# SIA-IDE/MMGT

Measured on AMD Instinct MI355X. Metric: UNet3D denoise-steps/sec at 512x512x24 bf16, higher is better.
Workload: dtype bf16; 1 GPU; BASELINE configs[1]: 512x512x24 pose2vid denoise step (CFG batch 2, UNet3D + MM-HAA, 16 reference banks, 1 window of 24 frames, guidance 3.5, DDIM v-pred), random-init weights; frames=24, parallelism=clip-parallel x1

## Files before the change

### include/mmgt_hip.h

```cpp
#ifndef MMGT_HIP_H
#define MMGT_HIP_H

#ifdef __cplusplus
extern "C" {
#endif

#define MMGT_F32 0
#define MMGT_BF16 1

#define MMGT_ACT_NONE 0
#define MMGT_ACT_GEGLU 1
#define MMGT_ACT_SILU 2
#define MMGT_ACT_RELU 3
#define MMGT_ACT_QUICK_GELU 4
#define MMGT_ACT_GELU 5
#define MMGT_ACT_MISH 6

int mmgt_abi_version(void);
const char* mmgt_last_error(void);
int mmgt_tune(const char* key, int value);
int mmgt_tune_get(const char* key, int* value);
int mmgt_box_calib(float warm_seconds, float* mfma_mhz, float* mfma_tflops, void* stream);
void mmgt_gemm16_set_trace(void* p);
void mmgt_ffn_set_trace(void* p);

int mmgt_gemm(const void* A, long lda, const void* W, const float* bias, const float* bias2, int bias2_rows,
              const float* row_scale, float alpha, const void* residual, long ldr, void* out, long ldo, int M, int N,
              int K, int act, int batch, long bsA, long bsW, long bsR, long bsO, int dtype, void* stream);

int mmgt_gemm_post(const void* A, long lda, const void* W, const float* bias, const float* row_scale, float alpha,
                   const float* bias_post, const void* residual, long ldr, void* out, long ldo, int M, int N, int K,
                   int dtype, void* stream);

int mmgt_conv3x3_nhwc(const void* x0, int C0, const void* x1, int C1, int NB, int IH, int IW, int stride, int upsample,
                      const void* Wp, const float* bias, const float* bias2, int bias2_rows, const void* residual,
                      void* out, int Cout, int act, int dtype, void* stream);

int mmgt_conv1x1_cat_nhwc(const void* x0, int C0, const void* x1, int C1, long rows, const void* Wp, const float* bias, const void* residual, void* out,
                          int Cout, int dtype, void* stream);

int mmgt_conv_taps_gather(const void* Y, int ldY, const float* bias, void* out, int NB, int H, int W, int dtype, void* stream);

int mmgt_groupnorm_chunks(int HW);
int mmgt_groupnorm_affine(const void* x, int C, const float* gamma, const float* beta, float* workspace, float* scale, float* shift,
                          int NB, int HW, int G, float eps, int dtype, void* stream);
int mmgt_groupnorm_affine2(const void* x0, int C0, const void* x1, int C1, const float* gamma, const float* beta, float* workspace, float* scale,
                           float* shift, int NB, int HW, int G, float eps, int dtype, void* stream);
int mmgt_groupnorm_nhwc(const void* x0, int C0, const void* x1, int C1, const float* gamma, const float* beta, void* out,
                        float* workspace, int NB, int HW, int G, float eps, int silu, int dtype, void* stream);

int mmgt_layernorm(const void* x, long ldx, const float* gamma, const float* beta, float eps, const float* pe, int pe_div,
                   int pe_mod, void* out, long ldo, int rows, int C, int dtype, void* stream);

int mmgt_attention(const void* q, long q_bs0, long q_bs1, long q_ts, const void* k, long k_bs0, long k_bs1, long k_ts,
                   const void* v, long v_bs0, long v_bs1, long v_ts, void* o, long o_bs0, long o_bs1, long o_ts,
                   int bdiv, const void* k2, const void* v2, long k2_bs, long k2_ts, long v2_bs, long v2_ts, int k2_bdiv,
                   int nk2, int seg2_first_batch, int batch, int heads, int hd, int nq, int nk, float scale,
                   int v_transposed, int dtype, void* stream);

int mmgt_attention_scaled(const void* q, long q_bs0, long q_bs1, long q_ts, const void* k, long k_bs0, long k_bs1, long k_ts,
                          const void* v, long v_bs0, long v_bs1, long v_ts, void* o, long o_bs0, long o_bs1, long o_ts,
                          const float* out_scale, long os_group_stride, int os_heads, int batch, int heads, int hd, int nq, int nk,
                          float scale, int dtype, void* stream);

int mmgt_attention_twin(const void* q, long q_bs0, long q_bs1, long q_ts, const void* k, long k_bs0, long k_bs1, long k_ts,
                        const void* v, long v_bs0, long v_bs1, long v_ts, void* o, void* o_twin, long o_bs0, long o_bs1, long o_ts,
                        int bdiv, const void* k2, const void* v2, long k2_bs, long k2_ts, long v2_bs, long v2_ts, int k2_bdiv,
                        int nk2, int batch, int heads, int hd, int nq, int nk, float scale, int dtype, void* stream);

int mmgt_softmax_rows(const void* x, long ldx, void* out, long ldo, int rows, int cols, float scale, int dtype,
                      void* stream);

int mmgt_gemm_bf16_f32(const void* A, long lda, const void* W, long ldw, float* out, long ldo, int M, int N, int K, void* stream);
int mmgt_qk_split3(const float* qk, const float* bias_q, const float* bias_k, void* Qp, void* Kp, long rows, int C, void* stream);
int mmgt_softmax_rows_f32_bf16(const float* x, long ldx, void* out, long ldo, int rows, int cols, float scale, void* stream);

int mmgt_ncfhw_to_nhwc(const float* in, void* out, int B, int C, int F, int H, int W, int Cpad, float scale, int dtype,
                       void* stream);
int mmgt_nhwc_to_ncfhw(const void* in, float* out, int B, int C, int F, int H, int W, int Cpad, float scale, float shift,
                       int clamp01, int dtype, void* stream);

int mmgt_timestep_features(const float* timesteps, void* out, int B, int dim, int dtype, void* stream);

int mmgt_ff_fused_image_bytes(int C, int inner);
int mmgt_ff_fused(const void* x, long ldx, const float* ln_gamma, const float* ln_beta, float eps, const void* wimg,
                  const float* bias2, const void* residual, long ldr, void* out, long ldo, int M, int C, int inner, int dtype,
                  void* stream);
int mmgt_ff_fused_po(const void* x, long ldx, const float* ln_gamma, const float* ln_beta, float eps, const void* wimg,
                     const float* bias2, const void* residual, long ldr, const void* wpo, const float* bias_po, const void* residual2,
                     long ldr2, void* out, long ldo, int M, int C, int inner, int dtype, void* stream);

long mmgt_rowgemm320_image_bytes(int N);
// ... 105 lines not shown
```

### mmgt_amd/csrc/common.h

```cpp
#pragma once
#ifndef MMGT_ST_AUX
#define MMGT_ST_AUX 0
#endif
#include <hip/hip_runtime.h>
#include <hip/hip_bf16.h>
#include <stdint.h>

typedef __attribute__((ext_vector_type(16))) float f32x16;
typedef __attribute__((ext_vector_type(8))) short s16x8;
typedef __attribute__((ext_vector_type(4))) short s16x4;
typedef __attribute__((ext_vector_type(4))) float f32x4;
typedef __attribute__((ext_vector_type(4))) unsigned int u32x4;
typedef __attribute__((ext_vector_type(2))) unsigned int u32x2;

typedef unsigned short bf16_t;

__device__ __forceinline__ float bf16_to_f32(bf16_t v) { return __uint_as_float(((unsigned int)v) << 16); }
__device__ __forceinline__ bf16_t f32_to_bf16(float f) {
  __hip_bfloat16 b = __float2bfloat16(f);
  return *reinterpret_cast<bf16_t*>(&b);
}

template <typename T> struct Elem;
template <> struct Elem<float> {
// ... 61 lines not shown

__device__ __forceinline__ float silu_f(float x) { return x / (1.f + __expf(-x)); }
__device__ __forceinline__ float mish_f(float x) {
  if (x > 20.f) return x;
  const float e = __expf(x), n = e * (e + 2.f);
  return x * n / (n + 2.f);
}
__device__ __forceinline__ float quick_gelu_f(float x) { return x / (1.f + __expf(-1.702f * x)); }
typedef __attribute__((ext_vector_type(2))) float f32x2;
#define MMGT_GELU_K  1.0442737824274138f
#define MMGT_GELU_C1 (0.04986734694f * MMGT_GELU_K)
#define MMGT_GELU_C2 (0.02114100615f * MMGT_GELU_K)
#define MMGT_GELU_C3 (0.003277626324f * MMGT_GELU_K)
#define MMGT_GELU_C4 (0.000038003575f * MMGT_GELU_K)
#define MMGT_GELU_C5 (0.000048890636f * MMGT_GELU_K)
#define MMGT_GELU_C6 (0.00000538297500f * MMGT_GELU_K)
__device__ __forceinline__ float gelu_erf_f(float x) {
  const float z = fabsf(x);
  float p = fmaf(MMGT_GELU_C6, z, MMGT_GELU_C5);
  p = fmaf(p, z, MMGT_GELU_C4);
  p = fmaf(p, z, MMGT_GELU_C3);
  p = fmaf(p, z, MMGT_GELU_C2);
  p = fmaf(p, z, MMGT_GELU_C1);
  p = fmaf(p, z, MMGT_GELU_K);
  p *= p; p *= p; p *= p; p *= p;
  const float h = __builtin_amdgcn_rcpf(p);
  return fmaf(-z, h, fmaxf(x, 0.f));
}
__device__ __forceinline__ f32x2 gelu_erf_f2(f32x2 x) {
  const f32x2 z = {fabsf(x[0]), fabsf(x[1])};
  f32x2 p = z * MMGT_GELU_C6 + MMGT_GELU_C5;
  p = p * z + MMGT_GELU_C4;
  p = p * z + MMGT_GELU_C3;
  p = p * z + MMGT_GELU_C2;
  p = p * z + MMGT_GELU_C1;
  p = p * z + MMGT_GELU_K;
  p *= p; p *= p; p *= p; p *= p;
  const f32x2 h = {__builtin_amdgcn_rcpf(p[0]), __builtin_amdgcn_rcpf(p[1])};
  const f32x2 r = {fmaxf(x[0], 0.f), fmaxf(x[1], 0.f)};
  return r - z * h;
}

__device__ __forceinline__ float wave_sum(float v) {
#pragma unroll
  for (int o = 32; o > 0; o >>= 1) v += __shfl_xor(v, o);
  return v;
}
__device__ __forceinline__ float wave_max(float v) {
#pragma unroll
  for (int o = 32; o > 0; o >>= 1) v = fmaxf(v, __shfl_xor(v, o));
  return v;
}

#ifdef __cplusplus
extern "C" {
#endif
void mmgt_set_error(const char* fmt, ...);
#ifdef __cplusplus
}
#endif

#define MMGT_CHECK(cond, ...)      \
  do {                             \
    if (!(cond)) {                 \
      mmgt_set_error(__VA_ARGS__); \
      return 1;                    \
    }                              \
  } while (0)

#define MMGT_LAUNCH_CHECK()                                              \
  do {                                                                   \
    hipError_t e_ = hipGetLastError();                                   \
    if (e_ != hipSuccess) {                                              \
      mmgt_set_error("%s:%d: %s", __FILE__, __LINE__, hipGetErrorString(e_)); \
      return 2;                                                          \
    }                                                                    \
  } while (0)

__device__ __forceinline__ void st_out16(void* p, u32x4 v) {
#if MMGT_ST_AUX == 16
  asm volatile("global_store_dwordx4 %0, %1, off sc1\n\ts_nop 1" ::"v"(p), "v"(v) : "memory");
#else
  *reinterpret_cast<u32x4*>(p) = v;
#endif
}
```

### mmgt_amd/csrc/gemm.hip

```cpp
#include <string.h>

#include <type_traits>

#include "common.h"
#include "gemm_common.h"
#include "mmgt_hip.h"

#ifndef MMGT_GEMM_VARIANT
#define MMGT_GEMM_VARIANT 7
#endif

namespace {

constexpr bool V_FRAGDB = (MMGT_GEMM_VARIANT & 1) != 0;
constexpr bool V_ILV = (MMGT_GEMM_VARIANT & 2) != 0;
constexpr bool V_LATE = (MMGT_GEMM_VARIANT & 4) != 0;
constexpr bool V_LATE_ALL = (MMGT_GEMM_VARIANT & 8) != 0;
constexpr bool V_NODMA = (MMGT_GEMM_VARIANT & 16) != 0;

template <int CTRL>
__device__ __forceinline__ unsigned dpp_quad(unsigned v) {
  return (unsigned)__builtin_amdgcn_mov_dpp((int)v, CTRL, 0xf, 0xf, true);
}
template <int S>
// ... 560 lines not shown
              if (ep.act == 5) x = gelu_erf_f(x);
              if (ep.act == 6) x = mish_f(x);
              x *= (ep.row_scale ? ep.row_scale[m] : 1.f) * ep.alpha;
              if (POST_OK && ep.bias_post) x += ep.bias_post[ncol];
            }
            if (res) x += Elem<T>::ld(res + (long)m * ep.ldr + ocol);
            Elem<T>::st(out + (long)m * ep.ldo + ocol, x);
          }
        }
      }
    }
  }
}

template <typename T, int MODE, int BM, int BN, int WM, int WN, int NSTAGE, int ROWB = 128, int EPI = 0>
int launch_cfg(const ADesc& ad, const void* W, long bsw, const Epi& ep, int M, int N, int K, int batch, hipStream_t s) {
  const int tiles_m = (M + BM - 1) / BM, tiles_n = (N + BN - 1) / BN;
  const size_t lds = (size_t)NSTAGE * (BM + BN) * ROWB;
  auto kern = gemm_kernel<T, MODE, BM, BN, WM, WN, NSTAGE, ROWB, EPI>;
  static int resident = 0;
  if (!resident) {
    if (hipFuncSetAttribute(reinterpret_cast<const void*>(kern), hipFuncAttributeMaxDynamicSharedMemorySize, (int)lds) !=
        hipSuccess) {
      mmgt_set_error("gemm: cannot reserve %zu bytes of LDS", lds);
      return 2;
    }
    int per_cu = 0, dev = 0;
    hipDeviceProp_t prop;
    if (hipOccupancyMaxActiveBlocksPerMultiprocessor(&per_cu, kern, WM * WN * 64, lds) != hipSuccess || per_cu < 1 ||
        hipGetDevice(&dev) != hipSuccess || hipGetDeviceProperties(&prop, dev) != hipSuccess) {
      mmgt_set_error("gemm: occupancy query failed");
      return 2;
    }
    resident = per_cu * prop.multiProcessorCount;
  }
  long gx = (resident + batch - 1) / batch;
  gx = (gx + 7) / 8 * 8;
  if (gx > (long)tiles_m * tiles_n) gx = (long)tiles_m * tiles_n;
  dim3 grid((unsigned)gx, 1, batch);
  hipLaunchKernelGGL(kern, grid, dim3(WM * WN * 64), lds, s, ad, reinterpret_cast<const char*>(W), bsw, ep, M, N, K, tiles_m,
                     tiles_n);
  MMGT_LAUNCH_CHECK();
  return 0;
}

int g_splitk = 1;
int g_tailsplit = 1;
int g_gemm_cfg = 0;
int g_bm192 = 1;

}
int mmgt_gemm16_launch(int mode, int bn, const void* ad, const void* W, long bsw, const void* ep, int M, int N, int K,
                       int batch, void* stream);
int mmgt_gemm16_splitk(int mode, int bn, const void* ad, const void* W, const void* ep, int M, int N, int K, int S, void* stream, int m0);
namespace {

template <typename T, int MODE>
int launch(const ADesc& ad, const void* W, long bsw, const Epi& ep, int M, int N, int K, int batch, hipStream_t s) {
  const bool geglu = ep.act == 1;
  int cfg = g_gemm_cfg;
  if ((cfg == 0 || cfg == 18) && g_splitk && std::is_same<T, bf16_t>::value && batch == 1 && ep.act == 0 && ep.fast && !ep.row_scale &&
      ep.alpha == 1.f && !ep.bias_post && N % 8 == 0 && K >= 2560 && (N % 256 == 0 || N % 320 == 0) &&
      (((uintptr_t)ep.bias | (uintptr_t)ep.bias2) & 15) == 0) {
    const int bn = N % 256 == 0 ? 256 : 320;
    const long tiles = (long)((M + 255) / 256) * (N / bn);
    const int nch = K / 64;
    int S = 0;
    for (int c = 8; c >= 2; --c)
      if (tiles * c <= 256 && nch % c == 0 && nch / c >= (tiles <= 64 ? 16 : 64)) { S = c; break; }
    if (S >= 2 && tiles <= 128 && (MODE == 1 || tiles <= 32 || tiles > 64)) return mmgt_gemm16_splitk(MODE, bn, &ad, W, &ep, M, N, K, S, s, 0);
  }
  if (cfg == 18) cfg = 0;
  if (cfg == 0) {
    const long tiles128 = (long)((M + 127) / 128) * ((N + 127) / 128) * batch;
    const long tiles256 = (long)((M + 255) / 256) * ((N + 127) / 128) * batch;
    const long tiles256sq = (long)((M + 255) / 256) * ((N + 255) / 256) * batch;
    const bool big_ok = N % 256 == 0 && K >= 2560 && tiles256sq >= 192 && tiles256sq <= 512;
    const bool sq_ok = ((N + 255) / 256) * 256l * 100 <= (long)N * 107 && ((M + 255) / 256) * 256l * 100 <= (long)M * 115 && tiles256sq >= 192;
    const bool b16 = std::is_same<T, bf16_t>::value;
    if (MODE == 1) {
      if (b16 && N % 320 == 0 && (M >= 49152 || (M >= 24576 && N >= 640))) cfg = 17;
      else if (b16 && N % 256 == 0 && tiles256sq >= 192) cfg = 16;
      else cfg = (N % 320 == 0 && M >= 49152) ? 12 : big_ok ? 9 : (tiles128 < 512 || N <= 64) ? 3 : 1;
    } else if (b16 && !geglu && N % 320 == 0 && N <= 960 && M >= 131072) cfg = 17;
    else if (b16 && !geglu && N % 320 == 0 && N <= 1280 && M >= 49152 && (K >= 1280 || ep.residual || N == 1280)) cfg = 17;
    else if (b16 && !geglu && N == 640 && M >= 24576 && K >= 2560 && g_bm192) cfg = 17;
    else if (sq_ok) cfg = b16 ? 16 : 9;
    else if (geglu || K >= 1280) cfg = tiles256 >= 256 ? 6 : (!geglu && tiles128 <= 256) ? 3 : 1;
    else if (M >= 131072 && N >= 640) cfg = 6;
    else cfg = 1;
  }
  if (geglu && (cfg == 3 || cfg == 12)) cfg = 1;
  if (MODE == 1 && ad.up >= 2 && cfg != 16 && cfg != 17) cfg = N % 320 == 0 ? 17 : 16;
  bool bm192 = cfg == 19;
  if (cfg == 19) cfg = 17;
  if (cfg == 17 && !bm192 && g_gemm_cfg == 0 && g_bm192 && std::is_same<T, bf16_t>::value && batch == 1 && N % 320 == 0) {
    const long tn = N / 320;
    const long r256 = (((long)(M + 255) / 256) * tn + 255) / 256, r192 = (((long)(M + 191) / 192) * tn + 255) / 256;
    bm192 = (double)r192 * 0.88 < (double)r256 * 0.97;
  }
  if (cfg == 16 || cfg == 17) {
    const bool post = ep.row_scale || ep.alpha != 1.f || ep.bias_post;
    if (std::is_same<T, bf16_t>::value && ep.fast && ep.act <= (cfg == 16 && !post ? 1 : 0) &&
        (((uintptr_t)ep.bias | (uintptr_t)ep.bias2 | (uintptr_t)ep.bias_post) & 15) == 0 && N % 4 == 0) {
      const int bn = cfg == 16 ? 256 : bm192 ? 192320 : 320;
      const int bnc = cfg == 16 ? 256 : 320;
      const long tiles_n = (N + bnc - 1) / bnc, tiles_m = (M + 255) / 256, ntile = tiles_m * tiles_n;
      const int nch = K / 64;
      if (g_tailsplit && (!bm192 || g_gemm_cfg == 0) && MODE == 1 && batch == 1 && !ad.ksplit && ep.act == 0 && !post && N % bnc == 0 && N % 8 == 0 && K >= 2560 && nch % 2 == 0 && ntile > 256) {
        const long rows_a = (256 * (ntile / 256) / tiles_n) * 256;
        const long tail = (tiles_m - rows_a / 256) * tiles_n;
        const long img = MODE == 1 ? (long)ad.OH * ad.OW : 1;
        if (rows_a > 0 && rows_a < M && tail > 0 && 2 * tail <= 256 && 4 * tail >= 256 && rows_a % img == 0) {
          int rc = mmgt_gemm16_launch(MODE, bnc, &ad, W, bsw, &ep, (int)rows_a, N, K, 1, s);
          if (rc) return rc;
          ADesc adb = ad;
          Epi epb = ep;
          const long esz = sizeof(T);
          if (MODE == 1) {
            const long n0 = rows_a / img;
            adb.src0 = ad.src0 + n0 * ad.IH * ad.IW * ad.C0 * esz;
            if (ad.src1) adb.src1 = ad.src1 + n0 * ad.IH * ad.IW * ad.C1 * esz;
          } else {
            adb.src0 = ad.src0 + rows_a * ad.ld0 * esz;
          }
          if (ep.residual) epb.residual = ep.residual + rows_a * ep.ldr * esz;
          epb.out = ep.out + rows_a * ep.ldo * esz;
          return mmgt_gemm16_splitk(MODE, bnc, &adb, W, &epb, (int)(M - rows_a), N, K, 2, s, (int)rows_a);
        }
      }
      return mmgt_gemm16_launch(MODE, bn, &ad, W, bsw, &ep, M, N, K, batch, s);
    }
    if (MODE == 1 && ad.up >= 2) {
      mmgt_set_error("conv: the four-phase upsample form and the two-source 1 x 1 conv need the gemm16 path (bf16, 16-byte aligned bias, Cout %% 4 == 0)");
      return 1;
    }
    cfg = cfg == 16 ? 9 : geglu ? 1 : 12;
  }
  if (cfg == 20) {
    if (std::is_same<T, bf16_t>::value && ep.fast && ep.act == 0 && (((uintptr_t)ep.bias | (uintptr_t)ep.bias2 | (uintptr_t)ep.bias_post) & 15) == 0 && N % 4 == 0)
      return mmgt_gemm16_launch(MODE, 128, &ad, W, bsw, &ep, M, N, K, batch, s);
    cfg = 1;
  }
  if (!ep.fast || ep.act >= 2) return launch_cfg<T, MODE, 128, 128, 2, 2, 2, 128, 2>(ad, W, bsw, ep, M, N, K, batch, s);
  if (ep.row_scale || ep.alpha != 1.f || ep.bias_post) {
    if (MODE == 0 && !geglu) return launch_cfg<T, 0, 128, 128, 2, 2, 2, 128, 1>(ad, W, bsw, ep, M, N, K, batch, s);
    return launch_cfg<T, MODE, 128, 128, 2, 2, 2, 128, 2>(ad, W, bsw, ep, M, N, K, batch, s);
  }
#ifdef MMGT_GEMM_AB
  switch (cfg) {
    case 3: return launch_cfg<T, MODE, 128, 64, 2, 2, 2>(ad, W, bsw, ep, M, N, K, batch, s);
    case 6: return launch_cfg<T, MODE, 256, 128, 4, 2, 3>(ad, W, bsw, ep, M, N, K, batch, s);
    case 9: return launch_cfg<T, MODE, 256, 256, 2, 4, 2>(ad, W, bsw, ep, M, N, K, batch, s);
    case 12: return launch_cfg<T, MODE, 128, 320, 4, 2, 2>(ad, W, bsw, ep, M, N, K, batch, s);
    default: return launch_cfg<T, MODE, 128, 128, 2, 2, 2>(ad, W, bsw, ep, M, N, K, batch, s);
  }
#else
  switch (cfg) {
    case 1: return launch_cfg<T, MODE, 128, 128, 2, 2, 2>(ad, W, bsw, ep, M, N, K, batch, s);
    case 3: return launch_cfg<T, MODE, 128, 64, 2, 2, 2>(ad, W, bsw, ep, M, N, K, batch, s);
    case 6: return launch_cfg<T, MODE, 256, 128, 4, 2, 3>(ad, W, bsw, ep, M, N, K, batch, s);
    case 9: return launch_cfg<T, MODE, 256, 256, 2, 4, 2>(ad, W, bsw, ep, M, N, K, batch, s);
    case 12: return launch_cfg<T, MODE, 128, 320, 4, 2, 2>(ad, W, bsw, ep, M, N, K, batch, s);
    default: return launch_cfg<T, MODE, 128, 128, 2, 2, 2>(ad, W, bsw, ep, M, N, K, batch, s);
  }
#endif
}

int epi_fast(const Epi& ep, int N, int n_out, int esz) {
  auto al16 = [](const void* p) { return (reinterpret_cast<uintptr_t>(p) & 15) == 0; };
  bool ok = N % 8 == 0 && n_out % 8 == 0 && al16(ep.out) && (ep.ldo * esz) % 16 == 0 && (ep.bso * esz) % 16 == 0;
  ok = ok && (ep.bias2 == nullptr || ep.bias2_rows >= 256);
  if (ep.residual) ok = ok && al16(ep.residual) && (ep.ldr * esz) % 16 == 0 && (ep.bsr * esz) % 16 == 0;
  return ok ? 1 : 0;
}

int check_common(int dtype, int M, int N, int K, int act) {
  MMGT_CHECK(dtype == MMGT_F32 || dtype == MMGT_BF16, "gemm: bad dtype %d", dtype);
  MMGT_CHECK(M > 0 && N > 0 && K > 0, "gemm: empty problem M=%d N=%d K=%d", M, N, K);
  MMGT_CHECK(K % 64 == 0, "gemm: K=%d must be a multiple of 64 (pad channels on the host)", K);
  MMGT_CHECK(act >= 0 && act <= 6, "gemm: bad act %d", act);
  MMGT_CHECK(act != 1 || N % 64 == 0, "gemm: GEGLU needs N %% 64 == 0 (N=%d)", N);
  return 0;
}

}

void mmgt_attn_set64(int v);
void mmgt_gn_set_rows(int v);
void mmgt_attn_set_heads_inner(int v);
void mmgt_attn_set_attn80(int v);
void mmgt_attn_set_nomax(int v);
void mmgt_gemm16_set_pb(int v);
void mmgt_gemm16_set_stagger(int v);
void mmgt_gn_set_interleave(int v);
void mmgt_gn_set_lpr0(int v);
void mmgt_gn_set_narrow(int v);
void mmgt_gn_set_slab(int v);
void mmgt_ffn_set_dbg(int v);
void mmgt_rowgemm_set_dbg(int v);
void mmgt_tleg_set_abl(int v);
void mmgt_gnconv_set_abl(int v);
void mmgt_rconv_set_abl(int v);
void mmgt_rconv_set_stagger(int v);
void mmgt_rconv_set_cb(int v);
namespace {
struct HostSwitch { const char* key; int value; };
HostSwitch g_host[] = {
    {"fused_ff", 1},
    {"twin_attention", 1},
    {"shared_rows", 1},
    {"oz3", 1},
    {"rowgemm", 1},
    {"tleg", 1},
    {"rconv", 5},
    {"conv_out_taps", 1},
    {"ffpo_cat", 1},
    {"sc_cat", 1},
    {"up2", 1},
    {"rconv_stats", 1},
    {"gnconv", 2},
    {"zero_audio_skip", 1},
    {"window_state", 1},
    {"smga_graph", 1},
};
}
extern "C" int mmgt_tune_get(const char* key, int* value) {
  if (key && value)
    for (const HostSwitch& h : g_host)
      if (!strcmp(key, h.key)) { *value = h.value; return 0; }
  mmgt_set_error("tune_get: unknown key");
  return 1;
}
extern "C" int mmgt_tune(const char* key, int value) {
  if (key)
    for (HostSwitch& h : g_host)
      if (!strcmp(key, h.key)) { h.value = value; return 0; }
  if (key && !strcmp(key, "gemm_cfg")) { g_gemm_cfg = value; return 0; }
  if (key && !strcmp(key, "attn64")) { mmgt_attn_set64(value); return 0; }
  if (key && !strcmp(key, "attn_nomax") && (value == 0 || value == 1)) { mmgt_attn_set_nomax(value); return 0; }
  if (key && !strcmp(key, "attn_heads_inner")) { mmgt_attn_set_heads_inner(value); return 0; }
  if (key && !strcmp(key, "attn80")) { mmgt_attn_set_attn80(value); return 0; }
  if (key && !strcmp(key, "g16_pb")) { mmgt_gemm16_set_pb(value); return 0; }
  if (key && !strcmp(key, "g16_stagger")) { mmgt_gemm16_set_stagger(value); return 0; }
  if (key && !strcmp(key, "gn_rows")) { mmgt_gn_set_rows(value); return 0; }
  if (key && !strcmp(key, "gn_interleave")) { mmgt_gn_set_interleave(value); return 0; }
  if (key && !strcmp(key, "gn_narrow")) { mmgt_gn_set_narrow(value); return 0; }
  if (key && !strcmp(key, "gn_slab")) { mmgt_gn_set_slab(value); return 0; }
  if (key && !strcmp(key, "gn_lpr0")) { if (value != 4 && value != 8 && value != 16) return -1; mmgt_gn_set_lpr0(value); return 0; }
  if (key && !strcmp(key, "splitk")) { g_splitk = value; return 0; }
  if (key && !strcmp(key, "bm192")) { g_bm192 = value; return 0; }
  if (key && !strcmp(key, "tailsplit")) { g_tailsplit = value; return 0; }
  if (key && !strcmp(key, "rconv_cb") && (value == 0 || value == 320 || value == 256 || value == 160)) { mmgt_rconv_set_cb(value); return 0; }
  if (key && !strcmp(key, "rconv_stagger") && value >= 0 && value <= 8192) { mmgt_rconv_set_stagger(value); return 0; }
#ifdef MMGT_ABLATE
  if (key && !strcmp(key, "ffn_dbg") && value >= 0 && value <= 2) { mmgt_ffn_set_dbg(value); return 0; }
  if (key && !strcmp(key, "gnconv_abl") && value >= 0 && value <= 255) { mmgt_gnconv_set_abl(value); return 0; }
  if (key && !strcmp(key, "tleg_abl") && value >= 0 && value <= 128) { mmgt_tleg_set_abl(value); return 0; }
  if (key && !strcmp(key, "rconv_abl") && value >= 0 && value <= 31) { mmgt_rconv_set_abl(value); return 0; }
  if (key && !strcmp(key, "rowgemm_dbg") && value >= 0 && value <= 5) { mmgt_rowgemm_set_dbg(value); return 0; }
#else
  if (key && !strcmp(key, "rowgemm_dbg") && (value == 0 || value == 5)) { mmgt_rowgemm_set_dbg(value); return 0; }
  if (key && (!strcmp(key, "ffn_dbg") || !strcmp(key, "gnconv_abl") || !strcmp(key, "tleg_abl") || !strcmp(key, "rconv_abl") || !strcmp(key, "rowgemm_dbg"))) {
    mmgt_set_error("tune: '%s' selects a timing ablation whose results are garbage; the product library does not contain them (build libmmgt_hip_abl.so with `make -C mmgt_amd/csrc abl` and load it through MMGT_LIB)", key);
    return 1;
  }
#endif
  mmgt_set_error("tune: unknown key");
  return 1;
}

namespace {
template <typename T>
__global__ __launch_bounds__(256) void gemv_kernel(const T* __restrict__ A, long lda, const T* __restrict__ W, const float* __restrict__ bias,
                                                   T* __restrict__ out, long ldo, int M, int N, int K, int act) {
  constexpr int VEC = 16 / sizeof(T);
  const int lane = threadIdx.x & 63, n = blockIdx.x * 4 + (threadIdx.x >> 6);
  if (n >= N) return;
// ... 28 lines not shown
                      long ldo, int M, int N, int K, int act, int batch, long bsA, long bsW, long bsR, long bsO, int dtype,
                      void* stream) {
  if (check_common(dtype, M, N, K, act)) return 1;
  MMGT_CHECK(A && W && out, "gemm: null pointer");
  MMGT_CHECK(lda >= 1 && batch >= 1, "gemm: lda %ld < 1 or batch %d < 1", lda, batch);
  MMGT_CHECK(!bias2 || bias2_rows > 0, "gemm: bias2_rows must be positive");
  const int esz = dtype == MMGT_BF16 ? 2 : 4;
  MMGT_CHECK(((uintptr_t)A % 16) == 0 && ((uintptr_t)W % 16) == 0 && (lda * esz) % 16 == 0 && (bsA * esz) % 16 == 0 &&
                 (bsW * esz) % 16 == 0,
             "gemm: A/W must be 16-byte aligned with 16-byte aligned rows");
  MMGT_CHECK(((long)(M - 1) * lda + K) * esz < (1l << 31) && (long)N * K * esz < (1l << 31),
             "gemm: an operand (per batch entry) exceeds the 2 GiB range of the 32-bit LDS-DMA offsets");
  if (M == 1 && batch == 1 && !bias2 && !row_scale && alpha == 1.f && !bias_post && !residual && (act == 0 || act == 2) && K % (16 / esz) == 0) {
    if (dtype == MMGT_BF16)
      hipLaunchKernelGGL(gemv_kernel<bf16_t>, dim3((unsigned)((N + 3) / 4)), dim3(256), 0, (hipStream_t)stream, (const bf16_t*)A, lda, (const bf16_t*)W, bias,
                         (bf16_t*)out, ldo, M, N, K, act);
    else
      hipLaunchKernelGGL(gemv_kernel<float>, dim3((unsigned)((N + 3) / 4)), dim3(256), 0, (hipStream_t)stream, (const float*)A, lda, (const float*)W, bias,
                         (float*)out, ldo, M, N, K, act);
    MMGT_LAUNCH_CHECK();
    return 0;
  }
  ADesc ad{};
  ad.src0 = (const char*)A;
  ad.ld0 = lda;
  ad.bs0 = bsA;
  Epi ep{};
  ep.bias = bias; ep.bias2 = bias2; ep.bias2_rows = bias2_rows; ep.row_scale = row_scale; ep.alpha = alpha;
  ep.bias_post = bias_post;
  MMGT_CHECK(!bias_post || (act != 1 && ((uintptr_t)bias_post % 16) == 0), "gemm: bias_post needs a 16-byte aligned vector and no GEGLU");
  ep.residual = (const char*)residual; ep.ldr = ldr; ep.out = (char*)out; ep.ldo = ldo; ep.act = act;
  ep.bsr = bsR; ep.bso = bsO;
  ep.fast = epi_fast(ep, N, act == 1 ? N / 2 : N, esz);
  hipStream_t s = (hipStream_t)stream;
  return dtype == MMGT_BF16 ? launch<bf16_t, 0>(ad, W, bsW, ep, M, N, K, batch, s)
                            : launch<float, 0>(ad, W, bsW, ep, M, N, K, batch, s);
}

extern "C" int mmgt_gemm(const void* A, long lda, const void* W, const float* bias, const float* bias2, int bias2_rows,
                         const float* row_scale, float alpha, const void* residual, long ldr, void* out, long ldo, int M,
                         int N, int K, int act, int batch, long bsA, long bsW, long bsR, long bsO, int dtype,
                         void* stream) {
  return gemm_entry(A, lda, W, bias, bias2, bias2_rows, row_scale, alpha, nullptr, residual, ldr, out, ldo, M, N, K, act,
                    batch, bsA, bsW, bsR, bsO, dtype, stream);
}

extern "C" int mmgt_gemm_post(const void* A, long lda, const void* W, const float* bias, const float* row_scale, float alpha,
                              const float* bias_post, const void* residual, long ldr, void* out, long ldo, int M, int N,
                              int K, int dtype, void* stream) {
  return gemm_entry(A, lda, W, bias, nullptr, 0, row_scale, alpha, bias_post, residual, ldr, out, ldo, M, N, K, 0, 1, 0, 0, 0,
                    0, dtype, stream);
}

extern "C" int mmgt_conv3x3_nhwc(const void* x0, int C0, const void* x1, int C1, int NB, int IH, int IW, int stride,
                                 int upsample, const void* Wp, const float* bias, const float* bias2, int bias2_rows,
                                 const void* residual, void* out, int Cout, int act, int dtype, void* stream) {
  MMGT_CHECK(x0 && Wp && out, "conv3x3: null pointer");
  int pad_lo = 1;
  if (stride == -2) { stride = 2; pad_lo = 0; }
  MMGT_CHECK(stride == 1 || stride == 2, "conv3x3: stride %d", stride);
  MMGT_CHECK(!(upsample && stride != 1), "conv3x3: upsample requires stride 1");
  MMGT_CHECK(upsample >= 0 && upsample <= 2, "conv3x3: upsample = %d (0, 1, or 2 = the four-phase form with the packing.pack_conv3x3_up2 image)", upsample);
  MMGT_CHECK(C0 % 64 == 0 && C1 % 64 == 0 && (x1 != nullptr) == (C1 > 0),
             "conv3x3: channel counts must be multiples of 64 (C0=%d C1=%d)", C0, C1);
  MMGT_CHECK(act == 0 || act == 2 || act == 3, "conv3x3: act %d unsupported", act);
  MMGT_CHECK(((uintptr_t)x0 % 16) == 0 && ((uintptr_t)x1 % 16) == 0 && ((uintptr_t)Wp % 16) == 0,
             "conv3x3: pointers must be 16-byte aligned");
  const bool up2 = upsample == 2;
  MMGT_CHECK(!up2 || (dtype == MMGT_BF16 && !residual && !bias2 && act == 0 && !x1 && (Cout % 256 == 0 || Cout % 320 == 0)),
             "conv3x3: the four-phase upsample form is bf16, one source, bias only, Cout a multiple of 256 or 320");
  const int VH = upsample == 1 ? IH * 2 : IH, VW = upsample == 1 ? IW * 2 : IW;
  const int OH = up2 ? IH : (VH + pad_lo + 1 - 3) / stride + 1, OW = up2 ? IW : (VW + pad_lo + 1 - 3) / stride + 1;
  const long M = (long)NB * OH * OW;
  MMGT_CHECK(M < (1l << 31) && (!up2 || 4 * M * Cout * 2 < (1l << 31) * 8), "conv3x3: too many output pixels");
  {
    const long esz_ = dtype == MMGT_BF16 ? 2 : 4, px = (long)NB * IH * IW;
    MMGT_CHECK(px * C0 * esz_ < (1l << 31) && px * C1 * esz_ < (1l << 31) && (long)Cout * 9 * (C0 + C1) * esz_ < (1l << 31),
               "conv3x3: a tensor exceeds the 2 GiB range of the 32-bit LDS-DMA offsets (split the batch)");
  }
  const int K = (up2 ? 4 : 9) * (C0 + C1);
  if (check_common(dtype, (int)M, Cout, K, act)) return 1;
  ADesc ad{};
  ad.src0 = (const char*)x0; ad.src1 = (const char*)x1; ad.C0 = C0; ad.C1 = C1; ad.IH = IH; ad.IW = IW; ad.OH = OH;
  ad.OW = OW; ad.stride = stride; ad.up = upsample; ad.pad = pad_lo;
  make_fastdiv((unsigned)(OH * OW), ad.fd_hw);
  make_fastdiv((unsigned)OW, ad.fd_ow);
  Epi ep{};
  ep.bias = bias; ep.bias2 = bias2; ep.bias2_rows = bias2_rows; ep.alpha = 1.f; ep.residual = (const char*)residual;
  ep.ldr = Cout; ep.out = (char*)out; ep.ldo = Cout; ep.act = act;
  ep.fast = epi_fast(ep, Cout, Cout, dtype == MMGT_BF16 ? 2 : 4);
  hipStream_t s = (hipStream_t)stream;
  if (up2) return launch<bf16_t, 1>(ad, Wp, (long)Cout * K, ep, (int)M, Cout, K, 4, s);
  return dtype == MMGT_BF16 ? launch<bf16_t, 1>(ad, Wp, 0, ep, (int)M, Cout, K, 1, s)
                            : launch<float, 1>(ad, Wp, 0, ep, (int)M, Cout, K, 1, s);
}

extern "C" int mmgt_conv1x1_cat_nhwc(const void* x0, int C0, const void* x1, int C1, long rows, const void* Wp, const float* bias, const void* residual,
                                     void* out, int Cout, int dtype, void* stream) {
  MMGT_CHECK(x0 && x1 && Wp && out && rows > 0, "conv1x1_cat: null pointer");
  MMGT_CHECK(dtype == MMGT_BF16, "conv1x1_cat: bf16 only");
  MMGT_CHECK(C0 > 0 && C1 > 0 && C0 % 64 == 0 && C1 % 64 == 0 && (Cout % 256 == 0 || Cout % 320 == 0), "conv1x1_cat: C0 = %d, C1 = %d must be multiples of 64, Cout = %d of 256 or 320",
             C0, C1, Cout);
  MMGT_CHECK(rows < (1l << 31) && rows * C0 * 2 < (1l << 31) && rows * C1 * 2 < (1l << 31) && (long)Cout * (C0 + C1) * 2 < (1l << 31), "conv1x1_cat: an operand exceeds 2 GiB");
  MMGT_CHECK((((uintptr_t)x0 | (uintptr_t)x1 | (uintptr_t)Wp | (uintptr_t)residual | (uintptr_t)out | (uintptr_t)bias) & 15) == 0, "conv1x1_cat: pointers must be 16-byte aligned");
  const int K = C0 + C1;
  if (check_common(dtype, (int)rows, Cout, K, 0)) return 1;
  ADesc ad{};
  ad.src0 = (const char*)x0; ad.src1 = (const char*)x1; ad.C0 = C0; ad.C1 = C1; ad.IH = 1; ad.IW = (int)rows; ad.OH = 1; ad.OW = (int)rows;
  ad.stride = 1; ad.up = 3; ad.pad = 1;
  make_fastdiv((unsigned)rows, ad.fd_hw);
  make_fastdiv((unsigned)rows, ad.fd_ow);
  Epi ep{};
  ep.bias = bias; ep.alpha = 1.f; ep.residual = (const char*)residual; ep.ldr = Cout; ep.out = (char*)out; ep.ldo = Cout;
  ep.fast = epi_fast(ep, Cout, Cout, 2);
  return launch<bf16_t, 1>(ad, Wp, 0, ep, (int)rows, Cout, K, 1, (hipStream_t)stream);
}
```

### mmgt_amd/csrc/gemm16.hip

```cpp
#include <type_traits>

#include "common.h"
#include "gemm_common.h"
#include "mmgt_hip.h"

namespace {

typedef __attribute__((ext_vector_type(4))) float acc4;

__device__ __forceinline__ acc4 mma16(s16x8 a, s16x8 b, acc4 c) {
  return __builtin_amdgcn_mfma_f32_16x16x32_bf16(a, b, c, 0, 0, 0);
}

template <int MODE, int BN, int BM = 256>
__global__ __launch_bounds__(512, 2) void gemm16_kernel(ADesc ad, const char* __restrict__ W, long bsw, Epi ep, int M, int N,
                                                        int K, int tiles_m, int tiles_n, int pb_stg, unsigned long long* trace) {
  extern __shared__ __attribute__((aligned(1024))) char smem[];
  typedef bf16_t T;
  static_assert(BN == 128 || BN == 256 || BN == 320, "BN");
  static_assert(BM == 256 || BM == 192, "BM");
  constexpr int ESZ = 2, ROWB = 128, BK = 64, NW = 8;
  constexpr int WROWS = BM / 4, RT = WROWS / 16;
  constexpr int A_BYTES = BM * ROWB, B_BYTES = BN * ROWB, STAGE_BYTES = A_BYTES + B_BYTES;
  constexpr int CPR = 8, RPD = 8;
// ... 418 lines not shown
    } else {
      epilogue(false_type{}, false_type{}, false_type{});
    }
    stamp(3);
    ++trace_n;
    if (wr == 1) __builtin_amdgcn_s_barrier();
  }
  if (wr == 0) __builtin_amdgcn_s_barrier();
}

unsigned long long* g_trace = nullptr;
int g_stg = -1;
int g_pb = -1;

template <int MODE, int BN, int BM = 256>
int launch16(const ADesc& ad, const void* W, long bsw, const Epi& ep, int M, int N, int K, int batch, hipStream_t s) {
  const int tiles_m = (M + BM - 1) / BM, tiles_n = (N + BN - 1) / BN;
  const size_t lds = (size_t)2 * (BM + BN) * 128 + 4 * 2048;
  auto kern = gemm16_kernel<MODE, BN, BM>;
  static int resident = 0;
  if (!resident) {
    if (hipFuncSetAttribute(reinterpret_cast<const void*>(kern), hipFuncAttributeMaxDynamicSharedMemorySize, (int)lds) !=
        hipSuccess) {
      mmgt_set_error("gemm16: cannot reserve %zu bytes of LDS", lds);
      return 2;
    }
    int dev = 0;
    hipDeviceProp_t prop;
    if (hipGetDevice(&dev) != hipSuccess || hipGetDeviceProperties(&prop, dev) != hipSuccess) {
      mmgt_set_error("gemm16: device query failed");
      return 2;
    }
    resident = prop.multiProcessorCount;
  }
  long gx = (resident + batch - 1) / batch;
  gx = (gx + 7) / 8 * 8;
  if (gx > (long)tiles_m * tiles_n) gx = (long)tiles_m * tiles_n;
  dim3 grid((unsigned)gx, 1, batch);
  const int pb = g_pb >= 0 ? g_pb : (MODE == 0 && tiles_n >= 8 && tiles_m >= 8) ? 8 : 1;
  const int stg = g_stg >= 0 ? g_stg : (MODE == 0 && ep.residual && !ad.ksplit && K <= 1280) ? 10 : 0;
  hipLaunchKernelGGL(kern, grid, dim3(512), lds, s, ad, reinterpret_cast<const char*>(W), bsw, ep, M, N, K, tiles_m, tiles_n, pb | (stg << 8), g_trace);
  MMGT_LAUNCH_CHECK();
  return 0;
}

}

extern "C" void mmgt_gemm16_set_trace(void* p) { g_trace = reinterpret_cast<unsigned long long*>(p); }
void mmgt_gemm16_set_pb(int v) { g_pb = v; }
void mmgt_gemm16_set_stagger(int v) { g_stg = v; }

namespace {

__global__ __launch_bounds__(256) void splitk_reduce_kernel(const float* __restrict__ part, int S, long slab, const float* __restrict__ bias,
                                                            const float* __restrict__ bias2, int b2rows, const bf16_t* __restrict__ res,
                                                            long ldr, bf16_t* __restrict__ out, long ldo, int M, int N, int m0) {
  const int nv = N / 8;
  const long idx = (long)blockIdx.x * 256 + threadIdx.x;
  if (idx >= (long)M * nv) return;
  const int m = (int)(idx / nv), c = (int)(idx - (long)m * nv) * 8;
  const float* p = part + (long)m * N + c;
  f32x4 a0 = *reinterpret_cast<const f32x4*>(p), a1 = *reinterpret_cast<const f32x4*>(p + 4);
  for (int z = 1; z < S; ++z) {
    a0 += *reinterpret_cast<const f32x4*>(p + z * slab);
    a1 += *reinterpret_cast<const f32x4*>(p + z * slab + 4);
  }
  if (bias) { a0 += *reinterpret_cast<const f32x4*>(bias + c); a1 += *reinterpret_cast<const f32x4*>(bias + c + 4); }
  if (bias2) {
    const float* b2 = bias2 + (long)((m + m0) / b2rows) * N + c;
    a0 += *reinterpret_cast<const f32x4*>(b2);
    a1 += *reinterpret_cast<const f32x4*>(b2 + 4);
  }
  if (res) {
    union { u32x4 u; bf16_t e[8]; } r8;
    r8.u = *reinterpret_cast<const u32x4*>(res + (long)m * ldr + c);
#pragma unroll
    for (int e = 0; e < 4; ++e) { a0[e] += bf16_to_f32(r8.e[e]); a1[e] += bf16_to_f32(r8.e[4 + e]); }
  }
  *reinterpret_cast<u32x4*>(out + (long)m * ldo + c) =
      (u32x4){pack_bf16x2(a0[0], a0[1]), pack_bf16x2(a0[2], a0[3]), pack_bf16x2(a1[0], a1[1]), pack_bf16x2(a1[2], a1[3])};
}

constexpr int MAX_DEV = 16, MAX_RETIRED = 8;
struct SplitkWs {
  float* p = nullptr; size_t bytes = 0; bool captured = false;
  float* retired[MAX_RETIRED] = {};
  size_t retired_bytes[MAX_RETIRED] = {};
  int nretired = 0;
};
SplitkWs g_splitk_ws[MAX_DEV];

float* splitk_workspace(size_t need, hipStream_t s) {
  int dev = 0;
  if (hipGetDevice(&dev) != hipSuccess || dev < 0 || dev >= MAX_DEV) {
    mmgt_set_error("gemm16 split-K: device query failed");
    return nullptr;
  }
  SplitkWs& w = g_splitk_ws[dev];
  hipStreamCaptureStatus cs = hipStreamCaptureStatusNone;
  const bool capturing = hipStreamIsCapturing(s, &cs) == hipSuccess && cs != hipStreamCaptureStatusNone;
  if (need > w.bytes) {
    if (capturing) {
      mmgt_set_error("gemm16 split-K: the partial-sum workspace would have to grow to %zu bytes inside a stream capture; run the "
                     "shape once outside the capture (warm-up) first", need);
      return nullptr;
    }
    size_t want = need;
    if (w.bytes && want < 2 * w.bytes) want = 2 * w.bytes;
    if (w.p && !w.captured) {
      (void)hipFree(w.p);
    } else if (w.p) {
      if (w.nretired == MAX_RETIRED) {
        mmgt_set_error("gemm16 split-K: %d captured workspaces already retired; destroy the graphs that hold them and restart", MAX_RETIRED);
        return nullptr;
      }
      w.retired[w.nretired] = w.p;
      w.retired_bytes[w.nretired++] = w.bytes;
    }
    w.p = nullptr; w.bytes = 0; w.captured = false;
    if (hipMalloc(reinterpret_cast<void**>(&w.p), want) != hipSuccess) {
      if (want == need || hipMalloc(reinterpret_cast<void**>(&w.p), need) != hipSuccess) {
        w.p = nullptr;
        mmgt_set_error("gemm16 split-K: cannot allocate %zu bytes of partial sums", need);
        return nullptr;
      }
      want = need;
    }
    w.bytes = want;
  }
  if (capturing) w.captured = true;
  return w.p;
}

}

int mmgt_gemm16_splitk(int mode, int bn, const void* adp, const void* W, const void* epp, int M, int N, int K, int S, void* stream, int m0) {
  ADesc ad = *reinterpret_cast<const ADesc*>(adp);
  const Epi& ep = *reinterpret_cast<const Epi*>(epp);
  hipStream_t s = (hipStream_t)stream;
  const size_t need = (size_t)S * M * N * sizeof(float);
  float* ws = splitk_workspace(need, s);
  if (!ws) return 2;
  ad.ksplit = 1;
  ad.ldw = K;
  Epi pe{};
  pe.out = reinterpret_cast<char*>(ws);
  pe.ldo = N;
  pe.bso = (long)M * N;
  pe.alpha = 1.f;
  pe.fast = 1;
  const int ks = K / S;
  int rc;
  if (bn == 320) rc = mode == 0 ? launch16<0, 320>(ad, W, 0, pe, M, N, ks, S, s) : launch16<1, 320>(ad, W, 0, pe, M, N, ks, S, s);
  else rc = mode == 0 ? launch16<0, 256>(ad, W, 0, pe, M, N, ks, S, s) : launch16<1, 256>(ad, W, 0, pe, M, N, ks, S, s);
  if (rc) return rc;
  const long nthr = (long)M * (N / 8);
  hipLaunchKernelGGL(splitk_reduce_kernel, dim3((unsigned)((nthr + 255) / 256)), dim3(256), 0, s, ws, S, (long)M * N, ep.bias, ep.bias2,
                     ep.bias2 ? ep.bias2_rows : 1, reinterpret_cast<const bf16_t*>(ep.residual), ep.ldr, reinterpret_cast<bf16_t*>(ep.out), ep.ldo, M, N, m0);
  MMGT_LAUNCH_CHECK();
  return 0;
}

extern "C" int mmgt_gemm_bf16_f32(const void* A, long lda, const void* W, long ldw, float* out, long ldo, int M, int N, int K, void* stream) {
  MMGT_CHECK(A && W && out && M > 0 && N > 0 && K > 0, "gemm_bf16_f32: bad arguments");
  MMGT_CHECK(K % 64 == 0 && N % 8 == 0 && lda >= K && ldw >= K && ldo >= N && lda % 8 == 0 && ldw % 8 == 0 && ldo % 4 == 0,
             "gemm_bf16_f32: unsupported shape M=%d N=%d K=%d lda=%ld ldw=%ld ldo=%ld", M, N, K, lda, ldw, ldo);
  MMGT_CHECK(((uintptr_t)A % 16) == 0 && ((uintptr_t)W % 16) == 0 && ((uintptr_t)out % 16) == 0, "gemm_bf16_f32: pointers must be 16-byte aligned");
  MMGT_CHECK(((long)(M - 1) * lda + K) * 2 < (1l << 31) && ((long)(N - 1) * ldw + K) * 2 < (1l << 31),
             "gemm_bf16_f32: an operand exceeds the 2 GiB range of the 32-bit LDS-DMA offsets");
  ADesc ad{};
  ad.src0 = reinterpret_cast<const char*>(A);
  ad.ld0 = lda;
  ad.ksplit = 1;
  ad.ldw = (int)ldw;
  Epi pe{};
  pe.out = reinterpret_cast<char*>(out);
  pe.ldo = ldo;
  pe.alpha = 1.f;
  pe.fast = 1;
  return launch16<0, 256>(ad, W, 0, pe, M, N, K, 1, (hipStream_t)stream);
}

int mmgt_gemm16_launch(int mode, int bn, const void* adp, const void* W, long bsw, const void* epp, int M, int N, int K,
                       int batch, void* stream) {
  const ADesc& ad = *reinterpret_cast<const ADesc*>(adp);
  const Epi& ep = *reinterpret_cast<const Epi*>(epp);
  hipStream_t s = (hipStream_t)stream;
  if (bn == 192320) return mode == 0 ? launch16<0, 320, 192>(ad, W, bsw, ep, M, N, K, batch, s) : launch16<1, 320, 192>(ad, W, bsw, ep, M, N, K, batch, s);
  if (bn == 320) return mode == 0 ? launch16<0, 320>(ad, W, bsw, ep, M, N, K, batch, s) : launch16<1, 320>(ad, W, bsw, ep, M, N, K, batch, s);
  if (bn == 128) return mode == 0 ? launch16<0, 128>(ad, W, bsw, ep, M, N, K, batch, s) : launch16<1, 128>(ad, W, bsw, ep, M, N, K, batch, s);
  return mode == 0 ? launch16<0, 256>(ad, W, bsw, ep, M, N, K, batch, s) : launch16<1, 256>(ad, W, bsw, ep, M, N, K, batch, s);
}
```

### mmgt_amd/csrc/norm.hip

```cpp
#include "common.h"
#include "mmgt_hip.h"

namespace {

constexpr int GN_MAXC = 2560;

int g_gn_interleave = -1;
int g_gn_lpr0 = 8;
int g_gn_narrow = 2;
int g_gn_slab = 1;
int g_gn_rows = 0;
inline int gn_chunks(int HW) {
  int c = HW >= 2048 ? (HW + 127) / 128 : (HW + 31) / 32;
  return c < 1 ? 1 : (c > 256 ? 256 : c);
}
inline int gn_chunks_used(int HW, int C, int NB) {
  int rows = g_gn_rows > 0 ? g_gn_rows : HW >= 2048 ? (C <= 320 ? 256 : 128) : 64;
  if (g_gn_rows <= 0 && HW >= 65536) rows = max(rows, (int)(((long)HW * NB + 1023) / 1024));
  int c = (HW + rows - 1) / rows;
  const int cap = gn_chunks(HW);
  return c < 1 ? 1 : (c > cap ? cap : c);
}

template <typename T>
// ... 365 lines not shown
  for (int e = 0; e < VEC; ++e) acc[e] = 0.f;
  if (active)
#pragma unroll 4
    for (int r = r0; r < HW; r += rp) {
      float f[VEC];
      VecIO<T>::load(src + r * rstride, f);
#pragma unroll
      for (int e = 0; e < VEC; ++e) acc[e] += f[e];
    }
  reduce(acc, 0);
  const float cnt = (float)HW * (float)cg;
  float mean[VEC];
#pragma unroll
  for (int e = 0; e < VEC; ++e) { mean[e] = gstat[0][gid[e]] / cnt; acc[e] = 0.f; }
  if (active)
#pragma unroll 4
    for (int r = r0; r < HW; r += rp) {
      float f[VEC];
      VecIO<T>::load(src + r * rstride, f);
#pragma unroll
      for (int e = 0; e < VEC; ++e) { const float d = f[e] - mean[e]; acc[e] += d * d; }
    }
  reduce(acc, 1);
  if (active) {
    float sc[VEC], sh[VEC];
#pragma unroll
    for (int e = 0; e < VEC; ++e) {
      const float rstd = rsqrtf(gstat[1][gid[e]] / cnt + eps);
      sc[e] = rstd * gamma[c + e];
      sh[e] = beta[c + e] - mean[e] * sc[e];
    }
    if (tscale) {
      if (r0 == 0) {
#pragma unroll
        for (int e = 0; e < VEC; ++e) { tscale[(long)n * C + c + e] = sc[e]; tshift[(long)n * C + c + e] = sh[e]; }
      }
      return;
    }
    T* dst = out + (long)n * HW * C + c;
#pragma unroll 4
    for (int r = r0; r < HW; r += rp) {
      float f[VEC];
      VecIO<T>::load(src + r * rstride, f);
#pragma unroll
      for (int e = 0; e < VEC; ++e) {
        const float v = f[e] * sc[e] + sh[e];
        f[e] = silu ? silu_f(v) : v;
      }
      VecIO<T>::store(dst + (long)r * C, f);
    }
  }
}

template <typename T, int NR, int NTHR = 256>
__global__ __launch_bounds__(NTHR) void gn_slab_kernel(const T* __restrict__ x0, int C0, const T* __restrict__ x1, int C1,
                                                      const float* __restrict__ gamma, const float* __restrict__ beta,
                                                      T* __restrict__ out, int HW, int G, int gpw, float eps, int silu,
                                                      float* __restrict__ tscale, float* __restrict__ tshift) {
  constexpr int VEC = VecIO<T>::VEC;
  __shared__ float part[NTHR * VEC];
  __shared__ float chan[320];
  __shared__ float gstat[2][4];
  const int C = C0 + C1, cg = C / G, cw = gpw * cg, nvw = cw / VEC;
  int n = blockIdx.y, sl = blockIdx.x;
  {
    const int nsl = gridDim.x, tot = nsl * gridDim.y;
    if ((tot & 7) == 0) {
      const int lin = blockIdx.y * nsl + blockIdx.x, v = (lin & 7) * (tot >> 3) + (lin >> 3);
      n = v / nsl;
      sl = v - n * nsl;
    }
  }
  const int c_lo = sl * cw;
  const int tid = threadIdx.x;
  const int rp = NTHR / nvw;
  const int vc = tid % nvw, r0 = tid / nvw;
  const bool active = r0 < rp;
  const int c = c_lo + vc * VEC;
  const T* src = c < C0 ? x0 + (long)n * HW * C0 + c : x1 + (long)n * HW * C1 + (c - C0);
  const long rstride = c < C0 ? C0 : C1;
  int gid[VEC];
#pragma unroll
  for (int e = 0; e < VEC; ++e) gid[e] = (vc * VEC + e) / cg;

  u32x4 raw[NR];
#pragma unroll
  for (int i = 0; i < NR; ++i) {
    const int r = r0 + i * rp;
    raw[i] = (active && r < HW) ? *reinterpret_cast<const u32x4*>(src + r * rstride) : (u32x4)(0u);
  }
  auto dec = [](const u32x4& u, float* f) {
    union { u32x4 u; T e[VEC]; } v;
    v.u = u;
#pragma unroll
    for (int e = 0; e < VEC; ++e) f[e] = Elem<T>::ld(&v.e[e]);
  };
  auto reduce = [&](const float (&acc)[VEC], int which) {
#pragma unroll
    for (int e = 0; e < VEC; ++e) part[tid * VEC + e] = active ? acc[e] : 0.f;
    __syncthreads();
    for (int ch = tid; ch < cw; ch += NTHR) {
      const int v = ch / VEC, e = ch % VEC;
      float s = 0.f;
      for (int r = 0; r < rp; ++r) s += part[(r * nvw + v) * VEC + e];
      chan[ch] = s;
    }
    __syncthreads();
    if (tid < gpw) {
      float s = 0.f;
      for (int k = 0; k < cg; ++k) s += chan[tid * cg + k];
      gstat[which][tid] = s;
    }
    __syncthreads();
  };

  float acc[VEC];
#pragma unroll
  for (int e = 0; e < VEC; ++e) acc[e] = 0.f;
#pragma unroll
  for (int i = 0; i < NR; ++i)
    if (active && r0 + i * rp < HW) {
      float f[VEC];
      dec(raw[i], f);
#pragma unroll
      for (int e = 0; e < VEC; ++e) acc[e] += f[e];
    }
  reduce(acc, 0);
  const float cnt = (float)HW * (float)cg;
  float mean[VEC];
#pragma unroll
  for (int e = 0; e < VEC; ++e) { mean[e] = gstat[0][gid[e]] / cnt; acc[e] = 0.f; }
#pragma unroll
  for (int i = 0; i < NR; ++i)
    if (active && r0 + i * rp < HW) {
      float f[VEC];
      dec(raw[i], f);
#pragma unroll
      for (int e = 0; e < VEC; ++e) { const float d = f[e] - mean[e]; acc[e] += d * d; }
    }
  reduce(acc, 1);
  if (active) {
    float sc[VEC], sh[VEC];
// ... 7 lines not shown
      if (r0 == 0) {
#pragma unroll
        for (int e = 0; e < VEC; ++e) { tscale[(long)n * C + c + e] = sc[e]; tshift[(long)n * C + c + e] = sh[e]; }
      }
      return;
    }
    T* dst = out + (long)n * HW * C + c;
#pragma unroll
    for (int i = 0; i < NR; ++i) {
      const int r = r0 + i * rp;
      if (r < HW) {
        float f[VEC];
        dec(raw[i], f);
#pragma unroll
        for (int e = 0; e < VEC; ++e) {
          const float v = f[e] * sc[e] + sh[e];
          f[e] = silu ? silu_f(v) : v;
        }
        VecIO<T>::store(dst + (long)r * C, f);
      }
    }
  }
}

inline int gn_slab_gpw(int C, int G, int HW, int vec, int* nr, int* nthr) {
  const int cg = C / G;
  auto need = [&](int gpw, int threads) {
    const int cw = gpw * cg;
    if (G % gpw || cw % vec || cw > 320 || cw / vec > 256) return 1 << 30;
    const int rp = threads / (cw / vec);
    return (HW + rp - 1) / rp;
  };
  int pick = 0;
  *nthr = 256;
  for (int gpw = 4; gpw >= 1 && !pick; gpw >>= 1)
    if (need(gpw, 256) <= 6) pick = gpw;
  for (int gpw = 1; gpw <= 4 && !pick; gpw <<= 1)
    if (need(gpw, 256) <= 22) pick = gpw;
  if (!pick) {
    for (int gpw = 1; gpw <= 4 && !pick; gpw <<= 1)
      if (need(gpw, 1024) <= 16) pick = gpw;
    if (!pick) return 0;
    *nthr = 1024;
    *nr = 16;
    return pick;
  }
  const int n = need(pick, 256);
  *nr = n <= 2 ? 2 : n <= 4 ? 4 : n <= 6 ? 6 : n <= 12 ? 12 : 22;
  return pick;
}
template <typename T>
void gn_slab_launch(int nr, int nthr, dim3 grid, hipStream_t s, const void* x0, int C0, const void* x1, int C1, const float* gamma, const float* beta, void* out,
                    int HW, int G, int gpw, float eps, int silu, float* tscale, float* tshift) {
#define GN_SLAB(NR_, NT_) hipLaunchKernelGGL((gn_slab_kernel<T, NR_, NT_>), grid, dim3(NT_), 0, s, (const T*)x0, C0, (const T*)x1, C1, gamma, beta, (T*)out, HW, G, gpw, \
                                             eps, silu, tscale, tshift)
  if (nthr == 1024) GN_SLAB(16, 1024);
  else if (nr == 2) GN_SLAB(2, 256); else if (nr == 4) GN_SLAB(4, 256); else if (nr == 6) GN_SLAB(6, 256); else if (nr == 12) GN_SLAB(12, 256); else GN_SLAB(22, 256);
#undef GN_SLAB
}

template <typename T>
__global__ __launch_bounds__(256) void ln_kernel(const T* __restrict__ x, long ldx, const float* __restrict__ gamma,
                                                 const float* __restrict__ beta, float eps, const float* __restrict__ pe,
                                                 int pe_div, int pe_mod, T* __restrict__ out, long ldo, int rows, int C,
                                                 int lpr, int vpl) {
  constexpr int VEC = VecIO<T>::VEC;
  constexpr int MAXV = 5;
  const int lane = threadIdx.x & 63, wid = threadIdx.x >> 6;
  const int rpw = 64 / lpr;
  const int sub = lane / lpr, li = lane - sub * lpr;
  const long row = ((long)blockIdx.x * 4 + wid) * rpw + sub;
  const bool ok = row < rows;
  const long rrow = ok ? row : rows - 1;
  float f[MAXV][VEC];
  float sum = 0.f;
#pragma unroll
  for (int i = 0; i < MAXV; ++i) {
    if (i < vpl) {
      VecIO<T>::load(x + rrow * ldx + (li + lpr * i) * VEC, f[i]);
#pragma unroll
      for (int e = 0; e < VEC; ++e) sum += f[i][e];
    }
  }
  for (int o = lpr >> 1; o > 0; o >>= 1) sum += __shfl_xor(sum, o);
  const float mean = sum / (float)C;
  float sq = 0.f;
#pragma unroll
  for (int i = 0; i < MAXV; ++i) {
    if (i < vpl)
#pragma unroll
      for (int e = 0; e < VEC; ++e) { const float d = f[i][e] - mean; sq += d * d; }
  }
  for (int o = lpr >> 1; o > 0; o >>= 1) sq += __shfl_xor(sq, o);
  const float rstd = rsqrtf(sq / (float)C + eps);
  if (!ok) return;
  const float* perow = pe ? pe + (long)((row / pe_div) % pe_mod) * C : nullptr;
  if (!pe && pe_mod > 1) beta += (long)((row / pe_div) % pe_mod) * C;
#pragma unroll
  for (int i = 0; i < MAXV; ++i) {
    if (i < vpl) {
      const int c = (li + lpr * i) * VEC;
      float g[VEC], b[VEC];
#pragma unroll
      for (int e = 0; e < VEC; e += 4) {
        *reinterpret_cast<f32x4*>(&g[e]) = *reinterpret_cast<const f32x4*>(gamma + c + e);
        *reinterpret_cast<f32x4*>(&b[e]) = *reinterpret_cast<const f32x4*>(beta + c + e);
      }
#pragma unroll
      for (int e = 0; e < VEC; ++e) {
        float v = (f[i][e] - mean) * rstd * g[e] + b[e];
        if (perow) v += perow[c + e];
        f[i][e] = v;
      }
      VecIO<T>::store(out + row * ldo + c, f[i]);
    }
  }
}

}

void mmgt_gn_set_rows(int v) { g_gn_rows = v; }
void mmgt_gn_set_interleave(int v) { g_gn_interleave = v; }
void mmgt_gn_set_lpr0(int v) { g_gn_lpr0 = v; }
void mmgt_gn_set_narrow(int v) { g_gn_narrow = v; }
void mmgt_gn_set_slab(int v) { g_gn_slab = v; }

namespace {
constexpr int GN_NARROW_U = 4;
inline bool gn_narrow_fits(int nvec, int C1, int HW) {
  return g_gn_narrow && C1 == 0 && nvec >= 8 && nvec <= 64 && (64 % nvec == 0 || (nvec > 32 && g_gn_narrow >= 2)) &&
         HW % (4 * (64 / nvec) * GN_NARROW_U) == 0;
}
inline int gn_narrow_chunks(int HW, int NB, int nvec) {
  const int step = 4 * (64 / nvec) * GN_NARROW_U;
  int rows = g_gn_rows > 0 ? g_gn_rows : 64;
  if (g_gn_rows <= 0) rows = max(rows, (int)(((long)HW * NB + 2047) / 2048));
  rows = (rows + step - 1) / step * step;
  int chunks = (HW + rows - 1) / rows;
  const int cap = gn_chunks(HW);
  return chunks < 1 ? 1 : (chunks > cap ? cap : chunks);
}
}
extern "C" int mmgt_groupnorm_chunks(int HW) { return gn_chunks(HW); }

extern "C" int mmgt_groupnorm_nhwc(const void* x0, int C0, const void* x1, int C1, const float* gamma, const float* beta,
                                   void* out, float* workspace, int NB, int HW, int G, float eps, int silu, int dtype,
                                   void* stream) {
  MMGT_CHECK(x0 && gamma && beta && out && workspace, "groupnorm: null pointer");
  MMGT_CHECK(dtype == MMGT_F32 || dtype == MMGT_BF16, "groupnorm: bad dtype %d", dtype);
  MMGT_CHECK((x1 != nullptr) == (C1 > 0), "groupnorm: x1/C1 mismatch");
  const int C = C0 + C1, vec = dtype == MMGT_BF16 ? 8 : 4;
  MMGT_CHECK(C <= GN_MAXC && C % G == 0 && G <= 64 && C0 % vec == 0 && C1 % vec == 0,
             "groupnorm: unsupported channels C0=%d C1=%d G=%d", C0, C1, G);
  MMGT_CHECK(NB > 0 && HW > 0 && NB <= 65535, "groupnorm: bad NB=%d HW=%d", NB, HW);
  hipStream_t s = (hipStream_t)stream;
  {
    int nr = 0, nthr = 256;
    const int gpw = g_gn_slab ? gn_slab_gpw(C, G, HW, vec, &nr, &nthr) : 0;
    if (gpw) {
      dim3 grid(G / gpw, NB);
      if (dtype == MMGT_BF16) gn_slab_launch<bf16_t>(nr, nthr, grid, s, x0, C0, x1, C1, gamma, beta, out, HW, G, gpw, eps, silu, nullptr, nullptr);
      else gn_slab_launch<float>(nr, nthr, grid, s, x0, C0, x1, C1, gamma, beta, out, HW, G, gpw, eps, silu, nullptr, nullptr);
      MMGT_LAUNCH_CHECK();
      return 0;
    }
  }
  {
    const int cg = C / G;
    const int gpw = (HW > 64 && G % 2 == 0 && (2 * cg) % vec == 0) ? 2 : 4;
    const int cw = gpw * cg;
    if (HW <= 256 && G % gpw == 0 && cw % vec == 0 && cw <= 320 && cw / vec <= 256 && C0 % vec == 0) {
// ... 149 lines not shown
```

### mmgt_amd/hip.py

```python
import ctypes
import os
from ctypes import c_float, c_int, c_long, c_void_p

import torch

_HERE = os.path.dirname(os.path.abspath(__file__))
LIB_PATH = os.environ.get("MMGT_LIB") or os.path.join(_HERE, "libmmgt_hip.so")

F32, BF16 = 0, 1
ACT_NONE, ACT_GEGLU, ACT_SILU, ACT_RELU, ACT_QUICK_GELU, ACT_GELU, ACT_MISH = 0, 1, 2, 3, 4, 5, 6

_lib = None
DMA_LIMIT = (1 << 31) - 1

_SIGS = {
    "mmgt_abi_version": (c_int, []),
    "mmgt_last_error": (ctypes.c_char_p, []),
    "mmgt_tune": (c_int, [ctypes.c_char_p, c_int]),
    "mmgt_tune_get": (c_int, [ctypes.c_char_p, ctypes.POINTER(c_int)]),
    "mmgt_box_calib": (c_int, [c_float, ctypes.POINTER(c_float), ctypes.POINTER(c_float), c_void_p]),
    "mmgt_gemm16_set_trace": (None, [c_void_p]),
    "mmgt_ffn_set_trace": (None, [c_void_p]),
    "mmgt_rconv_set_trace": (None, [c_void_p]),
    "mmgt_gemm": (c_int, [c_void_p, c_long, c_void_p, c_void_p, c_void_p, c_int, c_void_p, c_float, c_void_p, c_long,
                          c_void_p, c_long, c_int, c_int, c_int, c_int, c_int, c_long, c_long, c_long, c_long, c_int,
                          c_void_p]),
    "mmgt_gemm_post": (c_int, [c_void_p, c_long, c_void_p, c_void_p, c_void_p, c_float, c_void_p, c_void_p, c_long, c_void_p,
                               c_long, c_int, c_int, c_int, c_int, c_void_p]),
    "mmgt_conv3x3_nhwc": (c_int, [c_void_p, c_int, c_void_p, c_int, c_int, c_int, c_int, c_int, c_int, c_void_p,
                                  c_void_p, c_void_p, c_int, c_void_p, c_void_p, c_int, c_int, c_int, c_void_p]),
    "mmgt_groupnorm_chunks": (c_int, [c_int]),
    "mmgt_groupnorm_nhwc": (c_int, [c_void_p, c_int, c_void_p, c_int, c_void_p, c_void_p, c_void_p, c_void_p, c_int,
                                    c_int, c_int, c_float, c_int, c_int, c_void_p]),
    "mmgt_layernorm": (c_int, [c_void_p, c_long, c_void_p, c_void_p, c_float, c_void_p, c_int, c_int, c_void_p, c_long,
                               c_int, c_int, c_int, c_void_p]),
    "mmgt_attention": (c_int, [c_void_p, c_long, c_long, c_long, c_void_p, c_long, c_long, c_long, c_void_p, c_long,
                               c_long, c_long, c_void_p, c_long, c_long, c_long, c_int, c_void_p, c_void_p, c_long,
                               c_long, c_long, c_long, c_int, c_int, c_int, c_int, c_int, c_int, c_int, c_int, c_float,
                               c_int, c_int, c_void_p]),
    "mmgt_attention_scaled": (c_int, [c_void_p, c_long, c_long, c_long, c_void_p, c_long, c_long, c_long, c_void_p, c_long, c_long, c_long,
                                      c_void_p, c_long, c_long, c_long, c_void_p, c_long, c_int, c_int, c_int, c_int, c_int, c_int, c_float,
                                      c_int, c_void_p]),
    "mmgt_attention_twin": (c_int, [c_void_p, c_long, c_long, c_long, c_void_p, c_long, c_long, c_long, c_void_p, c_long, c_long, c_long,
                                    c_void_p, c_void_p, c_long, c_long, c_long, c_int, c_void_p, c_void_p, c_long, c_long, c_long, c_long,
                                    c_int, c_int, c_int, c_int, c_int, c_int, c_int, c_float, c_int, c_void_p]),
    "mmgt_softmax_rows": (c_int, [c_void_p, c_long, c_void_p, c_long, c_int, c_int, c_float, c_int, c_void_p]),
    "mmgt_gemm_bf16_f32": (c_int, [c_void_p, c_long, c_void_p, c_long, c_void_p, c_long, c_int, c_int, c_int, c_void_p]),
    "mmgt_qk_split3": (c_int, [c_void_p, c_void_p, c_void_p, c_void_p, c_void_p, c_long, c_int, c_void_p]),
    "mmgt_softmax_rows_f32_bf16": (c_int, [c_void_p, c_long, c_void_p, c_long, c_int, c_int, c_float, c_void_p]),
    "mmgt_ncfhw_to_nhwc": (c_int, [c_void_p, c_void_p, c_int, c_int, c_int, c_int, c_int, c_int, c_float, c_int, c_void_p]),
    "mmgt_nhwc_to_ncfhw": (c_int, [c_void_p, c_void_p, c_int, c_int, c_int, c_int, c_int, c_int, c_float, c_float, c_int,
                                   c_int, c_void_p]),
    "mmgt_conv1x1_cat_nhwc": (c_int, [c_void_p, c_int, c_void_p, c_int, c_long, c_void_p, c_void_p, c_void_p, c_void_p, c_int, c_int, c_void_p]),
    "mmgt_conv_taps_gather": (c_int, [c_void_p, c_int, c_void_p, c_void_p, c_int, c_int, c_int, c_int, c_void_p]),
    "mmgt_timestep_features": (c_int, [c_void_p, c_void_p, c_int, c_int, c_int, c_void_p]),
    "mmgt_ff_fused_image_bytes": (c_int, [c_int, c_int]),
    "mmgt_ff_fused": (c_int, [c_void_p, c_long, c_void_p, c_void_p, c_float, c_void_p, c_void_p, c_void_p, c_long, c_void_p, c_long,
                              c_int, c_int, c_int, c_int, c_void_p]),
    "mmgt_rowgemm320_image_bytes": (c_long, [c_int]),
    "mmgt_rowgemm_set_trace": (None, [c_void_p]),
    "mmgt_ff_fused_po": (c_int, [c_void_p, c_long, c_void_p, c_void_p, c_float, c_void_p, c_void_p, c_void_p, c_long, c_void_p, c_void_p,
                                 c_void_p, c_long, c_void_p, c_long, c_int, c_int, c_int, c_int, c_void_p]),
    "mmgt_groupnorm_affine": (c_int, [c_void_p, c_int, c_void_p, c_void_p, c_void_p, c_void_p, c_void_p, c_int, c_int, c_int, c_float, c_int,
                                      c_void_p]),
    "mmgt_rowgemm320": (c_int, [c_void_p, c_long, c_int, c_void_p, c_void_p, c_int, c_int, c_float, c_void_p, c_void_p, c_void_p, c_int, c_void_p,
                                c_long, c_void_p, c_long, c_int, c_void_p, c_int, c_int, c_int, c_int, c_int, c_void_p]),
    "mmgt_gn_silu_conv3x3_image_bytes": (c_long, [c_int, c_int]),
    "mmgt_gn_silu_conv3x3": (c_int, [c_void_p, c_void_p, c_void_p, c_void_p, c_void_p, c_void_p, c_void_p, c_void_p, c_int, c_int, c_int, c_int, c_int, c_int, c_int, c_void_p]),
    "mmgt_gn_silu_conv3x3_unet_image_bytes": (c_long, [c_int, c_int]),
    "mmgt_gn_silu_conv3x3_unet": (c_int, [c_void_p, c_int, c_void_p, c_int, c_void_p, c_void_p, c_void_p, c_void_p, c_int, c_void_p, c_void_p,
                                          c_int, c_int, c_int, c_int, c_int, c_void_p]),
    "mmgt_gn_silu_conv3x3_unet_stats_rows": (c_int, [c_int, c_int, c_int, c_int]),
    "mmgt_gn_silu_conv3x3_unet_stats": (c_int, [c_void_p, c_int, c_void_p, c_int, c_void_p, c_void_p, c_void_p, c_void_p, c_int, c_void_p, c_void_p, c_void_p,
                                                c_int, c_int, c_int, c_int, c_int, c_void_p]),
    "mmgt_gn_stats_finalize_unet": (c_int, [c_void_p, c_void_p, c_void_p, c_void_p, c_int, c_int, c_int, c_int, c_int, c_float, c_void_p]),
    "mmgt_groupnorm_affine2": (c_int, [c_void_p, c_int, c_void_p, c_int, c_void_p, c_void_p, c_void_p, c_void_p, c_void_p, c_int, c_int, c_int,
                                       c_float, c_int, c_void_p]),
    "mmgt_gn_stats_finalize": (c_int, [c_void_p, c_void_p, c_void_p, c_void_p, c_void_p, c_int, c_int, c_int, c_int, c_float, c_void_p]),
    "mmgt_temporal_leg320_image_bytes": (c_long, []),
    "mmgt_temporal_leg320": (c_int, [c_void_p, c_void_p, c_void_p, c_void_p, c_int, c_void_p, c_void_p, c_int, c_int, c_int, c_float, c_float, c_int,
                                     c_void_p]),
    "mmgt_channel_norm_gelu": (c_int, [c_void_p, c_void_p, c_void_p, c_void_p, c_int, c_int, c_float, c_int, c_void_p]),
    "mmgt_lerp_rows": (c_int, [c_void_p, c_void_p, c_int, c_int, c_int, c_int, c_void_p]),
    "mmgt_relpos_attention": (c_int, [c_void_p, c_long, c_long, c_void_p, c_long, c_long, c_void_p, c_long, c_long, c_void_p, c_long, c_long,
                                      c_void_p, c_long, c_long, c_void_p, c_void_p, c_void_p, c_void_p, c_int, c_int, c_int, c_int, c_float,
                                      c_int, c_void_p]),
    "mmgt_silu": (c_int, [c_void_p, c_void_p, c_long, c_int, c_void_p]),
    "mmgt_cfg_ddim_step": (c_int, [c_void_p, c_void_p, c_void_p, c_void_p, c_long, c_int, c_int, c_float, c_float,
                                   c_float, c_float, c_float, c_void_p]),
    "mmgt_accumulate_window": (c_int, [c_void_p, c_void_p, c_void_p, c_void_p, c_int, c_int, c_int, c_int, c_int, c_int,
                                       c_void_p]),
    "mmgt_rotary": (c_int, [c_void_p, c_void_p, c_void_p, c_long, c_int, c_int, c_int, c_void_p]),
    "mmgt_film_residual": (c_int, [c_void_p, c_void_p, c_long, c_void_p, c_void_p, c_void_p, c_long, c_int, c_int, c_int, c_void_p]),
    "mmgt_mean_tokens": (c_int, [c_void_p, c_void_p, c_int, c_int, c_int, c_int, c_void_p]),
    "mmgt_activation": (c_int, [c_void_p, c_void_p, c_long, c_int, c_int, c_void_p]),
    "mmgt_smga_ddim_step": (c_int, [c_void_p, c_void_p, c_void_p, c_void_p, c_void_p, c_long, c_float, c_float, c_float, c_float,
                                    c_float, c_float, c_int, c_int, c_void_p]),
    "mmgt_blur_mask_u8": (c_int, [c_void_p, c_void_p, c_int, c_int, c_int, c_int, c_void_p]),
    "mmgt_resample_u8": (c_int, [c_void_p, c_void_p, c_void_p, c_int, c_int, c_int, c_void_p, c_void_p, c_int, c_void_p]),
    "mmgt_window_stack": (c_int, [c_void_p, c_void_p, c_int, c_long, c_int, c_void_p]),
    "mmgt_frames_to_u8": (c_int, [c_void_p, c_void_p, c_long, c_int, c_float, c_float, c_int, c_void_p]),
    "mmgt_jpeg_dct_quant": (c_int, [c_void_p, c_void_p, c_int, c_int, c_int, c_int, c_int, c_void_p]),
    "mmgt_jpeg_entropy": (c_int, [c_void_p, c_void_p, c_void_p, c_int, c_int, c_int, c_int, c_long, c_void_p]),
    "mmgt_jpeg_segment_stride": (c_int, [c_int, c_int, ctypes.POINTER(c_long)]),
    "mmgt_jpeg_scan": (c_int, [c_void_p, c_void_p, c_int, c_void_p]),
    "mmgt_jpeg_compact": (c_int, [c_void_p, c_long, c_void_p, c_void_p, c_void_p, ctypes.c_longlong, c_int, c_int, c_void_p]),
# ... 132 lines not shown
            if bias2 is None:
                b2, b2r = None, 0
            elif one_row:
                b2, b2r = bias2[:1], max(m1 - m0, bias2_rows)
            else:
                b2, b2r = bias2[m0 // bias2_rows:(m1 + bias2_rows - 1) // bias2_rows], bias2_rows
            gemm(a[m0:m1], w, bias, out=out[m0:m1], residual=None if residual is None else residual[m0:m1], bias2=b2, bias2_rows=b2r,
                 row_scale=None if row_scale is None else row_scale[m0:m1], alpha=alpha, act=act)
        return out
    _check(lib().mmgt_gemm(_ptr(a), a.stride(0), _ptr(w), _ptr(_f32(bias, "bias")), _ptr(_f32(bias2, "bias2")),
                           bias2_rows, _ptr(_f32(row_scale, "row_scale")), alpha, _ptr(residual),
                           residual.stride(0) if residual is not None else 0, _ptr(out), out.stride(0), M, N, K, act, 1,
                           0, 0, 0, 0, dtype_code(a.dtype), _stream()), "mmgt_gemm")
    return out


def gemm_post(a, w, bias, row_scale, alpha, bias_post, residual, out=None):
    _dev(a, w, bias, row_scale, bias_post, residual, out)
    assert a.dim() == 2 and w.dim() == 2 and a.stride(1) == 1 and w.is_contiguous() and a.dtype == w.dtype
    M, K = a.shape
    N = w.shape[0]
    if out is None:
        out = torch.empty((M, N), device=a.device, dtype=a.dtype)
    assert out.shape == (M, N) and residual.shape == (M, N) and residual.stride(1) == 1 and out.stride(1) == 1
    _check(lib().mmgt_gemm_post(_ptr(a), a.stride(0), _ptr(w), _ptr(_f32(bias, "bias")), _ptr(_f32(row_scale, "row_scale")),
                                alpha, _ptr(_f32(bias_post, "bias_post")), _ptr(residual), residual.stride(0), _ptr(out),
                                out.stride(0), M, N, K, dtype_code(a.dtype), _stream()), "mmgt_gemm_post")
    return out


def gemm_batched_wx(w, x, bias_unused=None, *, out):
    _dev(w, x, out)
    B, ntok, K = x.shape
    R = w.shape[0]
    assert x.is_contiguous() and w.is_contiguous() and out.dim() == 3 and out.shape[0] == B and out.shape[1] == R
    assert out.stride(2) == 1
    _check(lib().mmgt_gemm(_ptr(w), K, _ptr(x), None, None, 0, None, 1.0, None, 0, _ptr(out), out.stride(1), R, ntok, K,
                           ACT_NONE, B, 0, x.stride(0), 0, out.stride(0), dtype_code(x.dtype), _stream()),
           "mmgt_gemm(batched)")
    return out


def gemm_batched(a, w, *, out):
    _dev(a, w, out)
    B, M, K = a.shape
    N = w.shape[1]
    assert a.is_contiguous() and w.is_contiguous() and out.is_contiguous() and w.shape == (B, N, K) and out.shape == (B, M, N)
    _check(lib().mmgt_gemm(_ptr(a), K, _ptr(w), None, None, 0, None, 1.0, None, 0, _ptr(out), N, M, N, K, ACT_NONE, B,
                           M * K, N * K, 0, M * N, dtype_code(a.dtype), _stream()), "mmgt_gemm(batched)")
    return out


def conv3x3(x, wp, bias=None, *, stride=1, upsample=False, bias2=None, bias2_rows=0, residual=None, act=ACT_NONE,
            x1=None, out=None, pad_high_only=False):
    _dev(x, wp, bias, bias2, residual, x1)
    assert x.dim() == 4 and x.is_contiguous() and wp.is_contiguous() and wp.dtype == x.dtype
    NB, IH, IW, C0 = x.shape
    C1 = 0 if x1 is None else x1.shape[3]
    if upsample is not True and upsample == 2:
        assert wp.dim() == 5 and wp.shape[0] == 4 and wp.shape[2:] == (2, 2, C0) and x1 is None and residual is None and bias2 is None
        assert x.dtype == torch.bfloat16 and act == ACT_NONE and stride == 1 and not pad_high_only
        cout = wp.shape[1]
        assert cout % 256 == 0 or cout % 320 == 0
    else:
        upsample = bool(upsample)
        cout = wp.shape[0]
        assert wp.numel() == cout * 9 * (C0 + C1)
    vh, vw = (IH * 2, IW * 2) if upsample else (IH, IW)
    if pad_high_only:
        assert stride == 2 and not upsample
        oh, ow = (vh - 2) // 2 + 1, (vw - 2) // 2 + 1
    else:
        oh, ow = (vh - 1) // stride + 1, (vw - 1) // stride + 1
    if out is None:
        out = torch.empty((NB, oh, ow, cout), device=x.device, dtype=x.dtype)
    assert out.shape == (NB, oh, ow, cout) and out.is_contiguous()
    if residual is not None:
        assert residual.shape == out.shape and residual.is_contiguous()
    lim = DMA_LIMIT
    per_img = max(t.numel() // NB * t.element_size() for t in (x, out, x1, residual) if t is not None)
    if per_img * NB > lim and NB > 1:
        step = max(1, lim // per_img)
        for n0 in range(0, NB, step):
            n1 = min(NB, n0 + step)
            b2, b2r = None, bias2_rows
            if bias2 is not None:
                m0, m1 = n0 * oh * ow, n1 * oh * ow
                if bias2_rows >= NB * oh * ow:
                    b2, b2r = bias2[:1], max(m1 - m0, bias2_rows)
                elif m0 % bias2_rows:
                    raise RuntimeError("conv3x3: a batch split inside a bias2 row group is not supported")
                else:
                    b2 = bias2[m0 // bias2_rows:(m1 + bias2_rows - 1) // bias2_rows]
            conv3x3(x[n0:n1], wp, bias, stride=stride, upsample=upsample, bias2=b2, bias2_rows=b2r,
                    residual=None if residual is None else residual[n0:n1], act=act, x1=None if x1 is None else x1[n0:n1],
                    out=out[n0:n1], pad_high_only=pad_high_only)
        return out
    _check(lib().mmgt_conv3x3_nhwc(_ptr(x), C0, _ptr(x1), C1, NB, IH, IW, -2 if pad_high_only else stride, int(upsample), _ptr(wp),
                                   _ptr(_f32(bias, "bias")), _ptr(_f32(bias2, "bias2")), bias2_rows, _ptr(residual),
                                   _ptr(out), cout, act, dtype_code(x.dtype), _stream()), "mmgt_conv3x3_nhwc")
    return out



def groupnorm(x, gamma, beta, groups, eps, silu=False, x1=None, out=None):
    _dev(x, gamma, beta, x1)
    assert x.dim() == 3 and x.is_contiguous()
    NB, HW, C0 = x.shape
    C1 = 0 if x1 is None else x1.shape[2]
    if x1 is not None:
        assert x1.is_contiguous() and x1.shape[:2] == x.shape[:2] and x1.dtype == x.dtype
    if out is None:
        out = torch.empty((NB, HW, C0 + C1), device=x.device, dtype=x.dtype)
    chunks = lib().mmgt_groupnorm_chunks(HW)
    ws = torch.empty((NB * chunks * groups * 2,), device=x.device, dtype=torch.float32)
    _check(lib().mmgt_groupnorm_nhwc(_ptr(x), C0, _ptr(x1), C1, _ptr(_f32(gamma, "gamma")), _ptr(_f32(beta, "beta")),
                                     _ptr(out), _ptr(ws), NB, HW, groups, eps, int(silu), dtype_code(x.dtype),
                                     _stream()), "mmgt_groupnorm_nhwc")
    return out


def groupnorm_affine(x, gamma, beta, groups, eps, x1=None):
    _dev(x, gamma, beta, x1)
    assert x.dim() == 3 and x.is_contiguous()
    NB, HW, C = x.shape
    C1 = 0
    if x1 is not None:
        assert x1.is_contiguous() and x1.shape[:2] == x.shape[:2] and x1.dtype == x.dtype
        C1 = x1.shape[2]
    chunks = lib().mmgt_groupnorm_chunks(HW)
    ws = torch.empty((NB * chunks * groups * 2,), device=x.device, dtype=torch.float32)
    tab = torch.empty((2, NB, C + C1), device=x.device, dtype=torch.float32)
    scale, shift = tab[0], tab[1]
    _check(lib().mmgt_groupnorm_affine2(_ptr(x), C, _ptr(x1), C1, _ptr(_f32(gamma, "gamma")), _ptr(_f32(beta, "beta")), _ptr(ws), _ptr(scale),
                                        _ptr(shift), NB, HW, groups, eps, dtype_code(x.dtype), _stream()), "mmgt_groupnorm_affine2")
    return scale, shift


def gn_silu_conv3x3_unet_supported(dtype, c0, c1, cout, H, W):
    return dtype == torch.bfloat16 and c0 % 64 == 0 and c1 % 64 == 0 and c0 > 0 and cout % 160 == 0 and H % 16 == 0 and W % 16 == 0


def gn_silu_conv3x3_unet(x, scale, shift, wimg, cout, bias=None, bias2=None, b2_imgs=0, residual=None, x1=None, out=None, next_norm=None):
    _dev(x, scale, shift, wimg, bias, bias2, residual, x1, out)
    assert x.dim() == 4 and x.is_contiguous()
    NB, H, W, C0 = x.shape
    C1 = 0
    if x1 is not None:
        assert x1.is_contiguous() and x1.shape[:3] == x.shape[:3] and x1.dtype == x.dtype
        C1 = x1.shape[3]
    assert gn_silu_conv3x3_unet_supported(x.dtype, C0, C1, cout, H, W)
    C = C0 + C1
    assert scale.shape == (NB, C) and shift.shape == (NB, C) and scale.dtype == torch.float32 and scale.is_contiguous() and shift.is_contiguous()
    assert shift.data_ptr() == scale.data_ptr() + 4 * NB * C, "scale and shift must be the two halves of one allocation (groupnorm_affine)"
    assert wimg.dtype == torch.uint8 and wimg.is_contiguous() and wimg.numel() == lib().mmgt_gn_silu_conv3x3_unet_image_bytes(C, cout)
    if out is None:
        out = torch.empty((NB, H, W, cout), device=x.device, dtype=x.dtype)
    assert out.shape == (NB, H, W, cout) and out.is_contiguous() and out.dtype == x.dtype
    if residual is not None:
        assert residual.shape == out.shape and residual.is_contiguous() and residual.dtype == x.dtype
    if bias2 is not None:
        assert bias2.dim() == 2 and bias2.shape[1] == cout and bias2.is_contiguous() and b2_imgs > 0 and (NB + b2_imgs - 1) // b2_imgs <= bias2.shape[0]
    stats = None
    if next_norm is not None:
        rows = lib().mmgt_gn_silu_conv3x3_unet_stats_rows(NB, H, W, cout)
        assert rows in (2, 4)
        ppi = (H // 16) * (W // 16) * (16 // rows)
        stats = torch.empty((3, NB * ppi, cout), device=x.device, dtype=torch.float32)
    _check(lib().mmgt_gn_silu_conv3x3_unet_stats(_ptr(x), C0, _ptr(x1), C1, _ptr(scale), _ptr(wimg), _ptr(_f32(bias, "bias")), _ptr(_f32(bias2, "bias2")),
                                                 b2_imgs, _ptr(residual), _ptr(out), _ptr(stats), NB, H, W, cout, dtype_code(x.dtype), _stream()),
           "mmgt_gn_silu_conv3x3_unet")
# ... 263 lines not shown

def gemm_bf16_f32(a, w, out=None):
    _dev(a, w, out)
    assert a.dim() == 2 and w.dim() == 2 and a.shape[1] == w.shape[1] and a.stride(1) == 1 and w.stride(1) == 1
    assert a.dtype == torch.bfloat16 and w.dtype == torch.bfloat16
    M, K = a.shape
    N = w.shape[0]
    if out is None:
        out = torch.empty((M, N), device=a.device, dtype=torch.float32)
    assert out.shape == (M, N) and out.dtype == torch.float32 and out.stride(1) == 1
    _check(lib().mmgt_gemm_bf16_f32(_ptr(a), a.stride(0), _ptr(w), w.stride(0), _ptr(out), out.stride(0), M, N, K, _stream()),
           "mmgt_gemm_bf16_f32")
    return out


def qk_split3(qk, bias_q, bias_k):
    _dev(qk, bias_q, bias_k)
    assert qk.dim() == 2 and qk.is_contiguous() and qk.dtype == torch.float32 and qk.shape[1] % 16 == 0
    rows, C = qk.shape[0], qk.shape[1] // 4
    assert bias_q.shape == (C,) and bias_k.shape == (C,) and bias_q.dtype == torch.float32 and bias_k.dtype == torch.float32
    Qp = torch.empty((rows, 3 * C), device=qk.device, dtype=torch.bfloat16)
    Kp = torch.empty((rows, 3 * C), device=qk.device, dtype=torch.bfloat16)
    _check(lib().mmgt_qk_split3(_ptr(qk), _ptr(bias_q), _ptr(bias_k), _ptr(Qp), _ptr(Kp), rows, C, _stream()), "mmgt_qk_split3")
    return Qp, Kp



def ncfhw_to_nhwc(x, cpad, dtype, scale=1.0):
    _dev(x)
    assert x.dim() == 5 and x.dtype == torch.float32 and x.is_contiguous()
    B, C, F, H, W = x.shape
    out = torch.empty((B * F, H, W, cpad), device=x.device, dtype=dtype)
    _check(lib().mmgt_ncfhw_to_nhwc(_ptr(x), _ptr(out), B, C, F, H, W, cpad, scale, dtype_code(dtype), _stream()),
           "mmgt_ncfhw_to_nhwc")
    return out


def nhwc_to_ncfhw(x, B, C, scale=1.0, shift=0.0, clamp01=False):
    _dev(x)
    assert x.dim() == 4 and x.is_contiguous()
    BF, H, W, cpad = x.shape
    F = BF // B
    out = torch.empty((B, C, F, H, W), device=x.device, dtype=torch.float32)
    _check(lib().mmgt_nhwc_to_ncfhw(_ptr(x), _ptr(out), B, C, F, H, W, cpad, scale, shift, int(clamp01),
                                    dtype_code(x.dtype), _stream()),
           "mmgt_nhwc_to_ncfhw")
    return out


def conv1x1_cat_supported(dtype, c0, c1, cout):
    return dtype == torch.bfloat16 and c0 % 64 == 0 and c1 % 64 == 0 and c0 > 0 and c1 > 0 and (cout % 256 == 0 or cout % 320 == 0)


def conv1x1_cat(x0, x1, w, bias=None, residual=None, out=None):
    _dev(x0, x1, w, bias, residual, out)
    assert x0.dim() == 2 and x1.dim() == 2 and x0.shape[0] == x1.shape[0] and x0.is_contiguous() and x1.is_contiguous() and w.is_contiguous()
    rows, c0, c1, cout = x0.shape[0], x0.shape[1], x1.shape[1], w.shape[0]
    assert conv1x1_cat_supported(x0.dtype, c0, c1, cout) and w.shape == (cout, c0 + c1) and w.dtype == x0.dtype == x1.dtype
    if out is None:
        out = torch.empty((rows, cout), device=x0.device, dtype=x0.dtype)
    assert out.shape == (rows, cout) and out.is_contiguous()
    if residual is not None:
        assert residual.shape == out.shape and residual.is_contiguous() and residual.dtype == x0.dtype
    _check(lib().mmgt_conv1x1_cat_nhwc(_ptr(x0), c0, _ptr(x1), c1, rows, _ptr(w), _ptr(_f32(bias, "bias")), _ptr(residual), _ptr(out), cout,
                                       dtype_code(x0.dtype), _stream()), "mmgt_conv1x1_cat_nhwc")
    return out


def conv_taps_gather(y, bias, NB, H, W):
    _dev(y, bias)
    assert y.dim() == 2 and y.shape[0] == NB * H * W and y.shape[1] >= 36 and y.stride(1) == 1 and y.dtype == torch.bfloat16
    out = torch.empty((NB, H, W, 8), device=y.device, dtype=y.dtype)
    _check(lib().mmgt_conv_taps_gather(_ptr(y), y.stride(0), _ptr(_f32(bias, "bias")), _ptr(out), NB, H, W, dtype_code(y.dtype), _stream()),
           "mmgt_conv_taps_gather")
    return out


def timestep_features(timesteps, dim, dtype):
    _dev(timesteps)
    assert timesteps.dtype == torch.float32 and timesteps.dim() == 1
    out = torch.empty((timesteps.shape[0], dim), device=timesteps.device, dtype=dtype)
    _check(lib().mmgt_timestep_features(_ptr(timesteps), _ptr(out), timesteps.shape[0], dim, dtype_code(dtype),
                                        _stream()), "mmgt_timestep_features")
    return out


def silu(x):
    _dev(x)
    assert x.is_contiguous()
    out = torch.empty_like(x)
    _check(lib().mmgt_silu(_ptr(x), _ptr(out), x.numel(), dtype_code(x.dtype), _stream()), "mmgt_silu")
    return out


def cfg_ddim_step(pred_sum, counter, latents, guidance, sa_t, sb_t, sa_p, sb_p):
    _dev(pred_sum, counter, latents)
    assert latents.dtype == torch.float32 and latents.is_contiguous() and pred_sum.is_contiguous()
    _, C, F, H, W = latents.shape
    out = torch.empty_like(latents)
    _check(lib().mmgt_cfg_ddim_step(_ptr(pred_sum), _ptr(_f32(counter, "counter")), _ptr(latents), _ptr(out),
                                    latents.numel(), F, H * W, guidance, sa_t, sb_t, sa_p, sb_p, _stream()),
           "mmgt_cfg_ddim_step")
    return out


def accumulate_window(pred, pred_sum, counter, idx, C, rows=2, row0=0, bump_counter=True):
    _dev(pred, pred_sum, counter, idx)
    assert idx.dtype == torch.int32 and pred.is_contiguous() and pred_sum.is_contiguous()
    Fw = idx.numel()
    F = pred_sum.shape[2]
    hw = pred.shape[1] * pred.shape[2]
    assert pred.shape[0] == rows * Fw and pred_sum.shape[0] == 2 and pred_sum.shape[3] * pred_sum.shape[4] == hw
    _check(lib().mmgt_accumulate_window_rows(_ptr(pred), _ptr(pred_sum), _ptr(counter), _ptr(idx), Fw, F, C, pred.shape[3],
                                             hw, rows, row0, int(bump_counter), dtype_code(pred.dtype), _stream()),
           "mmgt_accumulate_window_rows")

# ... 496 lines not shown
```

### mmgt_amd/reference_unet.py

```python
from typing import Dict

import torch

from . import hip
from .unet3d import UNet3DConditionModel
from .unet3d_spec import unet2d_reference_spec


class UNet2DConditionOutput:
    def __init__(self, sample):
        self.sample = sample


class UNet2DConditionModel(UNet3DConditionModel):
    def __init__(self, device="cuda", dtype=torch.bfloat16, **config):
        super().__init__(device=device, dtype=dtype, **config)
        self.spec = unet2d_reference_spec(self.boc, self.config.cross_attention_dim, self.in_channels,
                                          self.config.layers_per_block)
        self.training = False
        self.bank: Dict[str, torch.Tensor] = {}

    def forward(self, sample, timestep, encoder_hidden_states, return_dict: bool = True, **unused):
        if not self._loaded:
            raise RuntimeError("UNet2DConditionModel.forward before load_state_dict")
        if not sample.is_cuda:
            raise RuntimeError("mmgt_amd.UNet2DConditionModel runs on the GPU only (no CPU path exists)")
        b, _, hh, ww = sample.shape
        lpb = self.config.layers_per_block
        temb = self._time_embedding(timestep, b)
        x = hip.ncfhw_to_nhwc(sample.to(torch.float32)[:, :, None].contiguous(), 64, self._dtype)
        x = hip.conv3x3(x, self.w["conv_in.w"], self.w["conv_in.bias"])
        ehs = encoder_hidden_states.to(self._device)
        bank: Dict[str, torch.Tensor] = {}
        skips = [x]
        for i in range(4):
            p = f"down_blocks.{i}"
            for j in range(lpb):
                x, _ = self._resnet(f"{p}.resnets.{j}", x, temb)
                if i < 3:
                    x = self._spatial_transformer(f"{p}.attentions.{j}", x, ehs, 1, write=bank)
                skips.append(x)
            if i != 3:
                x = hip.conv3x3(x, self.w[f"{p}.downsamplers.0.conv.w"], self.w[f"{p}.downsamplers.0.conv.bias"], stride=2)
                skips.append(x)
        x, _ = self._resnet("mid_block.resnets.0", x, temb)
        mid: Dict[str, torch.Tensor] = {}
        x = self._spatial_transformer("mid_block.attentions.0", x, ehs, 1, write=mid)
        x, _ = self._resnet("mid_block.resnets.1", x, temb)
        for i in range(4):
            p = f"up_blocks.{i}"
            for j in range(lpb + 1):
                x, _ = self._resnet(f"{p}.resnets.{j}", x, temb, skip=skips.pop())
                if i > 0:
                    x = self._spatial_transformer(f"{p}.attentions.{j}", x, ehs, 1, write=bank)
            if i != 3:
                x = self._upsample(f"{p}.upsamplers.0.conv", x)
        bank.update(mid)
        self.bank = bank
        out = hip.nhwc_to_ncfhw(x, b, self.boc[0])[:, :, 0].to(sample.dtype)
        return UNet2DConditionOutput(out) if return_dict else (out,)

    __call__ = forward

    def write_banks(self, latents, timestep, encoder_hidden_states):
        self.forward(latents, timestep, encoder_hidden_states, return_dict=False)
        return self.bank

    def denoise_window(self, *a, **k):
        raise NotImplementedError("ReferenceNet has no denoise step")


class ReferenceAttentionControl:

    def __init__(self, unet, mode="write", do_classifier_free_guidance=False, attention_auto_machine_weight=float("inf"),
                 gn_auto_machine_weight=1.0, style_fidelity=1.0, reference_attn=True, reference_adain=False,
                 fusion_blocks="midup", batch_size=1):
        assert mode in ("read", "write") and fusion_blocks in ("midup", "full")
        if reference_adain:
            raise NotImplementedError("reference_adain is not used by the reference scripts")
        self.unet, self.mode = unet, mode
        self.reference_attn = reference_attn
        self.fusion_blocks = fusion_blocks
        self.do_classifier_free_guidance = do_classifier_free_guidance

    def _modules(self, unet):
        keys = unet.bank_keys()
        if self.fusion_blocks == "midup":
            keys = [k for k in keys if not k.startswith("down_blocks")]
            keys = [k for k in keys if k.startswith("mid_block")] + [k for k in keys if k.startswith("up_blocks")]
        width = lambda k: unet.spec[k + ".transformer_blocks.0.norm1.weight"][0]
        return sorted(keys, key=lambda k: -width(k))

    def update(self, writer, dtype=torch.float16):
        if not self.reference_attn:
            return
        readers, writers = self._modules(self.unet), self._modules(writer.unet)
        banks = {}
        for r, w in zip(readers, writers):
            if w in writer.unet.bank:
                banks[r] = writer.unet.bank[w].to(dtype)
        self.unet.bank_fp16_roundtrip = False
        self.unet.set_banks(banks)

    def clear(self):
        if self.mode == "read":
            self.unet.clear_banks()
        else:
# ... 2 lines not shown
```

### mmgt_amd/unet3d.py

```python
import math
from dataclasses import dataclass
from typing import Dict, List, Optional, Union

import torch

from . import hip
from .packing import pack_conv3x3, pack_conv3x3_up2, pack_conv_taps, pack_ff_fused, pack_ff_proj_out, pack_geglu, pack_rconv, pack_rowgemm, pack_tleg, pad_cols, pad_rows, round_up
from .unet3d_spec import unet3d_spec

SD15_CONFIG = dict(
    in_channels=4, out_channels=4, block_out_channels=(320, 640, 1280, 1280), layers_per_block=2, attention_head_dim=8,
    cross_attention_dim=768, audio_attention_dim=768, norm_num_groups=32, norm_eps=1e-5, center_input_sample=False,
    use_motion_module=True, use_audio_module=True, use_inflated_groupnorm=True,
    motion_module_kwargs=dict(num_attention_heads=8, temporal_position_encoding_max_len=32),
)


@dataclass
class UNet3DConditionOutput:
    sample: torch.Tensor

    def __getitem__(self, i):
        return (self.sample,)[i]


RCONV_LEVEL = {320: 1, 640: 2, 1280: 4}


class _Config(dict):
    __getattr__ = dict.__getitem__


def default_init(spec, seed=0):
    from .synthetic import sinusoid_pe
    g = torch.Generator().manual_seed(seed)
    out = {}
    fan = {}
    for k, shape in spec.items():
        if k.endswith(".weight") and len(shape) > 1:
            f = 1
            for s in shape[1:]:
                f *= s
            fan[k[:-len(".weight")]] = f
    for k, shape in spec.items():
        leaf = k.rsplit(".", 1)[-1]
        base = k[:-len(leaf) - 1]
        if leaf == "pe":
            out[k] = sinusoid_pe(shape[1], shape[2])
        elif any(z in k for z in ("zero_conv_", "temporal_transformer.proj_out")):
            out[k] = torch.zeros(shape)
        elif len(shape) == 1 and base not in fan:
            out[k] = torch.ones(shape) if leaf == "weight" else torch.zeros(shape)
        else:
            bound = 1.0 / math.sqrt(fan.get(base, shape[0]))
            out[k] = (torch.rand(shape, generator=g) * 2 - 1) * bound
    return out


def mask_bias_columns(rs, ncols, dtype):
    cols = torch.zeros((rs.shape[1], ncols), device=rs.device, dtype=dtype)
    rs_hi = rs.to(dtype)
    rs_lo = (rs - rs_hi.float()).to(dtype)
    for i in range(3):
        cols[:, 3 * i], cols[:, 3 * i + 1], cols[:, 3 * i + 2] = rs_hi[i], rs_hi[i], rs_lo[i]
    return cols


def check_group_operands(b, f, hh, ww, c0, dtype, cfg_row=None):
    cols, size = (4 * c0, 4) if dtype == torch.float32 else (round_up(3 * c0 + 9, 64), 2)
    widest = b * f * hh * ww * cols * size
    if widest > hip.DMA_LIMIT and b > (1 if cfg_row is not None else 2):
        raise RuntimeError(f"denoise_window: {b} x {f} frames of {hh} x {ww} latents need a {widest / 2 ** 30:.2f} GiB operand; the kernels address "
                           "2 GiB per tensor (fewer windows per forward: context_batch_size)")


class UNet3DConditionModel:
    _supports_gradient_checkpointing = True

    def __init__(self, device="cuda", dtype=torch.bfloat16, **config):
        cfg = dict(SD15_CONFIG)
        unknown = set(config) - set(cfg) - {"sample_size", "motion_module_type", "motion_module_resolutions",
                                            "motion_module_mid_block", "motion_module_decoder_only",
                                            "unet_use_cross_frame_attention", "unet_use_temporal_attention",
                                            "stack_enable_blocks_name", "stack_enable_blocks_depth", "flip_sin_to_cos",
                                            "freq_shift", "down_block_types", "up_block_types", "mid_block_type",
                                            "act_fn", "downsample_padding", "mid_block_scale_factor", "_class_name",
                                            "only_cross_attention", "dual_cross_attention", "use_linear_projection",
                                            "class_embed_type", "num_class_embeds", "upcast_attention",
                                            "resnet_time_scale_shift", "task_type", "mode", "_diffusers_version"}
        if unknown:
            raise ValueError(f"UNet3DConditionModel: unsupported config keys {sorted(unknown)}")
        cfg.update(config)
        self.config = _Config(cfg)
        boc = tuple(cfg["block_out_channels"])
        if len(boc) != 4 or any(c % 64 for c in boc) or any((c // 8) not in (40, 80, 160) for c in boc):
            raise ValueError(f"block_out_channels {boc}: the HIP kernels cover head dims 40/80/160 (SD-1.5 widths)")
        self.boc = boc
        self.heads = 8
        self.in_channels = cfg["in_channels"]
        self.out_channels = cfg["out_channels"]
        self._device = torch.device(device)
        self._dtype = dtype
        hip.dtype_code(dtype)
        self.training = True
        self.gradient_checkpointing = False
        self._fuse_ff = bool(hip.tune_get("fused_ff"))
        self._twin = bool(hip.tune_get("twin_attention"))
        self._share_rows = bool(hip.tune_get("shared_rows"))
        self._fuse_oz = bool(hip.tune_get("oz3"))
        self._fuse_ln = bool(hip.tune_get("rowgemm"))
        self._ffpo_cat = bool(hip.tune_get("ffpo_cat"))
        self._ffpo = {}
        self._sc_cat = bool(hip.tune_get("sc_cat"))
        self._up2 = bool(hip.tune_get("up2"))
        self._fuse_tleg = bool(hip.tune_get("tleg"))
        self._rconv_stats = bool(hip.tune_get("rconv_stats"))
        self._rconv = hip.tune_get("rconv")
        self.spec = unet3d_spec(boc, cfg["cross_attention_dim"], cfg["audio_attention_dim"], self.in_channels,
                                self.out_channels, cfg["layers_per_block"],
                                cfg["motion_module_kwargs"].get("temporal_position_encoding_max_len", 32))
        self.w: Dict[str, torch.Tensor] = {}
        self._banks: Dict[str, tuple] = {}
        self.bank_fp16_roundtrip = dtype == torch.float32
        self._loaded = False
        self._ehs_cache = None
        self._zbias = {}

    @classmethod
    def from_config(cls, config, **kwargs):
        config = dict(config)
        config.update(kwargs)
        dev = config.pop("device", "cuda")
        dt = config.pop("dtype", torch.bfloat16)
        return cls(device=dev, dtype=dt, **config)

    @classmethod
    def from_pretrained_2d(cls, pretrained_model_path, motion_module_path, subfolder=None, unet_additional_kwargs=None,
                           mm_zero_proj_out=False, device="cuda", dtype=torch.bfloat16):
        import json
        from pathlib import Path
        path = Path(pretrained_model_path)
        if subfolder is not None:
            path = path / subfolder
        cfg_file = path / "config.json"
        if not cfg_file.is_file():
            raise RuntimeError(f"{cfg_file} does not exist or is not a file")
        cfg = json.load(open(cfg_file))
        keep = {k: v for k, v in cfg.items() if k in SD15_CONFIG}
        model = cls(device=device, dtype=dtype, **keep, **{k: v for k, v in (unet_additional_kwargs or {}).items()})
        if (path / "diffusion_pytorch_model.safetensors").exists():
            from safetensors.torch import load_file
            sd = load_file(str(path / "diffusion_pytorch_model.safetensors"), device="cpu")
        elif (path / "diffusion_pytorch_model.bin").exists():
            sd = torch.load(path / "diffusion_pytorch_model.bin", map_location="cpu", weights_only=True)
        else:
            raise FileNotFoundError(f"no weights file found in {path}")
        mpath = Path(motion_module_path)
        if mpath.exists() and mpath.is_file():
            if mpath.suffix.lower() in (".pth", ".pt", ".ckpt"):
                msd = torch.load(mpath, map_location="cpu", weights_only=True)
            elif mpath.suffix.lower() == ".safetensors":
                from safetensors.torch import load_file
                msd = load_file(str(mpath), device="cpu")
            else:
                raise RuntimeError(f"unknown file format for motion module weights: {mpath.suffix}")
            if mm_zero_proj_out:
                msd = {k: v for k, v in msd.items() if "proj_out" not in k}
            sd.update(msd)
        model.load_state_dict(sd, strict=False)
# ... 210 lines not shown
        for p in self._motion:
            q = p + ".temporal_transformer"
            t = q + ".transformer_blocks.0"
            norm(q + ".norm")
            lin(q + ".proj_in")
            proj_in_img(q)
            lin(q + ".proj_out")
            for i in range(2):
                a = f"{t}.attention_blocks.{i}"
                if has(a + ".to_q.weight"):
                    w[a + ".qkv.w"] = self._t(torch.cat([sd[a + ".to_q.weight"], sd[a + ".to_k.weight"],
                                                         sd[a + ".to_v.weight"]], 0))
                    rowimg(a + ".qkv_img", [sd[a + ".to_q.weight"], sd[a + ".to_k.weight"], sd[a + ".to_v.weight"]])
                    if self._fuse_tleg and has(a + ".to_out.0.weight") and has(a + ".to_out.0.bias") and \
                            hip.temporal_leg320_supported(self._dtype, sd[a + ".to_q.weight"].shape[1], self.heads, 24, 4096):
                        w[a + ".tleg_img"] = pack_tleg(*(sd[a + k].to(self._device) for k in (".to_q.weight", ".to_k.weight", ".to_v.weight",
                                                                                               ".to_out.0.weight")))
                lin(a + ".to_out.0", a + ".o")
                if has(a + ".pos_encoder.pe"):
                    w[a + ".pe"] = self._f(sd[a + ".pos_encoder.pe"][0])
                norm(f"{t}.norms.{i}")
                if (a + ".pe") in w and (f"{t}.norms.{i}.b") in w:
                    w[f"{t}.norms.{i}.bpe"] = (w[f"{t}.norms.{i}.b"][None, :] + w[a + ".pe"]).contiguous()
            norm(t + ".ff_norm")
            ff(t + ".ff")

    def bank_keys(self) -> List[str]:
        down = [p for p in self._spatial if p.startswith("down_blocks")]
        up = [p for p in self._spatial if p.startswith("up_blocks")]
        mid = [p for p in self._spatial if p.startswith("mid_block")]
        return down + up + mid

    def set_banks(self, banks: Optional[Dict[str, torch.Tensor]]):
        self._banks = {}
        if not banks:
            return
        for p, bank in banks.items():
            if p not in self._spatial:
                raise KeyError(f"set_banks: {p} is not a reference-attention reader")
            t = p + ".transformer_blocks.0.attn1"
            bk = bank.to(self._device)
            if self.bank_fp16_roundtrip:
                bk = bk.to(torch.float16)
            bk = bk.to(self._dtype).contiguous()
            two, n, c = bk.shape
            kb = hip.gemm(bk.view(two * n, c), self.w[t + ".k.w"]).view(two, n, -1)
            vbt = torch.empty((two, kb.shape[2], round_up(n, 8)), device=self._device, dtype=self._dtype)
            hip.gemm_batched_wx(self.w[t + ".v.w"], bk, out=vbt)
            self._banks[p] = (kb, vbt, n)

    def clear_banks(self):
        self._banks = {}

    def _gn(self, p, x, eps, silu=False, x1=None):
        nb, h, ww, c = x.shape
        y = hip.groupnorm(x.view(nb, h * ww, c), self.w[p + ".g"], self.w[p + ".b"], 32, eps, silu=silu,
                          x1=None if x1 is None else x1.view(nb, h * ww, -1))
        return y.view(nb, h, ww, -1)

    def _ln(self, p, x, **kw):
        return hip.layernorm(x, self.w[p + ".g"], self.w[p + ".b"], 1e-5, **kw)

    def _lin(self, p, x, **kw):
        return hip.gemm(x, self.w[p + ".w"], self.w.get(p + ".bias"), **kw)

    def _ff(self, p, x, residual):
        g = hip.gemm(x, self.w[p + ".ff1.w"], self.w[p + ".ff1.bias"], act=hip.ACT_GEGLU)
        return hip.gemm(g, self.w[p + ".ff2.w"], self.w[p + ".ff2.bias"], residual=residual)

    def _norm_ff(self, p, norm, hid):
        img = self.w.get(p + ".ffimg")
        if img is not None:
            return hip.ff_fused(hid, self.w[norm + ".g"], self.w[norm + ".b"], img, self.w[p + ".ff2.bias"], hid,
                                self.w[p + ".ff2.w"].shape[1])
        return self._ff(p, self._ln(norm, hid), hid)

    def _proj_in_fused(self, p, n):
        return (p + ".proj_in.img") in self.w and n > 256 and n % 128 == 0

    def _norm_proj_in(self, p, x, tables=None):
        nb, h, ww, c = x.shape
        n = h * ww
        if self._proj_in_fused(p, n):
            if tables is not None and tables[0].shape == (nb, c):
                sc, sh = tables
            else:
                sc, sh = hip.groupnorm_affine(x.view(nb, n, c), self.w[p + ".norm.g"], self.w[p + ".norm.b"], 32, 1e-6)
            return hip.rowgemm320(x.view(nb * n, c), self.w[p + ".proj_in.img"], self.w[p + ".proj_in.w"].shape[0], self.w.get(p + ".proj_in.bias"),
                                  pre_scale=sc, pre_shift=sh, pre_rows=n)[0]
        xn = self._gn(p + ".norm", x, 1e-6)
        return self._lin(p + ".proj_in", xn.view(nb * n, c))

    def _norm_ff_proj_out(self, p, norm, hid, q, x_res):
        img, po = self.w.get(p + ".ffimg"), self.w.get(q + ".proj_out.img")
        if img is not None and po is not None and (q + ".proj_out.bias") in self.w:
            return hip.ff_fused_po(hid, self.w[norm + ".g"], self.w[norm + ".b"], img, self.w[p + ".ff2.bias"], hid,
                                   self.w[p + ".ff2.w"].shape[1], po, self.w[q + ".proj_out.bias"], x_res)
        wcat = self._ffpo_weights(p, q) if img is None else None
        if wcat is not None and hid.shape[0] * max(wcat[0].shape[1] - hid.shape[1], hid.shape[1]) * 2 < hip.DMA_LIMIT:
            g = hip.gemm(self._ln(norm, hid), self.w[p + ".ff1.w"], self.w[p + ".ff1.bias"], act=hip.ACT_GEGLU)
            return hip.conv1x1_cat(g, hid, wcat[0], wcat[1], residual=x_res)
        hid = self._norm_ff(p, norm, hid)
        return hip.gemm(hid, self.w[q + ".proj_out.w"], self.w.get(q + ".proj_out.bias"), residual=x_res)

    def _ffpo_weights(self, p, q):
        key = p + ".ffpo"
        if key not in self._ffpo:
            w2, wpo = self.w.get(p + ".ff2.w"), self.w.get(q + ".proj_out.w")
            ok = self._ffpo_cat and w2 is not None and wpo is not None and (p + ".ff2.bias") in self.w and (q + ".proj_out.bias") in self.w and \
                wpo.shape[0] == wpo.shape[1] == w2.shape[0] and hip.conv1x1_cat_supported(self._dtype, w2.shape[1], w2.shape[0], wpo.shape[0])
            if ok:
                wpf = wpo.float()
                wc = torch.cat([wpf @ w2.float(), wpf], 1).to(self._dtype).contiguous()
                bc = (self.w[q + ".proj_out.bias"].float() + wpf @ self.w[p + ".ff2.bias"].float()).contiguous()
                self._ffpo[key] = (wc, bc)
            else:
                self._ffpo[key] = None
        return self._ffpo[key]

    def _resnet(self, p, x, temb, skip=None, out=None, reader=None):
        nb, h, ww, c0 = x.shape
        hw = h * ww
        cout = self.spec[p + ".conv1.weight"][0]
        c1 = 0 if skip is None else skip.shape[3]
        fused = bool(self._rconv & RCONV_LEVEL.get(cout, 0)) and \
            hip.gn_silu_conv3x3_unet_supported(self._dtype, c0, c1, cout, h, ww) and hip.gn_silu_conv3x3_unet_supported(self._dtype, cout, 0, cout, h, ww)
        if fused:
            eps = self.config.norm_eps
            sc, sh = hip.groupnorm_affine(x.view(nb, hw, c0), self.w[p + ".norm1.g"], self.w[p + ".norm1.b"], 32, eps,
                                          x1=None if skip is None else skip.view(nb, hw, c1))
            if self._rconv_stats:
                hdn, (sc, sh) = hip.gn_silu_conv3x3_unet(x, sc, sh, self._rimg(p, ".conv1"), cout, self.w[p + ".conv1.bias"], temb[p], nb // temb[p].shape[0],
                                                         x1=skip, next_norm=(self.w[p + ".norm2.g"], self.w[p + ".norm2.b"], 32, eps))
            else:
                hdn = hip.gn_silu_conv3x3_unet(x, sc, sh, self._rimg(p, ".conv1"), cout, self.w[p + ".conv1.bias"], temb[p], nb // temb[p].shape[0], x1=skip)
                sc, sh = hip.groupnorm_affine(hdn.view(nb, hw, cout), self.w[p + ".norm2.g"], self.w[p + ".norm2.b"], 32, eps)
        else:
            hdn = self._gn(p + ".norm1", x, self.config.norm_eps, silu=True, x1=skip)
            b2rows = (nb // temb[p].shape[0]) * hw
            if temb[p].shape[0] == 1:
                b2rows = max(b2rows, 256)
            hdn = hip.conv3x3(hdn, self.w[p + ".conv1.w"], self.w[p + ".conv1.bias"], bias2=temb[p], bias2_rows=b2rows)
            hdn = self._gn(p + ".norm2", hdn, self.config.norm_eps, silu=True)
        if (p + ".sc.w") in self.w:
            wsc = self.w[p + ".sc.w"]
            if skip is None:
                res = hip.gemm(x.view(nb * hw, c0), wsc, self.w[p + ".sc.bias"])
            else:
                c1 = skip.shape[3]
                if self._sc_cat and nb * hw >= 6144 and hip.conv1x1_cat_supported(self._dtype, c0, c1, cout) and nb * hw * max(c0, c1) * 2 < hip.DMA_LIMIT:
                    res = hip.conv1x1_cat(x.view(nb * hw, c0), skip.view(nb * hw, c1), wsc, self.w[p + ".sc.bias"])
                else:
                    res = hip.gemm(x.view(nb * hw, c0), self._sc_split(p, c0, 0), self.w[p + ".sc.bias"])
                    res = hip.gemm(skip.view(nb * hw, c1), self._sc_split(p, c0, 1), None, residual=res)
            res = res.view(nb, h, ww, cout)
        else:
            assert skip is None
            res = x
        if fused:
            if reader is not None and self._rconv_stats and self._proj_in_fused(reader, hw):
                return hip.gn_silu_conv3x3_unet(hdn, sc, sh, self._rimg(p, ".conv2"), cout, self.w[p + ".conv2.bias"], residual=res, out=out,
                                                next_norm=(self.w[reader + ".norm.g"], self.w[reader + ".norm.b"], 32, 1e-6))
            return hip.gn_silu_conv3x3_unet(hdn, sc, sh, self._rimg(p, ".conv2"), cout, self.w[p + ".conv2.bias"], residual=res, out=out), None
        return hip.conv3x3(hdn, self.w[p + ".conv2.w"], self.w[p + ".conv2.bias"], residual=res, out=out), None

    def _rimg(self, p, cv):
        key = p + cv + ".rimg"
        if key not in self.w:
            self.w[key] = pack_rconv(self.w[p + cv + ".w"].permute(0, 3, 1, 2))
        return self.w[key]

    def _upsample(self, p, x):
        w2 = self.w.get(p + ".w2")
        if w2 is not None:
            return hip.conv3x3(x, w2, self.w[p + ".bias"], upsample=2)
        return hip.conv3x3(x, self.w[p + ".w"], self.w[p + ".bias"], upsample=True)

    def _sc_split(self, p, c0, which):
        key = f"{p}.sc.w.{which}"
        if key not in self.w:
            wsc = self.w[p + ".sc.w"]
            self.w[f"{p}.sc.w.0"] = wsc[:, :c0].contiguous()
            self.w[f"{p}.sc.w.1"] = wsc[:, c0:].contiguous()
        return self.w[key]

    def _self_attention(self, t, n1, nb, n, inner, bank=None, frames=1, cfg_row=None, norm=None):
        hd = inner // self.heads
        npad = round_up(n, 8)
        vt = torch.empty((nb, inner, npad), device=self._device, dtype=self._dtype)
        if norm is not None:
            qk, _ = hip.rowgemm320(n1, self.w[t + ".qkv_img"], 3 * inner, ln_gamma=self.w[norm + ".g"], ln_beta=self.w[norm + ".b"],
                                   n1=2 * inner, n_tok=n, out_t=vt)
        else:
            qk = hip.gemm(n1, self.w[t + ".qk.w"])
            hip.gemm_batched_wx(self.w[t + ".v.w"], n1.view(nb, n, inner), out=vt)
        o = torch.empty((nb * n, inner), device=self._device, dtype=self._dtype)
        kw = {}
        if bank is not None and cfg_row != 0:
            kb, vbt, nkb = bank
            if cfg_row == 1:
                kb, vbt = kb[1:], vbt[1:]
            kw = dict(k2=kb, v2=vbt, k2_str=(kb.stride(0), kb.stride(1)), v2_str=(vbt.stride(0), vbt.stride(1)),
                      k2_bdiv=nb if cfg_row == 1 else nb // 2, nk2=nkb, seg2_first_batch=0 if cfg_row == 1 else nb // 2)
        hip.attention(qk, qk[:, inner:], vt, o, batch=nb, heads=self.heads, hd=hd, nq=n, nk=n, scale=hd ** -0.5,
                      q_str=(n * 2 * inner, 0, 2 * inner), k_str=(n * 2 * inner, 0, 2 * inner),
                      v_str=(inner * npad, 0, npad), o_str=(n * inner, 0, inner), v_transposed=True, **kw)
        return o

    def _spatial_transformer(self, p, x, ehs, frames, write=None, cfg_row=None, tables=None):
        nb, h, ww, c = x.shape
        n = h * ww
        m = nb * n
        t = p + ".transformer_blocks.0"
        hid = self._norm_proj_in(p, x, tables)
        inner = hid.shape[1]
        fuse = write is None and (t + ".attn1.qkv_img") in self.w and n % 128 == 0
        n1 = hid if fuse else self._ln(t + ".norm1", hid)
        if write is not None:
            write[p] = n1.view(nb, n, inner).float()
        o = self._self_attention(t + ".attn1", n1, nb, n, inner, bank=None if write is not None else self._banks.get(p),
                                 frames=frames, cfg_row=cfg_row, norm=t + ".norm1" if fuse else None)
        if ehs.shape[1] == 1:
            cvec = self._clip_vector(t, ehs)
            if cfg_row is not None:
                cvec = cvec[cfg_row:cfg_row + 1]
            rows = nb // cvec.shape[0] * n if cvec.shape[0] != nb else n
            hid = hip.gemm(o, self.w[t + ".attn1.o.w"], self.w[t + ".attn1.o.bias"], residual=hid,
                           bias2=cvec, bias2_rows=rows)
        else:
            hid = hip.gemm(o, self.w[t + ".attn1.o.w"], self.w[t + ".attn1.o.bias"], residual=hid)
            hid = self._cross_attention(t, hid, ehs if cfg_row is None else ehs[cfg_row:cfg_row + 1], nb, n, inner)
        out = self._norm_ff_proj_out(t + ".ff", t + ".norm3", hid, p, x.view(m, c))
        return out.view(nb, h, ww, c)

    def _spatial_transformer_twin(self, p, x2, ehs, frames, tables=None):
        nb, h, ww, c = x2.shape
        f, n = nb // 2, h * ww
        t = p + ".transformer_blocks.0"
        bank = self._banks.get(p)
        inner = self.w[t + ".attn1.o.w"].shape[1]
        hd = inner // self.heads
        if bank is None or (t + ".attn1.qkv_img") not in self.w or ehs.shape[1] != 1 or self._dtype != torch.bfloat16 or hd != 40 \
                or n % 256 or bank[2] % 64 or nb % 2:
            return None
        hid = self._norm_proj_in(p, x2[:f], tables)
        npad = round_up(n, 8)
        vt = torch.empty((f, inner, npad), device=self._device, dtype=self._dtype)
        qk, _ = hip.rowgemm320(hid, self.w[t + ".attn1.qkv_img"], 3 * inner, ln_gamma=self.w[t + ".norm1.g"], ln_beta=self.w[t + ".norm1.b"],
                               n1=2 * inner, n_tok=n, out_t=vt)
        kb, vbt, nkb = bank
        kb, vbt = kb[1:], vbt[1:]
        o = torch.empty((nb * n, inner), device=self._device, dtype=self._dtype)
        hip.attention(qk, qk[:, inner:], vt, o[f * n:], batch=f, heads=self.heads, hd=hd, nq=n, nk=n, scale=hd ** -0.5,
                      q_str=(n * 2 * inner, 0, 2 * inner), k_str=(n * 2 * inner, 0, 2 * inner), v_str=(inner * npad, 0, npad),
                      o_str=(n * inner, 0, inner), v_transposed=True, k2=kb, v2=vbt, k2_str=(kb.stride(0), kb.stride(1)),
                      v2_str=(vbt.stride(0), vbt.stride(1)), k2_bdiv=f, nk2=nkb, seg2_first_batch=0, twin_out=o[:f * n])
        cvec = self._clip_vector(t, ehs)
        hid2 = torch.empty((nb * n, inner), device=self._device, dtype=self._dtype)
        for row in (0, 1):
            sl = slice(row * f * n, (row + 1) * f * n)
            hip.gemm(o[sl], self.w[t + ".attn1.o.w"], self.w[t + ".attn1.o.bias"], residual=hid, bias2=cvec[row:row + 1],
                     bias2_rows=max(f * n, 256), out=hid2[sl])
        out = self._norm_ff_proj_out(t + ".ff", t + ".norm3", hid2, p, x2.view(nb * n, c))
        return out.view(nb, h, ww, c)

    def _clip_vector(self, t, ehs):
        c = self._ehs_cache
        if c is None or c[0] is not ehs or c[1] != ehs._version:
            c = self._ehs_cache = (ehs, ehs._version, {})
        if t not in c[2]:
            e = ehs.reshape(ehs.shape[0], -1).to(self._dtype).contiguous()
            c[2][t] = hip.gemm(hip.gemm(e, self.w[t + ".attn2.v.w"]), self.w[t + ".attn2.o.w"],
                               self.w[t + ".attn2.o.bias"]).float()
        return c[2][t]

    def _cross_attention(self, t, hid, ehs, nb, n, inner):
        hd = inner // self.heads
        n2 = self._ln(t + ".norm2", hid)
        q = hip.gemm(n2, self.w[t + ".attn2.q.w"])
        e = ehs.to(self._dtype)
        if e.shape[0] != nb:
            e = e.repeat_interleave(nb // e.shape[0], dim=0)
        e = e.contiguous()
        l = e.shape[1]
        kv = hip.gemm(e.view(nb * l, -1), self.w[t + ".attn2.kv.w"])
        o = torch.empty_like(q)
        hip.attention(q, kv, kv[:, inner:], o, batch=nb, heads=self.heads, hd=hd, nq=n, nk=l, scale=hd ** -0.5,
                      q_str=(n * inner, 0, inner), k_str=(l * 2 * inner, 0, 2 * inner), v_str=(l * 2 * inner, 0, 2 * inner),
                      o_str=(n * inner, 0, inner))
        return hip.gemm(o, self.w[t + ".attn2.o.w"], self.w[t + ".attn2.o.bias"], residual=hid)

    def _audio_transformer(self, p, x, audio, masks, depth, motion_scale, ms_cache=None):
        nb, h, ww, c = x.shape
        n = h * ww
        m = nb * n
        t = p + ".transformer_blocks.0"
        hid = self._norm_proj_in(p, x)
        inner = hid.shape[1]
        hd = inner // self.heads
        if (t + ".attn1.qkv_img") in self.w and n % 128 == 0:
            o = self._self_attention(t + ".attn1", hid, nb, n, inner, norm=t + ".norm1")
        else:
            o = self._self_attention(t + ".attn1", self._ln(t + ".norm1", hid), nb, n, inner)
        hid = hip.gemm(o, self.w[t + ".attn1.o.w"], self.w[t + ".attn1.o.bias"], residual=hid)
        la = audio.shape[1]
        state = ms_cache.get("state") if ms_cache is not None else None
        fused = self._fuse_oz and (t + ".oz3.w") in self.w and ms_cache is not None
        nb0 = min(nb, ms_cache.get("zero_images", 0)) if fused else 0
        m0 = nb0 * n
        q3 = kv3 = None
        if nb0 < nb:
            hid_c = hid[m0:]
            if (t + ".q3_img") in self.w:
                q3, _ = hip.rowgemm320(hid_c, self.w[t + ".q3_img"], 3 * inner, ln_gamma=self.w[t + ".norm2.g"], ln_beta=self.w[t + ".norm2.b"])
            else:
                q3 = hip.gemm(self._ln(t + ".norm2", hid_c), self.w[t + ".q3.w"])
            kv3 = state.get(("kv3", t, nb0)) if state is not None else None
            if kv3 is None:
                kv3 = hip.gemm(audio[nb0:].reshape((nb - nb0) * la, -1), self.w[t + ".kv3.w"])
                if state is not None:
                    state[("kv3", t, nb0)] = kv3
        scales = tuple(1.0 if motion_scale is None else float(motion_scale[i]) for i in range(3))
        if fused:
            k3 = 3 * inner
            kp = self.w[t + ".oz3.w"].shape[1]
            ck = (depth, k3)
            if ck not in ms_cache:
                kept = state.get(("mask_rows", depth, kp - k3, scales)) if state is not None else None
                if kept is None:
                    rows = []
                    for i in range(3):
                        mask = masks[i][depth].reshape(-1).to(device=self._device, dtype=torch.float32)
                        if mask.numel() != m:
                            raise RuntimeError(f"mask level {depth} has {mask.numel()} entries, block has {m} tokens")
                        rows.append(mask if scales[i] == 1.0 else mask * scales[i])
                    rs = torch.stack(rows).contiguous()
                    cols = mask_bias_columns(rs, kp - k3, self._dtype)
                    kept = (rs, cols)
                    if state is not None:
                        state[("mask_rows", depth, kp - k3, scales)] = kept
                rs, cols = kept
                buf = torch.empty((m, kp), device=self._device, dtype=self._dtype)
                buf[:, k3:] = cols
                if m0:
                    buf[:m0, :k3] = 0
                ms_cache[ck] = (rs, buf)
            rs, a3 = ms_cache[ck]
            if nb0 < nb:
                hip.attention(q3, kv3, kv3[:, k3:], a3[m0:], batch=nb - nb0, heads=3 * self.heads, hd=hd, nq=n, nk=la, scale=hd ** -0.5,
                              q_str=(n * k3, 0, k3), k_str=(la * 2 * k3, 0, 2 * k3), v_str=(la * 2 * k3, 0, 2 * k3), o_str=(n * kp, 0, kp),
                              out_scale=rs[:, m0:], out_scale_heads=self.heads)
            key = (t + ".zsum", scales)
            if key not in self._zbias:
                self._zbias[key] = sum(self.w[f"{t}.z{i}.bias"] * scales[i] for i in range(3)).contiguous()
            if 0 < m0 < m:
                out = torch.empty_like(hid)
                hip.gemm(a3[:m0, k3:], self.w[t + ".oz3.wb"], self._zbias[key], residual=hid[:m0], out=out[:m0])
                hip.gemm(a3[m0:], self.w[t + ".oz3.w"], self._zbias[key], residual=hid[m0:], out=out[m0:])
                hid = out
            elif m0 == m:
                hid = hip.gemm(a3[:, k3:], self.w[t + ".oz3.wb"], self._zbias[key], residual=hid)
            else:
                hid = hip.gemm(a3, self.w[t + ".oz3.w"], self._zbias[key], residual=hid)
        else:
            a3 = torch.empty_like(q3)
            hip.attention(q3, kv3, kv3[:, 3 * inner:], a3, batch=nb, heads=3 * self.heads, hd=hd, nq=n, nk=la,
                          scale=hd ** -0.5, q_str=(n * 3 * inner, 0, 3 * inner), k_str=(la * 6 * inner, 0, 6 * inner),
                          v_str=(la * 6 * inner, 0, 6 * inner), o_str=(n * 3 * inner, 0, 3 * inner))
            for i in range(3):
                mask = masks[i][depth].reshape(-1).to(device=self._device, dtype=torch.float32).contiguous()
                if mask.numel() != m:
                    raise RuntimeError(f"mask level {depth} has {mask.numel()} entries, block has {m} tokens")
                s = scales[i]
                key = (f"{t}.z{i}", s)
                if key not in self._zbias:
                    self._zbias[key] = (self.w[f"{t}.z{i}.bias"] * s).contiguous()
                hid = hip.gemm_post(a3[:, i * inner:(i + 1) * inner], self.w[f"{t}.oz{i}.w"], self.w[f"{t}.oz{i}.bias"], mask, s,
                                    self._zbias[key], hid)
        out = self._norm_ff_proj_out(t + ".ff", t + ".norm3", hid, p, x.view(m, c))
        return out.view(nb, h, ww, c)

    def _motion_module(self, p, x, frames):
        nb, h, ww, c = x.shape
        n = h * ww
        m = nb * n
        b = nb // frames
        hd = c // self.heads
        if frames > 32:
            raise RuntimeError("temporal attention window is limited to 32 frames (positional encoding max_len)")
        q = p + ".temporal_transformer"
        t = q + ".transformer_blocks.0"
        hid = self._norm_proj_in(q, x)
        for i in range(2):
            a = f"{t}.attention_blocks.{i}"
            if (a + ".tleg_img") in self.w and (f"{t}.norms.{i}.bpe") in self.w and hip.temporal_leg320_supported(self._dtype, c, self.heads, frames, n, b):
                hid = hip.temporal_leg320(hid, self.w[f"{t}.norms.{i}.g"], self.w[f"{t}.norms.{i}.bpe"], self.w[a + ".tleg_img"], self.w[a + ".o.bias"],
                                          b, frames, n, hd ** -0.5)
                continue
            if (a + ".qkv_img") in self.w and n % 128 == 0:
                qkv, _ = hip.rowgemm320(hid, self.w[a + ".qkv_img"], 3 * c, ln_gamma=self.w[f"{t}.norms.{i}.g"],
                                        ln_beta=self.w[f"{t}.norms.{i}.bpe"], pe_div=n, pe_mod=frames)
            else:
                nrm = hip.layernorm(hid, self.w[f"{t}.norms.{i}.g"], self.w[f"{t}.norms.{i}.bpe"], 1e-5, pe_div=n, pe_mod=frames)
                qkv = hip.gemm(nrm, self.w[a + ".qkv.w"])
            o = torch.empty((m, c), device=self._device, dtype=self._dtype)
            st = (frames * n * 3 * c, 3 * c, n * 3 * c)
            hip.attention(qkv, qkv[:, c:], qkv[:, 2 * c:], o, batch=b * n, heads=self.heads, hd=hd, nq=frames, nk=frames,
                          scale=hd ** -0.5, q_str=st, k_str=st, v_str=st, o_str=(frames * n * c, c, n * c), bdiv=n)
            hid = hip.gemm(o, self.w[a + ".o.w"], self.w[a + ".o.bias"], residual=hid)
        out = self._norm_ff_proj_out(t + ".ff", t + ".ff_norm", hid, q, x.view(m, c))
        return out.view(nb, h, ww, c)

    def _time_embedding(self, timestep, batch):
        if not torch.is_tensor(timestep):
            ts = torch.tensor([float(timestep)], dtype=torch.float32, device=self._device)
        else:
            ts = timestep.to(device=self._device, dtype=torch.float32).reshape(-1)
        if ts.numel() == 1:
            batch = 1
        ts = ts.expand(batch).contiguous()
        feat = hip.timestep_features(ts, self.boc[0], self._dtype)
        e = self._lin("time_embedding.linear_1", feat, act=hip.ACT_SILU)
        e = self._lin("time_embedding.linear_2", e)
        all_t = hip.gemm(hip.silu(e), self.w["temb_all.w"], self.w["temb_all.bias"]).float()
        return {p: all_t[:, off:off + n].contiguous() for p, (off, n) in self._temb_slices.items()}

    def forward(self, sample, timestep, encoder_hidden_states, audio_embedding=None, class_labels=None,
                mask_cond_fea=None, pose_cond_fea=None, attention_mask=None, full_mask=None, face_mask=None,
                body_mask=None, motion_scale=None, down_block_additional_residuals=None,
                mid_block_additional_residual=None, return_dict: bool = True):
        if attention_mask is not None or class_labels is not None or down_block_additional_residuals is not None \
                or mid_block_additional_residual is not None:
            raise NotImplementedError("attention_mask / class_labels / additional residuals are not used on this path")
        x = self.denoise_window(sample, timestep, encoder_hidden_states, audio_embedding, pose_cond_fea, full_mask,
                                face_mask, body_mask, motion_scale)
        out = hip.nhwc_to_ncfhw(x, sample.shape[0], self.out_channels).to(sample.dtype)
        if not return_dict:
            return (out,)
        return UNet3DConditionOutput(sample=out)

    __call__ = forward

    def denoise_window(self, sample, timestep, encoder_hidden_states, audio_embedding=None, pose_cond_fea=None,
                       full_mask=None, face_mask=None, body_mask=None, motion_scale=None, cfg_row=None, window_state=None,
                       audio_zero_rows=0, cfg_rows_share_input=False):
        if cfg_row is not None and (cfg_row not in (0, 1) or encoder_hidden_states.shape[0] != 2):
            raise RuntimeError("cfg_row: one CFG row (0 or 1) with the (2, ...) encoder_hidden_states pair")
        if cfg_row is None and (sample.shape[0] % 2 or encoder_hidden_states.shape[0] != 2):
            raise RuntimeError(f"denoise_window: {sample.shape[0]} batch rows with {encoder_hidden_states.shape[0]} encoder_hidden_states rows: the "
                               "batch is the CFG pair of one or more windows, [uncond w0 .. uncond w(B-1), cond w0 .. cond w(B-1)], or one row with cfg_row")
        if not self._loaded:
            raise RuntimeError("UNet3DConditionModel.forward before load_state_dict")
        if not sample.is_cuda:
            raise RuntimeError("mmgt_amd.UNet3DConditionModel runs on the GPU only (no CPU path exists)")
        b, cin, f, hh, ww = sample.shape
        if hh % 8 or ww % 8:
            raise RuntimeError("latent height/width must be multiples of 8 (unet_3d.py:461-469)")
        check_group_operands(b, f, hh, ww, self.boc[0], self._dtype, cfg_row)
        lpb = self.config.layers_per_block
        ms = motion_scale if (self.training and self.gradient_checkpointing) else None
        x_in = sample.to(torch.float32).contiguous()
        if self.config.center_input_sample:
            x_in = 2 * x_in - 1.0
        temb = self._time_embedding(timestep, b)
        x = hip.ncfhw_to_nhwc(x_in, 64, self._dtype)
        pose = None
        if pose_cond_fea is not None:
            if pose_cond_fea.dim() == 4:
                pose = pose_cond_fea.to(self._dtype).contiguous()
            else:
                pose = hip.ncfhw_to_nhwc(pose_cond_fea.to(torch.float32).contiguous(), self.boc[0], self._dtype)
        shared = bool(cfg_rows_share_input) and b >= 2 and cfg_row is None and self._share_rows
        hf = b // 2 * f
        if shared:
            x2 = torch.empty((2 * hf, hh, ww, self.boc[0]), device=self._device, dtype=self._dtype)
            x = hip.conv3x3(x[:hf], self.w["conv_in.w"], self.w["conv_in.bias"], residual=None if pose is None else pose[:hf], out=x2[:hf])
            x2[hf:].copy_(x)
        else:
            x = hip.conv3x3(x, self.w["conv_in.w"], self.w["conv_in.bias"], residual=pose)
        audio = None
        if audio_embedding is not None:
            audio = audio_embedding.to(device=self._device, dtype=self._dtype).reshape(b * f, *audio_embedding.shape[2:])
            audio = audio.contiguous()
        masks = (full_mask, face_mask, body_mask)
        if not 0 <= int(audio_zero_rows) <= b:
            raise RuntimeError(f"audio_zero_rows = {audio_zero_rows} outside 0..{b}")
        ms_cache = {"state": window_state, "zero_images": int(audio_zero_rows) * f}
        ehs = encoder_hidden_states.to(self._device)

        skips = [x2 if shared else x]
        for i in range(4):
            p = f"down_blocks.{i}"
            for j in range(lpb):
                if shared and i == 0 and j == 0:
                    r = f"{p}.resnets.0"
                    x2 = torch.empty((2 * hf,) + tuple(x.shape[1:3]) + (self.spec[r + ".conv1.weight"][0],), device=self._device, dtype=self._dtype)
                    x, tab = self._resnet(r, x, {r: temb[r][:1]}, out=x2[:hf], reader=f"{p}.attentions.0" if self._twin else None)
                    x2[hf:].copy_(x)
                    x = x2
                else:
                    x, tab = self._resnet(f"{p}.resnets.{j}", x, temb, reader=f"{p}.attentions.{j}" if i < 3 else None)
                if i < 3:
                    y = self._spatial_transformer_twin(f"{p}.attentions.{j}", x, ehs, f, tab) if (shared and i == 0 and j == 0 and self._twin) else None
                    x = y if y is not None else self._spatial_transformer(f"{p}.attentions.{j}", x, ehs, f, cfg_row=cfg_row, tables=tab)
                    if f"{p}.audio_modules.{j}" in self._audio:
                        x = self._audio_transformer(f"{p}.audio_modules.{j}", x, audio, masks, i, ms, ms_cache)
                x = self._motion_module(f"{p}.motion_modules.{j}", x, f)
                skips.append(x)
            if i != 3:
                x = hip.conv3x3(x, self.w[f"{p}.downsamplers.0.conv.w"], self.w[f"{p}.downsamplers.0.conv.bias"], stride=2)
                skips.append(x)

        x, _ = self._resnet("mid_block.resnets.0", x, temb)
        x = self._spatial_transformer("mid_block.attentions.0", x, ehs, f, cfg_row=cfg_row)
        x = self._motion_module("mid_block.motion_modules.0", x, f)
        x, _ = self._resnet("mid_block.resnets.1", x, temb)

        for i in range(4):
            p = f"up_blocks.{i}"
            for j in range(lpb + 1):
                x, tab = self._resnet(f"{p}.resnets.{j}", x, temb, skip=skips.pop(), reader=f"{p}.attentions.{j}" if i > 0 else None)
                if i > 0:
                    x = self._spatial_transformer(f"{p}.attentions.{j}", x, ehs, f, cfg_row=cfg_row, tables=tab)
                x = self._motion_module(f"{p}.motion_modules.{j}", x, f)
            if i != 3:
                x = self._upsample(f"{p}.upsamplers.0.conv", x)

        timg = self.w.get("conv_out.timg")
        nb, h, ww, c = x.shape
        if timg is not None and c == 320 and (h * ww) % 128 == 0:
            sc, sh = hip.groupnorm_affine(x.view(nb, h * ww, c), self.w["conv_norm_out.g"], self.w["conv_norm_out.b"], 32, self.config.norm_eps)
            y, _ = hip.rowgemm320(x.view(nb * h * ww, c), timg, 64, pre_scale=sc, pre_shift=sh, pre_rows=h * ww, pre_silu=True)
            return hip.conv_taps_gather(y, self.w["conv_out.bias"], nb, h, ww)
        x = self._gn("conv_norm_out", x, self.config.norm_eps, silu=True)
        x = hip.conv3x3(x, self.w["conv_out.w"], self.w["conv_out.bias"])
        return x
```

Baseline: 14.91 steps/s.

## Fuse next block's GroupNorm into split-K reduction of conv/proj-out outputs

Adds norm-fused variants of conv3x3 and conv1x1_cat. When split-K is used, they compute the following block's GroupNorm (optionally with SiLU) directly from the fp32 partial sums while reducing, instead of running a separate reduce kernel and then a separate norm pass. The Python UNet forward threads next_norm/tables through the resnets, transformers, motion modules and downsamplers so each stage can consume the pre-normalized output. The aim is to cut a full read/write pass and kernel launches per block. In exchange it adds complexity, relies on fallback paths when the shapes don't match, and drops a zeroing step in the audio cache buffer.

```diff
diff --git a/include/mmgt_hip.h b/include/mmgt_hip.h
--- a/include/mmgt_hip.h
+++ b/include/mmgt_hip.h
@@ -38,6 +38,13 @@
 
 int mmgt_conv1x1_cat_nhwc(const void* x0, int C0, const void* x1, int C1, long rows, const void* Wp, const float* bias, const void* residual, void* out,
                           int Cout, int dtype, void* stream);
+
+int mmgt_conv3x3_norm_nhwc(const void* x0, int C0, const void* x1, int C1, int NB, int IH, int IW, int stride, int upsample, const void* Wp,
+                           const float* bias, const float* bias2, int bias2_rows, const void* residual, void* out, int Cout, int act, int dtype,
+                           const float* gamma, const float* beta, int groups, float eps, int silu, int keep_raw, void* out_norm, int* fused, void* stream);
+int mmgt_conv1x1_cat_norm_nhwc(const void* x0, int C0, const void* x1, int C1, long rows, int HW, const void* Wp, const float* bias, const void* residual,
+                               void* out, int Cout, int dtype, const float* gamma, const float* beta, int groups, float eps, int silu, int keep_raw,
+                               void* out_norm, int* fused, void* stream);
 
 int mmgt_conv_taps_gather(const void* Y, int ldY, const float* bias, void* out, int NB, int H, int W, int dtype, void* stream);
 
diff --git a/mmgt_amd/csrc/common.h b/mmgt_amd/csrc/common.h
--- a/mmgt_amd/csrc/common.h
+++ b/mmgt_amd/csrc/common.h
@@ -137,6 +137,78 @@
   return v;
 }
 
+struct SplitkSrc {
+  const float* part; int S; long slab;
+  const float* bias; const float* bias2; int b2rows;
+  const bf16_t* res; long ldr;
+  int N, m0;
+};
+#ifndef MMGT_SPLITK_ZB
+#define MMGT_SPLITK_ZB(NV) ((NV) <= 2 ? 4 : (NV) <= 6 ? 2 : 1)
+#endif
+template <int NV>
+__device__ __forceinline__ void splitk_reduce_vecs(const SplitkSrc& k, const int (&m)[NV], int c, u32x4 (&out)[NV]) {
+  constexpr int ZB = MMGT_SPLITK_ZB(NV);
+  u32x4 rv[NV];
+  if (k.res) {
+#pragma unroll
+    for (int i = 0; i < NV; ++i) rv[i] = *reinterpret_cast<const u32x4*>(k.res + (long)m[i] * k.ldr + c);
+  }
+  f32x4 a0[NV], a1[NV];
+  for (int z0 = 0; z0 < k.S; z0 += ZB) {
+    f32x4 t0[ZB][NV], t1[ZB][NV];
+#pragma unroll
+    for (int j = 0; j < ZB; ++j) {
+      const long zo = (long)min(z0 + j, k.S - 1) * k.slab + c;
+#pragma unroll
+      for (int i = 0; i < NV; ++i) {
+        const float* p = k.part + (long)m[i] * k.N + zo;
+        t0[j][i] = *reinterpret_cast<const f32x4*>(p);
+        t1[j][i] = *reinterpret_cast<const f32x4*>(p + 4);
+      }
+    }
+#pragma unroll
+    for (int j = 0; j < ZB; ++j) {
+      if (z0 + j >= k.S) continue;
+      if (j == 0 && z0 == 0) {
+#pragma unroll
+        for (int i = 0; i < NV; ++i) { a0[i] = t0[0][i]; a1[i] = t1[0][i]; }
+      } else {
+#pragma unroll
+        for (int i = 0; i < NV; ++i) { a0[i] += t0[j][i]; a1[i] += t1[j][i]; }
+      }
+    }
+  }
+  if (k.bias) {
+    const f32x4 b0 = *reinterpret_cast<const f32x4*>(k.bias + c), b1 = *reinterpret_cast<const f32x4*>(k.bias + c + 4);
+#pragma unroll
+    for (int i = 0; i < NV; ++i) { a0[i] += b0; a1[i] += b1; }
+  }
+  if (k.bias2) {
+#pragma unroll
+    for (int i = 0; i < NV; ++i) {
+      const float* b2 = k.bias2 + (long)((m[i] + k.m0) / k.b2rows) * k.N + c;
+      a0[i] += *reinterpret_cast<const f32x4*>(b2);
+      a1[i] += *reinterpret_cast<const f32x4*>(b2 + 4);
+    }
+  }
+  if (k.res) {
+#pragma unroll
+    for (int i = 0; i < NV; ++i) {
+      union { u32x4 u; bf16_t e[8]; } r8;
+      r8.u = rv[i];
+#pragma unroll
+      for (int e = 0; e < 4; ++e) { a0[i][e] += bf16_to_f32(r8.e[e]); a1[i][e] += bf16_to_f32(r8.e[4 + e]); }
+    }
+  }
+#pragma unroll
+  for (int i = 0; i < NV; ++i)
+    out[i] = (u32x4){pack_bf16x2(a0[i][0], a0[i][1]), pack_bf16x2(a0[i][2], a0[i][3]), pack_bf16x2(a1[i][0], a1[i][1]), pack_bf16x2(a1[i][2], a1[i][3])};
+}
+struct NextNorm {
+  const float* gamma; const float* beta; int G; float eps; int silu; int HW; void* out; int keep_raw; int fused;
+};
+
 #ifdef __cplusplus
 extern "C" {
 #endif
diff --git a/mmgt_amd/csrc/gemm.hip b/mmgt_amd/csrc/gemm.hip
--- a/mmgt_amd/csrc/gemm.hip
+++ b/mmgt_amd/csrc/gemm.hip
@@ -636,11 +636,11 @@
 }
 int mmgt_gemm16_launch(int mode, int bn, const void* ad, const void* W, long bsw, const void* ep, int M, int N, int K,
                        int batch, void* stream);
-int mmgt_gemm16_splitk(int mode, int bn, const void* ad, const void* W, const void* ep, int M, int N, int K, int S, void* stream, int m0);
+int mmgt_gemm16_splitk(int mode, int bn, const void* ad, const void* W, const void* ep, int M, int N, int K, int S, void* stream, int m0, NextNorm* nn);
 namespace {
 
 template <typename T, int MODE>
-int launch(const ADesc& ad, const void* W, long bsw, const Epi& ep, int M, int N, int K, int batch, hipStream_t s) {
+int launch(const ADesc& ad, const void* W, long bsw, const Epi& ep, int M, int N, int K, int batch, hipStream_t s, NextNorm* nn = nullptr) {
   const bool geglu = ep.act == 1;
   int cfg = g_gemm_cfg;
   if ((cfg == 0 || cfg == 18) && g_splitk && std::is_same<T, bf16_t>::value && batch == 1 && ep.act == 0 && ep.fast && !ep.row_scale &&
@@ -652,7 +652,7 @@
     int S = 0;
     for (int c = 8; c >= 2; --c)
       if (tiles * c <= 256 && nch % c == 0 && nch / c >= (tiles <= 64 ? 16 : 64)) { S = c; break; }
-    if (S >= 2 && tiles <= 128 && (MODE == 1 || tiles <= 32 || tiles > 64)) return mmgt_gemm16_splitk(MODE, bn, &ad, W, &ep, M, N, K, S, s, 0);
+    if (S >= 2 && tiles <= 128 && (MODE == 1 || tiles <= 32 || tiles > 64)) return mmgt_gemm16_splitk(MODE, bn, &ad, W, &ep, M, N, K, S, s, 0, nn);
   }
   if (cfg == 18) cfg = 0;
   if (cfg == 0) {
@@ -710,7 +710,7 @@
           }
           if (ep.residual) epb.residual = ep.residual + rows_a * ep.ldr * esz;
           epb.out = ep.out + rows_a * ep.ldo * esz;
-          return mmgt_gemm16_splitk(MODE, bnc, &adb, W, &epb, (int)(M - rows_a), N, K, 2, s, (int)rows_a);
+          return mmgt_gemm16_splitk(MODE, bnc, &adb, W, &epb, (int)(M - rows_a), N, K, 2, s, (int)rows_a, nullptr);
         }
       }
       return mmgt_gemm16_launch(MODE, bn, &ad, W, bsw, &ep, M, N, K, batch, s);
@@ -807,7 +807,13 @@
     {"zero_audio_skip", 1},
     {"window_state", 1},
     {"smga_graph", 1},
+    {"reduce_norm", 1},
 };
+int host_switch(const char* key) {
+  for (const HostSwitch& h : g_host)
+    if (!strcmp(key, h.key)) return h.value;
+  return 0;
+}
 }
 extern "C" int mmgt_tune_get(const char* key, int* value) {
   if (key && value)
@@ -942,9 +948,9 @@
                     0, dtype, stream);
 }
 
-extern "C" int mmgt_conv3x3_nhwc(const void* x0, int C0, const void* x1, int C1, int NB, int IH, int IW, int stride,
-                                 int upsample, const void* Wp, const float* bias, const float* bias2, int bias2_rows,
-                                 const void* residual, void* out, int Cout, int act, int dtype, void* stream) {
+static int conv3x3_entry(const void* x0, int C0, const void* x1, int C1, int NB, int IH, int IW, int stride,
+                         int upsample, const void* Wp, const float* bias, const float* bias2, int bias2_rows,
+                         const void* residual, void* out, int Cout, int act, int dtype, void* stream, NextNorm* nn) {
   MMGT_CHECK(x0 && Wp && out, "conv3x3: null pointer");
   int pad_lo = 1;
   if (stride == -2) { stride = 2; pad_lo = 0; }
@@ -981,12 +987,36 @@
   ep.fast = epi_fast(ep, Cout, Cout, dtype == MMGT_BF16 ? 2 : 4);
   hipStream_t s = (hipStream_t)stream;
   if (up2) return launch<bf16_t, 1>(ad, Wp, (long)Cout * K, ep, (int)M, Cout, K, 4, s);
-  return dtype == MMGT_BF16 ? launch<bf16_t, 1>(ad, Wp, 0, ep, (int)M, Cout, K, 1, s)
+  if (nn) nn->HW = OH * OW;
+  return dtype == MMGT_BF16 ? launch<bf16_t, 1>(ad, Wp, 0, ep, (int)M, Cout, K, 1, s, nn)
                             : launch<float, 1>(ad, Wp, 0, ep, (int)M, Cout, K, 1, s);
 }
 
-extern "C" int mmgt_conv1x1_cat_nhwc(const void* x0, int C0, const void* x1, int C1, long rows, const void* Wp, const float* bias, const void* residual,
-                                     void* out, int Cout, int dtype, void* stream) {
+extern "C" int mmgt_conv3x3_nhwc(const void* x0, int C0, const void* x1, int C1, int NB, int IH, int IW, int stride,
+                                 int upsample, const void* Wp, const float* bias, const float* bias2, int bias2_rows,
+                                 const void* residual, void* out, int Cout, int act, int dtype, void* stream) {
+  return conv3x3_entry(x0, C0, x1, C1, NB, IH, IW, stride, upsample, Wp, bias, bias2, bias2_rows, residual, out, Cout, act, dtype, stream, nullptr);
+}
+
+static NextNorm next_norm(const float* gamma, const float* beta, int groups, float eps, int silu, int keep_raw, void* out_norm) {
+  return NextNorm{gamma, beta, groups, eps, silu, 0, out_norm, keep_raw, 0};
+}
+extern "C" int mmgt_conv3x3_norm_nhwc(const void* x0, int C0, const void* x1, int C1, int NB, int IH, int IW, int stride, int upsample, const void* Wp,
+                                      const float* bias, const float* bias2, int bias2_rows, const void* residual, void* out, int Cout, int act, int dtype,
+                                      const float* gamma, const float* beta, int groups, float eps, int silu, int keep_raw, void* out_norm, int* fused,
+                                      void* stream) {
+  MMGT_CHECK(gamma && beta && out_norm && fused && groups > 0, "conv3x3_norm: null pointer");
+  MMGT_CHECK(((uintptr_t)out_norm % 16) == 0, "conv3x3_norm: out_norm must be 16-byte aligned");
+  NextNorm nn = next_norm(gamma, beta, groups, eps, silu, keep_raw, out_norm);
+  *fused = 0;
+  const int rc = conv3x3_entry(x0, C0, x1, C1, NB, IH, IW, stride, upsample, Wp, bias, bias2, bias2_rows, residual, out, Cout, act, dtype, stream,
+                               host_switch("reduce_norm") ? &nn : nullptr);
+  if (rc == 0) *fused = nn.fused;
+  return rc;
+}
+
+static int conv1x1_cat_entry(const void* x0, int C0, const void* x1, int C1, long rows, const void* Wp, const float* bias, const void* residual,
+                             void* out, int Cout, int dtype, void* stream, NextNorm* nn) {
   MMGT_CHECK(x0 && x1 && Wp && out && rows > 0, "conv1x1_cat: null pointer");
   MMGT_CHECK(dtype == MMGT_BF16, "conv1x1_cat: bf16 only");
   MMGT_CHECK(C0 > 0 && C1 > 0 && C0 % 64 == 0 && C1 % 64 == 0 && (Cout % 256 == 0 || Cout % 320 == 0), "conv1x1_cat: C0 = %d, C1 = %d must be multiples of 64, Cout = %d of 256 or 320",
@@ -1003,5 +1033,23 @@
   Epi ep{};
   ep.bias = bias; ep.alpha = 1.f; ep.residual = (const char*)residual; ep.ldr = Cout; ep.out = (char*)out; ep.ldo = Cout;
   ep.fast = epi_fast(ep, Cout, Cout, 2);
-  return launch<bf16_t, 1>(ad, Wp, 0, ep, (int)rows, Cout, K, 1, (hipStream_t)stream);
-}
+  return launch<bf16_t, 1>(ad, Wp, 0, ep, (int)rows, Cout, K, 1, (hipStream_t)stream, nn);
+}
+
+extern "C" int mmgt_conv1x1_cat_nhwc(const void* x0, int C0, const void* x1, int C1, long rows, const void* Wp, const float* bias, const void* residual,
+                                     void* out, int Cout, int dtype, void* stream) {
+  return conv1x1_cat_entry(x0, C0, x1, C1, rows, Wp, bias, residual, out, Cout, dtype, stream, nullptr);
+}
+
+extern "C" int mmgt_conv1x1_cat_norm_nhwc(const void* x0, int C0, const void* x1, int C1, long rows, int HW, const void* Wp, const float* bias, const void* residual,
+                                          void* out, int Cout, int dtype, const float* gamma, const float* beta, int groups, float eps, int silu, int keep_raw,
+                                          void* out_norm, int* fused, void* stream) {
+  MMGT_CHECK(gamma && beta && out_norm && fused && groups > 0 && HW > 0, "conv1x1_cat_norm: null pointer");
+  MMGT_CHECK(((uintptr_t)out_norm % 16) == 0, "conv1x1_cat_norm: out_norm must be 16-byte aligned");
+  NextNorm nn = next_norm(gamma, beta, groups, eps, silu, keep_raw, out_norm);
+  nn.HW = HW;
+  *fused = 0;
+  const int rc = conv1x1_cat_entry(x0, C0, x1, C1, rows, Wp, bias, residual, out, Cout, dtype, stream, host_switch("reduce_norm") ? &nn : nullptr);
+  if (rc == 0) *fused = nn.fused;
+  return rc;
+}
diff --git a/mmgt_amd/csrc/gemm16.hip b/mmgt_amd/csrc/gemm16.hip
--- a/mmgt_amd/csrc/gemm16.hip
+++ b/mmgt_amd/csrc/gemm16.hip
@@ -494,33 +494,15 @@
 
 namespace {
 
-__global__ __launch_bounds__(256) void splitk_reduce_kernel(const float* __restrict__ part, int S, long slab, const float* __restrict__ bias,
-                                                            const float* __restrict__ bias2, int b2rows, const bf16_t* __restrict__ res,
-                                                            long ldr, bf16_t* __restrict__ out, long ldo, int M, int N, int m0) {
-  const int nv = N / 8;
+__global__ __launch_bounds__(256) void splitk_reduce_kernel(SplitkSrc k, bf16_t* __restrict__ out, long ldo, int M) {
+  const int nv = k.N / 8;
   const long idx = (long)blockIdx.x * 256 + threadIdx.x;
   if (idx >= (long)M * nv) return;
   const int m = (int)(idx / nv), c = (int)(idx - (long)m * nv) * 8;
-  const float* p = part + (long)m * N + c;
-  f32x4 a0 = *reinterpret_cast<const f32x4*>(p), a1 = *reinterpret_cast<const f32x4*>(p + 4);
-  for (int z = 1; z < S; ++z) {
-    a0 += *reinterpret_cast<const f32x4*>(p + z * slab);
-    a1 += *reinterpret_cast<const f32x4*>(p + z * slab + 4);
-  }
-  if (bias) { a0 += *reinterpret_cast<const f32x4*>(bias + c); a1 += *reinterpret_cast<const f32x4*>(bias + c + 4); }
-  if (bias2) {
-    const float* b2 = bias2 + (long)((m + m0) / b2rows) * N + c;
-    a0 += *reinterpret_cast<const f32x4*>(b2);
-    a1 += *reinterpret_cast<const f32x4*>(b2 + 4);
-  }
-  if (res) {
-    union { u32x4 u; bf16_t e[8]; } r8;
-    r8.u = *reinterpret_cast<const u32x4*>(res + (long)m * ldr + c);
-#pragma unroll
-    for (int e = 0; e < 4; ++e) { a0[e] += bf16_to_f32(r8.e[e]); a1[e] += bf16_to_f32(r8.e[4 + e]); }
-  }
-  *reinterpret_cast<u32x4*>(out + (long)m * ldo + c) =
-      (u32x4){pack_bf16x2(a0[0], a0[1]), pack_bf16x2(a0[2], a0[3]), pack_bf16x2(a1[0], a1[1]), pack_bf16x2(a1[2], a1[3])};
+  const int rows[1] = {m};
+  u32x4 v[1];
+  splitk_reduce_vecs<1>(k, rows, c, v);
+  *reinterpret_cast<u32x4*>(out + (long)m * ldo + c) = v[0];
 }
 
 constexpr int MAX_DEV = 16, MAX_RETIRED = 8;
@@ -576,7 +558,8 @@
 
 }
 
-int mmgt_gemm16_splitk(int mode, int bn, const void* adp, const void* W, const void* epp, int M, int N, int K, int S, void* stream, int m0) {
+int mmgt_gn_slab_from_partials(const SplitkSrc* k, int M, const NextNorm* nn, void* raw_out, hipStream_t s);
+int mmgt_gemm16_splitk(int mode, int bn, const void* adp, const void* W, const void* epp, int M, int N, int K, int S, void* stream, int m0, NextNorm* nn) {
   ADesc ad = *reinterpret_cast<const ADesc*>(adp);
   const Epi& ep = *reinterpret_cast<const Epi*>(epp);
   hipStream_t s = (hipStream_t)stream;
@@ -596,9 +579,16 @@
   if (bn == 320) rc = mode == 0 ? launch16<0, 320>(ad, W, 0, pe, M, N, ks, S, s) : launch16<1, 320>(ad, W, 0, pe, M, N, ks, S, s);
   else rc = mode == 0 ? launch16<0, 256>(ad, W, 0, pe, M, N, ks, S, s) : launch16<1, 256>(ad, W, 0, pe, M, N, ks, S, s);
   if (rc) return rc;
+  SplitkSrc k{ws, S, (long)M * N, ep.bias, ep.bias2, ep.bias2 ? ep.bias2_rows : 1, reinterpret_cast<const bf16_t*>(ep.residual), ep.ldr, N, m0};
+  if (nn && m0 == 0 && nn->HW > 0 && M % nn->HW == 0 && ep.ldo == N) {
+    rc = mmgt_gn_slab_from_partials(&k, M, nn, nn->keep_raw ? ep.out : nullptr, s);
+    if (rc >= 0) {
+      nn->fused = rc == 0;
+      return rc;
+    }
+  }
   const long nthr = (long)M * (N / 8);
-  hipLaunchKernelGGL(splitk_reduce_kernel, dim3((unsigned)((nthr + 255) / 256)), dim3(256), 0, s, ws, S, (long)M * N, ep.bias, ep.bias2,
-                     ep.bias2 ? ep.bias2_rows : 1, reinterpret_cast<const bf16_t*>(ep.residual), ep.ldr, reinterpret_cast<bf16_t*>(ep.out), ep.ldo, M, N, m0);
+  hipLaunchKernelGGL(splitk_reduce_kernel, dim3((unsigned)((nthr + 255) / 256)), dim3(256), 0, s, k, reinterpret_cast<bf16_t*>(ep.out), ep.ldo, M);
   MMGT_LAUNCH_CHECK();
   return 0;
 }
diff --git a/mmgt_amd/csrc/norm.hip b/mmgt_amd/csrc/norm.hip
--- a/mmgt_amd/csrc/norm.hip
+++ b/mmgt_amd/csrc/norm.hip
@@ -441,16 +441,42 @@
   }
 }
 
-template <typename T, int NR, int NTHR = 256>
-__global__ __launch_bounds__(NTHR) void gn_slab_kernel(const T* __restrict__ x0, int C0, const T* __restrict__ x1, int C1,
-                                                      const float* __restrict__ gamma, const float* __restrict__ beta,
+template <typename T>
+struct SlabFromTensor {
+  const T* x0; int C0; const T* x1; int C1;
+  __device__ int channels() const { return C0 + C1; }
+  template <int NR>
+  __device__ void load(int n, int HW, const int (&r)[NR], int c, u32x4 (&raw)[NR]) const {
+    const T* src = c < C0 ? x0 + (long)n * HW * C0 + c : x1 + (long)n * HW * C1 + (c - C0);
+    const long rstride = c < C0 ? C0 : C1;
+#pragma unroll
+    for (int i = 0; i < NR; ++i) raw[i] = r[i] < HW ? *reinterpret_cast<const u32x4*>(src + r[i] * rstride) : (u32x4)(0u);
+  }
+  __device__ void keep(int, int, int, int, const u32x4&) const {}
+};
+struct SlabFromPartials {
+  SplitkSrc k; bf16_t* keep_out;
+  __device__ int channels() const { return k.N; }
+  template <int NR>
+  __device__ void load(int n, int HW, const int (&r)[NR], int c, u32x4 (&raw)[NR]) const {
+    int m[NR];
+#pragma unroll
+    for (int i = 0; i < NR; ++i) m[i] = n * HW + min(r[i], HW - 1);
+    splitk_reduce_vecs<NR>(k, m, c, raw);
+  }
+  __device__ void keep(int n, int HW, int r, int c, const u32x4& v) const {
+    if (keep_out) *reinterpret_cast<u32x4*>(keep_out + ((long)n * HW + r) * k.N + c) = v;
+  }
+};
+template <typename T, int NR, int NTHR = 256, class SRC = SlabFromTensor<T>>
+__global__ __launch_bounds__(NTHR) void gn_slab_kernel(SRC src, const float* __restrict__ gamma, const float* __restrict__ beta,
                                                       T* __restrict__ out, int HW, int G, int gpw, float eps, int silu,
                                                       float* __restrict__ tscale, float* __restrict__ tshift) {
   constexpr int VEC = VecIO<T>::VEC;
   __shared__ float part[NTHR * VEC];
   __shared__ float chan[320];
   __shared__ float gstat[2][4];
-  const int C = C0 + C1, cg = C / G, cw = gpw * cg, nvw = cw / VEC;
+  const int C = src.channels(), cg = C / G, cw = gpw * cg, nvw = cw / VEC;
   int n = blockIdx.y, sl = blockIdx.x;
   {
     const int nsl = gridDim.x, tot = nsl * gridDim.y;
@@ -466,17 +492,22 @@
   const int vc = tid % nvw, r0 = tid / nvw;
   const bool active = r0 < rp;
   const int c = c_lo + vc * VEC;
-  const T* src = c < C0 ? x0 + (long)n * HW * C0 + c : x1 + (long)n * HW * C1 + (c - C0);
-  const long rstride = c < C0 ? C0 : C1;
   int gid[VEC];
 #pragma unroll
   for (int e = 0; e < VEC; ++e) gid[e] = (vc * VEC + e) / cg;
 
   u32x4 raw[NR];
+  if (active) {
+    int rows[NR];
+#pragma unroll
+    for (int i = 0; i < NR; ++i) rows[i] = r0 + i * rp;
+    src.template load<NR>(n, HW, rows, c, raw);
+  }
 #pragma unroll
   for (int i = 0; i < NR; ++i) {
     const int r = r0 + i * rp;
-    raw[i] = (active && r < HW) ? *reinterpret_cast<const u32x4*>(src + r * rstride) : (u32x4)(0u);
+    if (active && r < HW) src.keep(n, HW, r, c, raw[i]);
+    else raw[i] = (u32x4)(0u);
   }
   auto dec = [](const u32x4& u, float* f) {
     union { u32x4 u; T e[VEC]; } v;
@@ -590,8 +621,8 @@
 template <typename T>
 void gn_slab_launch(int nr, int nthr, dim3 grid, hipStream_t s, const void* x0, int C0, const void* x1, int C1, const float* gamma, const float* beta, void* out,
                     int HW, int G, int gpw, float eps, int silu, float* tscale, float* tshift) {
-#define GN_SLAB(NR_, NT_) hipLaunchKernelGGL((gn_slab_kernel<T, NR_, NT_>), grid, dim3(NT_), 0, s, (const T*)x0, C0, (const T*)x1, C1, gamma, beta, (T*)out, HW, G, gpw, \
-                                             eps, silu, tscale, tshift)
+  const SlabFromTensor<T> src{(const T*)x0, C0, (const T*)x1, C1};
+#define GN_SLAB(NR_, NT_) hipLaunchKernelGGL((gn_slab_kernel<T, NR_, NT_>), grid, dim3(NT_), 0, s, src, gamma, beta, (T*)out, HW, G, gpw, eps, silu, tscale, tshift)
   if (nthr == 1024) GN_SLAB(16, 1024);
   else if (nr == 2) GN_SLAB(2, 256); else if (nr == 4) GN_SLAB(4, 256); else if (nr == 6) GN_SLAB(6, 256); else if (nr == 12) GN_SLAB(12, 256); else GN_SLAB(22, 256);
 #undef GN_SLAB
@@ -655,6 +686,22 @@
   }
 }
 
+}
+
+int mmgt_gn_slab_from_partials(const SplitkSrc* k, int M, const NextNorm* nn, void* raw_out, hipStream_t s) {
+  const int N = k->N, HW = nn->HW, NB = M / HW;
+  if (!g_gn_slab || !nn->gamma || !nn->beta || !nn->out || nn->G <= 0 || nn->G > 64 || N % nn->G || N > GN_MAXC || N % 8 || NB <= 0 || NB > 65535) return -1;
+  int nr = 0, nthr = 256;
+  const int gpw = gn_slab_gpw(N, nn->G, HW, 8, &nr, &nthr);
+  if (!gpw || nthr != 256) return -1;
+  const SlabFromPartials src{*k, (bf16_t*)raw_out};
+  dim3 grid(nn->G / gpw, NB);
+#define GN_SLAB_P(NR_) hipLaunchKernelGGL((gn_slab_kernel<bf16_t, NR_, 256, SlabFromPartials>), grid, dim3(256), 0, s, src, nn->gamma, nn->beta, (bf16_t*)nn->out, HW, \
+                                          nn->G, gpw, nn->eps, nn->silu, (float*)nullptr, (float*)nullptr)
+  if (nr == 2) GN_SLAB_P(2); else if (nr == 4) GN_SLAB_P(4); else if (nr == 6) GN_SLAB_P(6); else if (nr == 12) GN_SLAB_P(12); else GN_SLAB_P(22);
+#undef GN_SLAB_P
+  MMGT_LAUNCH_CHECK();
+  return 0;
 }
 
 void mmgt_gn_set_rows(int v) { g_gn_rows = v; }
diff --git a/mmgt_amd/hip.py b/mmgt_amd/hip.py
--- a/mmgt_amd/hip.py
+++ b/mmgt_amd/hip.py
@@ -52,6 +52,11 @@
     "mmgt_nhwc_to_ncfhw": (c_int, [c_void_p, c_void_p, c_int, c_int, c_int, c_int, c_int, c_int, c_float, c_float, c_int,
                                    c_int, c_void_p]),
     "mmgt_conv1x1_cat_nhwc": (c_int, [c_void_p, c_int, c_void_p, c_int, c_long, c_void_p, c_void_p, c_void_p, c_void_p, c_int, c_int, c_void_p]),
+    "mmgt_conv3x3_norm_nhwc": (c_int, [c_void_p, c_int, c_void_p, c_int, c_int, c_int, c_int, c_int, c_int, c_void_p, c_void_p, c_void_p, c_int, c_void_p,
+                                       c_void_p, c_int, c_int, c_int, c_void_p, c_void_p, c_int, c_float, c_int, c_int, c_void_p, ctypes.POINTER(c_int),
+                                       c_void_p]),
+    "mmgt_conv1x1_cat_norm_nhwc": (c_int, [c_void_p, c_int, c_void_p, c_int, c_long, c_int, c_void_p, c_void_p, c_void_p, c_void_p, c_int, c_int, c_void_p,
+                                           c_void_p, c_int, c_float, c_int, c_int, c_void_p, ctypes.POINTER(c_int), c_void_p]),
     "mmgt_conv_taps_gather": (c_int, [c_void_p, c_int, c_void_p, c_void_p, c_int, c_int, c_int, c_int, c_void_p]),
     "mmgt_timestep_features": (c_int, [c_void_p, c_void_p, c_int, c_int, c_int, c_void_p]),
     "mmgt_ff_fused_image_bytes": (c_int, [c_int, c_int]),
@@ -290,7 +295,7 @@
 
 
 def conv3x3(x, wp, bias=None, *, stride=1, upsample=False, bias2=None, bias2_rows=0, residual=None, act=ACT_NONE,
-            x1=None, out=None, pad_high_only=False):
+            x1=None, out=None, pad_high_only=False, next_norm=None, norm_out=None):
     _dev(x, wp, bias, bias2, residual, x1)
     assert x.dim() == 4 and x.is_contiguous() and wp.is_contiguous() and wp.dtype == x.dtype
     NB, IH, IW, C0 = x.shape
@@ -319,6 +324,9 @@
     per_img = max(t.numel() // NB * t.element_size() for t in (x, out, x1, residual) if t is not None)
     if per_img * NB > lim and NB > 1:
         step = max(1, lim // per_img)
+        if next_norm is not None:
+            return conv3x3(x, wp, bias, stride=stride, upsample=upsample, bias2=bias2, bias2_rows=bias2_rows, residual=residual, act=act, x1=x1, out=out,
+                           pad_high_only=pad_high_only), None
         for n0 in range(0, NB, step):
             n1 = min(NB, n0 + step)
             b2, b2r = None, bias2_rows
@@ -334,6 +342,19 @@
                     residual=None if residual is None else residual[n0:n1], act=act, x1=None if x1 is None else x1[n0:n1],
                     out=out[n0:n1], pad_high_only=pad_high_only)
         return out
+    if next_norm is not None:
+        gamma, beta, groups, eps, silu, keep_raw = next_norm
+        _dev(gamma, beta)
+        yn = torch.empty_like(out) if norm_out is None else norm_out
+        assert yn.shape == out.shape and yn.is_contiguous() and yn.dtype == out.dtype
+        fused = c_int(0)
+        _check(lib().mmgt_conv3x3_norm_nhwc(_ptr(x), C0, _ptr(x1), C1, NB, IH, IW, -2 if pad_high_only else stride, int(upsample), _ptr(wp),
+                                            _ptr(_f32(bias, "bias")), _ptr(_f32(bias2, "bias2")), bias2_rows, _ptr(residual), _ptr(out), cout, act,
+                                            dtype_code(x.dtype), _ptr(_f32(gamma, "gamma")), _ptr(_f32(beta, "beta")), groups, eps, int(silu), int(keep_raw),
+                                            _ptr(yn), ctypes.byref(fused), _stream()), "mmgt_conv3x3_norm_nhwc")
+        if not fused.value:
+            return out, None
+        return (out if keep_raw else None), yn
     _check(lib().mmgt_conv3x3_nhwc(_ptr(x), C0, _ptr(x1), C1, NB, IH, IW, -2 if pad_high_only else stride, int(upsample), _ptr(wp),
                                    _ptr(_f32(bias, "bias")), _ptr(_f32(bias2, "bias2")), bias2_rows, _ptr(residual),
                                    _ptr(out), cout, act, dtype_code(x.dtype), _stream()), "mmgt_conv3x3_nhwc")
@@ -355,6 +376,8 @@
     _check(lib().mmgt_groupnorm_nhwc(_ptr(x), C0, _ptr(x1), C1, _ptr(_f32(gamma, "gamma")), _ptr(_f32(beta, "beta")),
                                      _ptr(out), _ptr(ws), NB, HW, groups, eps, int(silu), dtype_code(x.dtype),
                                      _stream()), "mmgt_groupnorm_nhwc")
+    key = f"groupnorm hw={HW} sources={1 if x1 is None else 2}"
+    _calls[key] = _calls.get(key, 0) + 1
     return out
 
 
@@ -724,7 +747,7 @@
     return dtype == torch.bfloat16 and c0 % 64 == 0 and c1 % 64 == 0 and c0 > 0 and c1 > 0 and (cout % 256 == 0 or cout % 320 == 0)
 
 
-def conv1x1_cat(x0, x1, w, bias=None, residual=None, out=None):
+def conv1x1_cat(x0, x1, w, bias=None, residual=None, out=None, next_norm=None, hw=0, norm_out=None):
     _dev(x0, x1, w, bias, residual, out)
     assert x0.dim() == 2 and x1.dim() == 2 and x0.shape[0] == x1.shape[0] and x0.is_contiguous() and x1.is_contiguous() and w.is_contiguous()
     rows, c0, c1, cout = x0.shape[0], x0.shape[1], x1.shape[1], w.shape[0]
@@ -734,6 +757,19 @@
     assert out.shape == (rows, cout) and out.is_contiguous()
     if residual is not None:
         assert residual.shape == out.shape and residual.is_contiguous() and residual.dtype == x0.dtype
+    if next_norm is not None:
+        gamma, beta, groups, eps, silu, keep_raw = next_norm
+        _dev(gamma, beta)
+        assert hw > 0
+        yn = torch.empty_like(out) if norm_out is None else norm_out
+        assert yn.shape == out.shape and yn.is_contiguous() and yn.dtype == out.dtype
+        fused = c_int(0)
+        _check(lib().mmgt_conv1x1_cat_norm_nhwc(_ptr(x0), c0, _ptr(x1), c1, rows, hw, _ptr(w), _ptr(_f32(bias, "bias")), _ptr(residual), _ptr(out), cout,
+                                                dtype_code(x0.dtype), _ptr(_f32(gamma, "gamma")), _ptr(_f32(beta, "beta")), groups, eps, int(silu),
+                                                int(keep_raw), _ptr(yn), ctypes.byref(fused), _stream()), "mmgt_conv1x1_cat_norm_nhwc")
+        if not fused.value:
+            return out, None
+        return (out if keep_raw else None), yn
     _check(lib().mmgt_conv1x1_cat_nhwc(_ptr(x0), c0, _ptr(x1), c1, rows, _ptr(w), _ptr(_f32(bias, "bias")), _ptr(residual), _ptr(out), cout,
                                        dtype_code(x0.dtype), _stream()), "mmgt_conv1x1_cat_nhwc")
     return out
diff --git a/mmgt_amd/reference_unet.py b/mmgt_amd/reference_unet.py
--- a/mmgt_amd/reference_unet.py
+++ b/mmgt_amd/reference_unet.py
@@ -38,21 +38,21 @@
             for j in range(lpb):
                 x, _ = self._resnet(f"{p}.resnets.{j}", x, temb)
                 if i < 3:
-                    x = self._spatial_transformer(f"{p}.attentions.{j}", x, ehs, 1, write=bank)
+                    x, _ = self._spatial_transformer(f"{p}.attentions.{j}", x, ehs, 1, write=bank)
                 skips.append(x)
             if i != 3:
                 x = hip.conv3x3(x, self.w[f"{p}.downsamplers.0.conv.w"], self.w[f"{p}.downsamplers.0.conv.bias"], stride=2)
                 skips.append(x)
         x, _ = self._resnet("mid_block.resnets.0", x, temb)
         mid: Dict[str, torch.Tensor] = {}
-        x = self._spatial_transformer("mid_block.attentions.0", x, ehs, 1, write=mid)
+        x, _ = self._spatial_transformer("mid_block.attentions.0", x, ehs, 1, write=mid)
         x, _ = self._resnet("mid_block.resnets.1", x, temb)
         for i in range(4):
             p = f"up_blocks.{i}"
             for j in range(lpb + 1):
                 x, _ = self._resnet(f"{p}.resnets.{j}", x, temb, skip=skips.pop())
                 if i > 0:
-                    x = self._spatial_transformer(f"{p}.attentions.{j}", x, ehs, 1, write=bank)
+                    x, _ = self._spatial_transformer(f"{p}.attentions.{j}", x, ehs, 1, write=bank)
             if i != 3:
                 x = self._upsample(f"{p}.upsamplers.0.conv", x)
         bank.update(mid)
diff --git a/mmgt_amd/unet3d.py b/mmgt_amd/unet3d.py
--- a/mmgt_amd/unet3d.py
+++ b/mmgt_amd/unet3d.py
@@ -1,6 +1,6 @@
 import math
 from dataclasses import dataclass
-from typing import Dict, List, Optional, Union
+from typing import Dict, List, NamedTuple, Optional, Union
 
 import torch
 
@@ -25,6 +25,11 @@
 
 
 RCONV_LEVEL = {320: 1, 640: 2, 1280: 4}
+
+
+class Normed(NamedTuple):
+    key: tuple
+    y: torch.Tensor
 
 
 class _Config(dict):
@@ -115,6 +120,7 @@
         self._up2 = bool(hip.tune_get("up2"))
         self._fuse_tleg = bool(hip.tune_get("tleg"))
         self._rconv_stats = bool(hip.tune_get("rconv_stats"))
+        self._reduce_norm = bool(hip.tune_get("reduce_norm")) and dtype == torch.bfloat16
         self._rconv = hip.tune_get("rconv")
         self.spec = unet3d_spec(boc, cfg["cross_attention_dim"], cfg["audio_attention_dim"], self.in_channels,
                                 self.out_channels, cfg["layers_per_block"],
@@ -431,7 +437,9 @@
     def clear_banks(self):
         self._banks = {}
 
-    def _gn(self, p, x, eps, silu=False, x1=None):
+    def _gn(self, p, x, eps, silu=False, x1=None, normed=None):
+        if isinstance(normed, Normed) and x1 is None and normed.key == (p, eps, silu):
+            return normed.y.view(x.shape)
         nb, h, ww, c = x.shape
         y = hip.groupnorm(x.view(nb, h * ww, c), self.w[p + ".g"], self.w[p + ".b"], 32, eps, silu=silu,
                           x1=None if x1 is None else x1.view(nb, h * ww, -1))
@@ -454,6 +462,20 @@
                                 self.w[p + ".ff2.w"].shape[1])
         return self._ff(p, self._ln(norm, hid), hid)
 
+    def _next_norm(self, key, keep_raw=True):
+        if key is None:
+            return None
+        p, eps, silu = key
+        return (self.w[p + ".g"], self.w[p + ".b"], 32, eps, silu, keep_raw)
+
+    def _reader_norm(self, p, shape, resnet=False):
+        if not self._reduce_norm or p is None:
+            return None
+        nb, h, ww, c = shape
+        if resnet:
+            return None if self._resnet_fused(p, c, 0, h, ww) else (p + ".norm1", self.config.norm_eps, True)
+        return None if self._proj_in_fused(p, h * ww) else (p + ".norm", 1e-6, False)
+
     def _proj_in_fused(self, p, n):
         return (p + ".proj_in.img") in self.w and n > 256 and n % 128 == 0
 
@@ -461,26 +483,29 @@
         nb, h, ww, c = x.shape
         n = h * ww
         if self._proj_in_fused(p, n):
-            if tables is not None and tables[0].shape == (nb, c):
+            if tables is not None and not isinstance(tables, Normed) and tables[0].shape == (nb, c):
                 sc, sh = tables
             else:
                 sc, sh = hip.groupnorm_affine(x.view(nb, n, c), self.w[p + ".norm.g"], self.w[p + ".norm.b"], 32, 1e-6)
             return hip.rowgemm320(x.view(nb * n, c), self.w[p + ".proj_in.img"], self.w[p + ".proj_in.w"].shape[0], self.w.get(p + ".proj_in.bias"),
                                   pre_scale=sc, pre_shift=sh, pre_rows=n)[0]
-        xn = self._gn(p + ".norm", x, 1e-6)
+        xn = self._gn(p + ".norm", x, 1e-6, normed=tables)
         return self._lin(p + ".proj_in", xn.view(nb * n, c))
 
-    def _norm_ff_proj_out(self, p, norm, hid, q, x_res):
+    def _norm_ff_proj_out(self, p, norm, hid, q, x_res, next_norm=None, hw=0):
         img, po = self.w.get(p + ".ffimg"), self.w.get(q + ".proj_out.img")
         if img is not None and po is not None and (q + ".proj_out.bias") in self.w:
             return hip.ff_fused_po(hid, self.w[norm + ".g"], self.w[norm + ".b"], img, self.w[p + ".ff2.bias"], hid,
-                                   self.w[p + ".ff2.w"].shape[1], po, self.w[q + ".proj_out.bias"], x_res)
+                                   self.w[p + ".ff2.w"].shape[1], po, self.w[q + ".proj_out.bias"], x_res), None
         wcat = self._ffpo_weights(p, q) if img is None else None
         if wcat is not None and hid.shape[0] * max(wcat[0].shape[1] - hid.shape[1], hid.shape[1]) * 2 < hip.DMA_LIMIT:
             g = hip.gemm(self._ln(norm, hid), self.w[p + ".ff1.w"], self.w[p + ".ff1.bias"], act=hip.ACT_GEGLU)
-            return hip.conv1x1_cat(g, hid, wcat[0], wcat[1], residual=x_res)
+            if next_norm is not None:
+                y, yn = hip.conv1x1_cat(g, hid, wcat[0], wcat[1], residual=x_res, next_norm=self._next_norm(next_norm), hw=hw)
+                return y, (None if yn is None else Normed(next_norm, yn))
+            return hip.conv1x1_cat(g, hid, wcat[0], wcat[1], residual=x_res), None
         hid = self._norm_ff(p, norm, hid)
-        return hip.gemm(hid, self.w[q + ".proj_out.w"], self.w.get(q + ".proj_out.bias"), residual=x_res)
+        return hip.gemm(hid, self.w[q + ".proj_out.w"], self.w.get(q + ".proj_out.bias"), residual=x_res), None
 
     def _ffpo_weights(self, p, q):
         key = p + ".ffpo"
@@ -497,13 +522,17 @@
                 self._ffpo[key] = None
         return self._ffpo[key]
 
-    def _resnet(self, p, x, temb, skip=None, out=None, reader=None):
+    def _resnet_fused(self, p, c0, c1, h, ww):
+        cout = self.spec[p + ".conv1.weight"][0]
+        return bool(self._rconv & RCONV_LEVEL.get(cout, 0)) and \
+            hip.gn_silu_conv3x3_unet_supported(self._dtype, c0, c1, cout, h, ww) and hip.gn_silu_conv3x3_unet_supported(self._dtype, cout, 0, cout, h, ww)
+
+    def _resnet(self, p, x, temb, skip=None, out=None, reader=None, normed=None, next_norm=None):
         nb, h, ww, c0 = x.shape
         hw = h * ww
         cout = self.spec[p + ".conv1.weight"][0]
         c1 = 0 if skip is None else skip.shape[3]
-        fused = bool(self._rconv & RCONV_LEVEL.get(cout, 0)) and \
-            hip.gn_silu_conv3x3_unet_supported(self._dtype, c0, c1, cout, h, ww) and hip.gn_silu_conv3x3_unet_supported(self._dtype, cout, 0, cout, h, ww)
+        fused = self._resnet_fused(p, c0, c1, h, ww)
         if fused:
             eps = self.config.norm_eps
             sc, sh = hip.groupnorm_affine(x.view(nb, hw, c0), self.w[p + ".norm1.g"], self.w[p + ".norm1.b"], 32, eps,
@@ -515,12 +544,17 @@
                 hdn = hip.gn_silu_conv3x3_unet(x, sc, sh, self._rimg(p, ".conv1"), cout, self.w[p + ".conv1.bias"], temb[p], nb // temb[p].shape[0], x1=skip)
                 sc, sh = hip.groupnorm_affine(hdn.view(nb, hw, cout), self.w[p + ".norm2.g"], self.w[p + ".norm2.b"], 32, eps)
         else:
-            hdn = self._gn(p + ".norm1", x, self.config.norm_eps, silu=True, x1=skip)
+            hdn = self._gn(p + ".norm1", x, self.config.norm_eps, silu=True, x1=skip, normed=normed)
             b2rows = (nb // temb[p].shape[0]) * hw
             if temb[p].shape[0] == 1:
                 b2rows = max(b2rows, 256)
-            hdn = hip.conv3x3(hdn, self.w[p + ".conv1.w"], self.w[p + ".conv1.bias"], bias2=temb[p], bias2_rows=b2rows)
-            hdn = self._gn(p + ".norm2", hdn, self.config.norm_eps, silu=True)
+            nn2 = self._next_norm((p + ".norm2", self.config.norm_eps, True), keep_raw=False) if self._reduce_norm else None
+            if nn2 is not None:
+                raw, hdn = hip.conv3x3(hdn, self.w[p + ".conv1.w"], self.w[p + ".conv1.bias"], bias2=temb[p], bias2_rows=b2rows, next_norm=nn2)
+            else:
+                raw, hdn = hip.conv3x3(hdn, self.w[p + ".conv1.w"], self.w[p + ".conv1.bias"], bias2=temb[p], bias2_rows=b2rows), None
+            if hdn is None:
+                hdn = self._gn(p + ".norm2", raw, self.config.norm_eps, silu=True)
         if (p + ".sc.w") in self.w:
             wsc = self.w[p + ".sc.w"]
             if skip is None:
@@ -541,6 +575,9 @@
                 return hip.gn_silu_conv3x3_unet(hdn, sc, sh, self._rimg(p, ".conv2"), cout, self.w[p + ".conv2.bias"], residual=res, out=out,
                                                 next_norm=(self.w[reader + ".norm.g"], self.w[reader + ".norm.b"], 32, 1e-6))
             return hip.gn_silu_conv3x3_unet(hdn, sc, sh, self._rimg(p, ".conv2"), cout, self.w[p + ".conv2.bias"], residual=res, out=out), None
+        if next_norm is not None:
+            y, yn = hip.conv3x3(hdn, self.w[p + ".conv2.w"], self.w[p + ".conv2.bias"], residual=res, out=out, next_norm=self._next_norm(next_norm))
+            return y, (None if yn is None else Normed(next_norm, yn))
         return hip.conv3x3(hdn, self.w[p + ".conv2.w"], self.w[p + ".conv2.bias"], residual=res, out=out), None
 
     def _rimg(self, p, cv):
@@ -586,7 +623,7 @@
                       v_str=(inner * npad, 0, npad), o_str=(n * inner, 0, inner), v_transposed=True, **kw)
         return o
 
-    def _spatial_transformer(self, p, x, ehs, frames, write=None, cfg_row=None, tables=None):
+    def _spatial_transformer(self, p, x, ehs, frames, write=None, cfg_row=None, tables=None, next_norm=None):
         nb, h, ww, c = x.shape
         n = h * ww
         m = nb * n
@@ -609,8 +646,8 @@
         else:
             hid = hip.gemm(o, self.w[t + ".attn1.o.w"], self.w[t + ".attn1.o.bias"], residual=hid)
             hid = self._cross_attention(t, hid, ehs if cfg_row is None else ehs[cfg_row:cfg_row + 1], nb, n, inner)
-        out = self._norm_ff_proj_out(t + ".ff", t + ".norm3", hid, p, x.view(m, c))
-        return out.view(nb, h, ww, c)
+        out, nrm = self._norm_ff_proj_out(t + ".ff", t + ".norm3", hid, p, x.view(m, c), next_norm, n)
+        return out.view(nb, h, ww, c), nrm
 
     def _spatial_transformer_twin(self, p, x2, ehs, frames, tables=None):
         nb, h, ww, c = x2.shape
@@ -640,7 +677,7 @@
             sl = slice(row * f * n, (row + 1) * f * n)
             hip.gemm(o[sl], self.w[t + ".attn1.o.w"], self.w[t + ".attn1.o.bias"], residual=hid, bias2=cvec[row:row + 1],
                      bias2_rows=max(f * n, 256), out=hid2[sl])
-        out = self._norm_ff_proj_out(t + ".ff", t + ".norm3", hid2, p, x2.view(nb * n, c))
+        out, _ = self._norm_ff_proj_out(t + ".ff", t + ".norm3", hid2, p, x2.view(nb * n, c))
         return out.view(nb, h, ww, c)
 
     def _clip_vector(self, t, ehs):
@@ -669,12 +706,12 @@
                       o_str=(n * inner, 0, inner))
         return hip.gemm(o, self.w[t + ".attn2.o.w"], self.w[t + ".attn2.o.bias"], residual=hid)
 
-    def _audio_transformer(self, p, x, audio, masks, depth, motion_scale, ms_cache=None):
+    def _audio_transformer(self, p, x, audio, masks, depth, motion_scale, ms_cache=None, tables=None, next_norm=None):
         nb, h, ww, c = x.shape
         n = h * ww
         m = nb * n
         t = p + ".transformer_blocks.0"
-        hid = self._norm_proj_in(p, x)
+        hid = self._norm_proj_in(p, x, tables)
         inner = hid.shape[1]
         hd = inner // self.heads
         if (t + ".attn1.qkv_img") in self.w and n % 128 == 0:
@@ -721,8 +758,6 @@
                 rs, cols = kept
                 buf = torch.empty((m, kp), device=self._device, dtype=self._dtype)
                 buf[:, k3:] = cols
-                if m0:
-                    buf[:m0, :k3] = 0
                 ms_cache[ck] = (rs, buf)
             rs, a3 = ms_cache[ck]
             if nb0 < nb:
@@ -756,10 +791,10 @@
                     self._zbias[key] = (self.w[f"{t}.z{i}.bias"] * s).contiguous()
                 hid = hip.gemm_post(a3[:, i * inner:(i + 1) * inner], self.w[f"{t}.oz{i}.w"], self.w[f"{t}.oz{i}.bias"], mask, s,
                                     self._zbias[key], hid)
-        out = self._norm_ff_proj_out(t + ".ff", t + ".norm3", hid, p, x.view(m, c))
-        return out.view(nb, h, ww, c)
-
-    def _motion_module(self, p, x, frames):
+        out, nrm = self._norm_ff_proj_out(t + ".ff", t + ".norm3", hid, p, x.view(m, c), next_norm, n)
+        return out.view(nb, h, ww, c), nrm
+
+    def _motion_module(self, p, x, frames, tables=None, next_norm=None):
         nb, h, ww, c = x.shape
         n = h * ww
         m = nb * n
@@ -769,7 +804,7 @@
             raise RuntimeError("temporal attention window is limited to 32 frames (positional encoding max_len)")
         q = p + ".temporal_transformer"
         t = q + ".transformer_blocks.0"
-        hid = self._norm_proj_in(q, x)
+        hid = self._norm_proj_in(q, x, tables)
         for i in range(2):
             a = f"{t}.attention_blocks.{i}"
             if (a + ".tleg_img") in self.w and (f"{t}.norms.{i}.bpe") in self.w and hip.temporal_leg320_supported(self._dtype, c, self.heads, frames, n, b):
@@ -787,8 +822,8 @@
             hip.attention(qkv, qkv[:, c:], qkv[:, 2 * c:], o, batch=b * n, heads=self.heads, hd=hd, nq=frames, nk=frames,
                           scale=hd ** -0.5, q_str=st, k_str=st, v_str=st, o_str=(frames * n * c, c, n * c), bdiv=n)
             hid = hip.gemm(o, self.w[a + ".o.w"], self.w[a + ".o.bias"], residual=hid)
-        out = self._norm_ff_proj_out(t + ".ff", t + ".ff_norm", hid, q, x.view(m, c))
-        return out.view(nb, h, ww, c)
+        out, nrm = self._norm_ff_proj_out(t + ".ff", t + ".ff_norm", hid, q, x.view(m, c), next_norm, n)
+        return out.view(nb, h, ww, c), nrm
 
     def _time_embedding(self, timestep, batch):
         if not torch.is_tensor(timestep):
@@ -867,41 +902,58 @@
         ms_cache = {"state": window_state, "zero_images": int(audio_zero_rows) * f}
         ehs = encoder_hidden_states.to(self._device)
 
+        rn = self._reader_norm
+        mot = lambda q: q + ".temporal_transformer"
         skips = [x2 if shared else x]
+        tab = None
         for i in range(4):
             p = f"down_blocks.{i}"
             for j in range(lpb):
+                att = f"{p}.attentions.{j}" if i < 3 else None
+                aud = f"{p}.audio_modules.{j}" if i < 3 and f"{p}.audio_modules.{j}" in self._audio else None
+                mm = f"{p}.motion_modules.{j}"
                 if shared and i == 0 and j == 0:
                     r = f"{p}.resnets.0"
                     x2 = torch.empty((2 * hf,) + tuple(x.shape[1:3]) + (self.spec[r + ".conv1.weight"][0],), device=self._device, dtype=self._dtype)
-                    x, tab = self._resnet(r, x, {r: temb[r][:1]}, out=x2[:hf], reader=f"{p}.attentions.0" if self._twin else None)
+                    x, tab = self._resnet(r, x, {r: temb[r][:1]}, out=x2[:hf], reader=att if self._twin else None)
                     x2[hf:].copy_(x)
                     x = x2
                 else:
-                    x, tab = self._resnet(f"{p}.resnets.{j}", x, temb, reader=f"{p}.attentions.{j}" if i < 3 else None)
+                    x, tab = self._resnet(f"{p}.resnets.{j}", x, temb, reader=att, normed=tab, next_norm=rn(att or mot(mm), x.shape[:3] + (self.spec[f"{p}.resnets.{j}.conv1.weight"][0],)))
                 if i < 3:
-                    y = self._spatial_transformer_twin(f"{p}.attentions.{j}", x, ehs, f, tab) if (shared and i == 0 and j == 0 and self._twin) else None
-                    x = y if y is not None else self._spatial_transformer(f"{p}.attentions.{j}", x, ehs, f, cfg_row=cfg_row, tables=tab)
-                    if f"{p}.audio_modules.{j}" in self._audio:
-                        x = self._audio_transformer(f"{p}.audio_modules.{j}", x, audio, masks, i, ms, ms_cache)
-                x = self._motion_module(f"{p}.motion_modules.{j}", x, f)
+                    y = self._spatial_transformer_twin(att, x, ehs, f, tab) if (shared and i == 0 and j == 0 and self._twin) else None
+                    x, tab = (y, None) if y is not None else self._spatial_transformer(att, x, ehs, f, cfg_row=cfg_row, tables=tab, next_norm=rn(aud or mot(mm), x.shape))
+                    if aud:
+                        x, tab = self._audio_transformer(aud, x, audio, masks, i, ms, ms_cache, tables=tab, next_norm=rn(mot(mm), x.shape))
+                nxt = f"{p}.resnets.{j + 1}" if j + 1 < lpb else "mid_block.resnets.0" if i == 3 else None
+                x, tab = self._motion_module(mm, x, f, tables=tab, next_norm=rn(nxt, x.shape, resnet=True))
                 skips.append(x)
             if i != 3:
-                x = hip.conv3x3(x, self.w[f"{p}.downsamplers.0.conv.w"], self.w[f"{p}.downsamplers.0.conv.bias"], stride=2)
+                ds = f"{p}.downsamplers.0.conv"
+                key = rn(f"down_blocks.{i + 1}.resnets.0", (x.shape[0], x.shape[1] // 2, x.shape[2] // 2, self.spec[ds + ".weight"][0]), resnet=True)
+                if key is not None:
+                    x, yn = hip.conv3x3(x, self.w[ds + ".w"], self.w[ds + ".bias"], stride=2, next_norm=self._next_norm(key))
+                    tab = None if yn is None else Normed(key, yn)
+                else:
+                    x, tab = hip.conv3x3(x, self.w[ds + ".w"], self.w[ds + ".bias"], stride=2), None
                 skips.append(x)
 
-        x, _ = self._resnet("mid_block.resnets.0", x, temb)
-        x = self._spatial_transformer("mid_block.attentions.0", x, ehs, f, cfg_row=cfg_row)
-        x = self._motion_module("mid_block.motion_modules.0", x, f)
-        x, _ = self._resnet("mid_block.resnets.1", x, temb)
+        x, tab = self._resnet("mid_block.resnets.0", x, temb, normed=tab, next_norm=rn("mid_block.attentions.0", x.shape))
+        x, tab = self._spatial_transformer("mid_block.attentions.0", x, ehs, f, cfg_row=cfg_row, tables=tab, next_norm=rn(mot("mid_block.motion_modules.0"), x.shape))
+        x, tab = self._motion_module("mid_block.motion_modules.0", x, f, tables=tab, next_norm=rn("mid_block.resnets.1", x.shape, resnet=True))
+        x, _ = self._resnet("mid_block.resnets.1", x, temb, normed=tab)
 
         for i in range(4):
             p = f"up_blocks.{i}"
             for j in range(lpb + 1):
-                x, tab = self._resnet(f"{p}.resnets.{j}", x, temb, skip=skips.pop(), reader=f"{p}.attentions.{j}" if i > 0 else None)
+                att = f"{p}.attentions.{j}" if i > 0 else None
+                mm = f"{p}.motion_modules.{j}"
+                skip = skips.pop()
+                x, tab = self._resnet(f"{p}.resnets.{j}", x, temb, skip=skip, reader=att,
+                                      next_norm=rn(att or mot(mm), x.shape[:3] + (self.spec[f"{p}.resnets.{j}.conv1.weight"][0],)))
                 if i > 0:
-                    x = self._spatial_transformer(f"{p}.attentions.{j}", x, ehs, f, cfg_row=cfg_row, tables=tab)
-                x = self._motion_module(f"{p}.motion_modules.{j}", x, f)
+                    x, tab = self._spatial_transformer(att, x, ehs, f, cfg_row=cfg_row, tables=tab, next_norm=rn(mot(mm), x.shape))
+                x, _ = self._motion_module(mm, x, f, tables=tab)
             if i != 3:
                 x = self._upsample(f"{p}.upsamplers.0.conv", x)
 
```

New measurement: 14.91 steps/s. Within noise of the previous version (-0.0%).
